# leejaeyong7/tiny-cuda-nn

Hardware: AMD Instinct MI355X
Metric: training_step throughput (samples/s) HashGrid+64-wide FFMLP, batch=256k; % fp16-MFMA peak (higher is better)
Workload: dtype f16

## Files before the change

include/tcnn_amd.h:

```cpp
#ifndef TCNN_AMD_H
#define TCNN_AMD_H

#include <stddef.h>
#include <stdint.h>

#ifdef __cplusplus
extern "C" {
#endif

#define TCNN_OK 0
#define TCNN_ERROR 1

#define TCNN_PRECISION_FP32 0
#define TCNN_PRECISION_FP16 1

#define TCNN_GRADIENT_IGNORE 0
#define TCNN_GRADIENT_OVERWRITE 1
#define TCNN_GRADIENT_ACCUMULATE 2

#define TCNN_LAYOUT_SOA 0
#define TCNN_LAYOUT_AOS 1

#define TCNN_LOG_INFO 0
#define TCNN_LOG_DEBUG 1
#define TCNN_LOG_WARNING 2
#define TCNN_LOG_ERROR 3
#define TCNN_LOG_SUCCESS 4

#define TCNN_MEMCPY_HOST_TO_DEVICE 1
#define TCNN_MEMCPY_DEVICE_TO_HOST 2
#define TCNN_MEMCPY_DEVICE_TO_DEVICE 3

typedef struct tcnn_module_s* tcnn_module_t;
typedef struct tcnn_context_s* tcnn_context_t;
typedef struct tcnn_trainer_s* tcnn_trainer_t;
typedef struct tcnn_train_ctx_s* tcnn_train_ctx_t;
typedef struct tcnn_optimizer_s* tcnn_optimizer_t;
typedef void* tcnn_stream_t;

const char* tcnn_last_error(void);
const char* tcnn_version(void);

uint32_t tcnn_batch_size_granularity(void);
int      tcnn_device(int* device_out);
int      tcnn_set_device(int device);
void     tcnn_free_temporary_memory(void);
int      tcnn_has_networks(void);
float    tcnn_default_loss_scale(int precision);
int      tcnn_preferred_precision(void);
void     tcnn_set_log_callback(void (*callback)(int severity, const char* message, void* user), void* user);

int tcnn_gpu_malloc(size_t bytes, void** out);
int tcnn_gpu_free(void* ptr);
int tcnn_gpu_memcpy(void* dst, const void* src, size_t bytes, int kind);
int tcnn_gpu_memset(void* ptr, int value, size_t bytes);
int tcnn_stream_synchronize(tcnn_stream_t stream);
int tcnn_generate_random_uniform(tcnn_stream_t stream, uint64_t rng_state_inc[2], size_t n, float* out, float lower, float upper);

int  tcnn_create_network_with_input_encoding(uint32_t n_input_dims, uint32_t n_output_dims, const char* encoding_json, const char* network_json, tcnn_module_t* out);
int  tcnn_create_network(uint32_t n_input_dims, uint32_t n_output_dims, const char* network_json, tcnn_module_t* out);
int  tcnn_create_encoding(uint32_t n_input_dims, const char* encoding_json, int precision, tcnn_module_t* out);
int  tcnn_create_network_with_input_encoding_precision(uint32_t n_input_dims, uint32_t n_output_dims, const char* encoding_json, const char* network_json, int precision, tcnn_module_t* out);
int  tcnn_create_network_precision(uint32_t n_input_dims, uint32_t n_output_dims, const char* network_json, int precision, tcnn_module_t* out);
void tcnn_module_destroy(tcnn_module_t module);

int  tcnn_module_inference(tcnn_module_t m, tcnn_stream_t stream, uint32_t n_elements, const float* input, void* output, void* params);
int  tcnn_module_forward(tcnn_module_t m, tcnn_stream_t stream, uint32_t n_elements, const float* input, void* output, void* params,
                         int prepare_input_gradients, tcnn_context_t* ctx_out);
int  tcnn_module_backward(tcnn_module_t m, tcnn_stream_t stream, tcnn_context_t ctx, uint32_t n_elements, float* dL_dinput,
                          const void* dL_doutput, void* dL_dparams, const float* input, const void* output, const void* params);
int  tcnn_module_backward_backward_input(tcnn_module_t m, tcnn_stream_t stream, tcnn_context_t ctx, uint32_t n_elements, const float* dL_ddLdinput,
                                         const float* input, const void* dL_doutput, void* dL_dparams, void* dL_ddLdoutput, float* dL_dinput, const void* params);
int  tcnn_module_backward_backward_input_mode(tcnn_module_t m, tcnn_stream_t stream, tcnn_context_t ctx, uint32_t n_elements, const float* dL_ddLdinput,
                                              const float* input, const void* dL_doutput, void* dL_dparams, void* dL_ddLdoutput, float* dL_dinput, const void* params,
                                              int gradient_mode);
int  tcnn_module_input_gradient(tcnn_module_t m, tcnn_stream_t stream, uint32_t n_elements, uint32_t dim, const float* input, float* d_dinput, void* output,
                                const void* params, float backprop_scale);
const char* tcnn_module_last_input_gradient_route(tcnn_module_t m);
int  tcnn_module_input_jacobian(tcnn_module_t m, tcnn_stream_t stream, uint32_t n_elements, const uint32_t* dims, uint32_t n_dims, const float* input, float* jacobian,
                                void* output, const void* params, float backprop_scale);
const char* tcnn_module_last_input_jacobian_route(tcnn_module_t m);
int  tcnn_module_input_jvp(tcnn_module_t m, tcnn_stream_t stream, uint32_t n_elements, uint32_t n_tangents, const float* input, const float* tangents, void* jvp, void* output,
                           const void* params);
const char* tcnn_module_last_input_jvp_route(tcnn_module_t m);
int  tcnn_module_input_jvp_forward(tcnn_module_t m, tcnn_stream_t stream, uint32_t n_elements, uint32_t n_tangents, const float* input, const float* tangents, void* jvp,
                                   void* output, const void* params, tcnn_context_t* ctx_out);
int  tcnn_module_input_jvp_backward(tcnn_module_t m, tcnn_stream_t stream, tcnn_context_t ctx, uint32_t n_elements, uint32_t n_tangents, const float* input,
                                    const float* tangents, const void* dL_djvp, const void* dL_doutput, const void* params, void* dL_dparams, float* dL_dinput,
                                    float* dL_dtangents, int gradient_mode);
const char* tcnn_module_last_input_jvp_backward_route(tcnn_module_t m);
void tcnn_context_destroy(tcnn_context_t ctx);

uint32_t    tcnn_module_n_input_dims(tcnn_module_t m);
uint32_t    tcnn_module_n_output_dims(tcnn_module_t m);
size_t      tcnn_module_n_params(tcnn_module_t m);
int         tcnn_module_param_precision(tcnn_module_t m);
int         tcnn_module_output_precision(tcnn_module_t m);
int         tcnn_module_initialize_params(tcnn_module_t m, uint64_t seed, float* params_full_precision, float scale);
const char* tcnn_module_hyperparams(tcnn_module_t m);
const char* tcnn_module_name(tcnn_module_t m);

int  tcnn_create_from_config(uint32_t n_input_dims, uint32_t n_output_dims, const char* config_json, tcnn_trainer_t* out);
int  tcnn_create_from_config_seeded(uint32_t n_input_dims, uint32_t n_output_dims, const char* config_json, uint32_t seed, tcnn_trainer_t* out);
int  tcnn_create_from_config_precision(uint32_t n_input_dims, uint32_t n_output_dims, const char* config_json, uint32_t seed, int precision, tcnn_trainer_t* out);
int  tcnn_trainer_precision(tcnn_trainer_t t);
void tcnn_trainer_destroy(tcnn_trainer_t t);

int  tcnn_trainer_training_step(tcnn_trainer_t t, tcnn_stream_t stream, uint32_t n_elements, const float* input, int input_layout,
                                const float* target, const float* data_pdf, int run_optimizer, float* dL_dinput, int use_inference_params,
                                int gradient_mode, const void* external_dL_dy, tcnn_train_ctx_t* ctx_out);
int  tcnn_trainer_loss(tcnn_trainer_t t, tcnn_stream_t stream, tcnn_train_ctx_t ctx, float* loss_out);
int  tcnn_trainer_forward(tcnn_trainer_t t, tcnn_stream_t stream, float loss_scale, uint32_t n_elements, const float* input, int input_layout, const float* target,
                          const float* data_pdf, int use_inference_params, int prepare_input_gradients, const void* external_dL_dy, tcnn_train_ctx_t* ctx_out);
int  tcnn_trainer_backward(tcnn_trainer_t t, tcnn_stream_t stream, tcnn_train_ctx_t ctx, uint32_t n_elements, const float* input, int input_layout,
                           float* dL_dinput, int use_inference_params, int gradient_mode);
int  tcnn_trainer_optimizer_step(tcnn_trainer_t t, tcnn_stream_t stream, float loss_scale);
void tcnn_train_ctx_destroy(tcnn_train_ctx_t ctx);
const void*  tcnn_train_ctx_output(tcnn_train_ctx_t ctx);
const void*  tcnn_train_ctx_dL_doutput(tcnn_train_ctx_t ctx);
const float* tcnn_train_ctx_L(tcnn_train_ctx_t ctx);

int  tcnn_trainer_inference(tcnn_trainer_t t, tcnn_stream_t stream, uint32_t n_elements, const float* input, int input_layout,
                            float* output, int output_layout, int use_inference_params);
int  tcnn_trainer_input_gradient(tcnn_trainer_t t, tcnn_stream_t stream, uint32_t n_elements, uint32_t dim, const float* input, float* d_dinput, float backprop_scale);
int  tcnn_trainer_input_jacobian(tcnn_trainer_t t, tcnn_stream_t stream, uint32_t n_elements, const uint32_t* dims, uint32_t n_dims, const float* input, float* jacobian,
                                 float backprop_scale);
int  tcnn_trainer_input_jvp(tcnn_trainer_t t, tcnn_stream_t stream, uint32_t n_elements, uint32_t n_tangents, const float* input, const float* tangents, void* jvp);
int  tcnn_trainer_input_jvp_forward(tcnn_trainer_t t, tcnn_stream_t stream, uint32_t n_elements, uint32_t n_tangents, const float* input, const float* tangents, void* jvp,
                                    void* output, tcnn_context_t* ctx_out);
int  tcnn_trainer_input_jvp_backward(tcnn_trainer_t t, tcnn_stream_t stream, tcnn_context_t ctx, uint32_t n_elements, uint32_t n_tangents, const float* input,
                                     const float* tangents, const void* dL_djvp, const void* dL_doutput, float* dL_dinput, float* dL_dtangents, int gradient_mode);

int  tcnn_trainer_inference_mixed_precision(tcnn_trainer_t t, tcnn_stream_t stream, uint32_t n_elements, const float* input, int input_layout,
                                            void* output_half, int use_inference_params);

size_t   tcnn_trainer_n_params(tcnn_trainer_t t);
uint32_t tcnn_trainer_padded_output_width(tcnn_trainer_t t);
float*   tcnn_trainer_params_full_precision(tcnn_trainer_t t);
void*    tcnn_trainer_params(tcnn_trainer_t t);
void*    tcnn_trainer_params_inference(tcnn_trainer_t t);
void*    tcnn_trainer_param_gradients(tcnn_trainer_t t);
int      tcnn_trainer_set_params_full_precision(tcnn_trainer_t t, const float* params, size_t n_params, int device_ptr);
int      tcnn_trainer_set_params(tcnn_trainer_t t, const void* params_half, size_t n_params, int device_ptr);
int      tcnn_trainer_initialize_params(tcnn_trainer_t t);
int      tcnn_trainer_update_hyperparams(tcnn_trainer_t t, const char* json);
const char* tcnn_trainer_hyperparams(tcnn_trainer_t t);
int      tcnn_trainer_serialize(tcnn_trainer_t t, int serialize_optimizer, const void** out_bytes, size_t* out_size);
int      tcnn_trainer_deserialize(tcnn_trainer_t t, const void* bytes, size_t size);
const char* tcnn_trainer_network_hyperparams(tcnn_trainer_t t);
uint32_t tcnn_trainer_optimizer_step_count(tcnn_trainer_t t);
int  tcnn_trainer_profile_next_step(tcnn_trainer_t t);
int  tcnn_trainer_profile_collect(tcnn_trainer_t t, tcnn_stream_t stream, float* ms_per_piece , uint32_t* n_steps);
size_t tcnn_trainer_params_updated_in_flush(tcnn_trainer_t t);
size_t tcnn_trainer_image_preps(tcnn_trainer_t t);
size_t tcnn_trainer_scatter_wide_fallbacks(tcnn_trainer_t t);
size_t tcnn_trainer_optimizer_prologue_steps(tcnn_trainer_t t);
size_t tcnn_trainer_list_scatters(tcnn_trainer_t t);
size_t tcnn_module_list_scatters(tcnn_module_t m);
size_t tcnn_trainer_list_gradient_tails(tcnn_trainer_t t);
const char* tcnn_trainer_last_step_kernel(tcnn_trainer_t t);

int   tcnn_module_set_max_level(tcnn_module_t m, float max_level);
float tcnn_module_max_level(tcnn_module_t m);
int   tcnn_module_set_max_level_gpu(tcnn_module_t m, const float* per_sample);
int   tcnn_trainer_set_max_level(tcnn_trainer_t t, float max_level);
int   tcnn_trainer_set_max_level_gpu(tcnn_trainer_t t, const float* per_sample);
float tcnn_trainer_max_level(tcnn_trainer_t t);
int tcnn_train_ctx_keeps_weight_gradient_slabs(tcnn_trainer_t t, tcnn_train_ctx_t ctx);


int         tcnn_module_layer_sizes(tcnn_module_t m, uint32_t* rows_cols, size_t capacity, size_t* n_layers_out);
int         tcnn_optimizer_create(const char* optimizer_json, size_t n_params, const uint32_t* layer_sizes, size_t n_layers, tcnn_optimizer_t* out);
int         tcnn_optimizer_create_precision(const char* optimizer_json, size_t n_params, const uint32_t* layer_sizes, size_t n_layers, int weight_precision, tcnn_optimizer_t* out);
int         tcnn_optimizer_weight_precision(tcnn_optimizer_t o);
void        tcnn_optimizer_destroy(tcnn_optimizer_t o);
int         tcnn_optimizer_step(tcnn_optimizer_t o, tcnn_stream_t stream, float loss_scale, float* params_full_precision, void* params_half,
                                const void* gradients, int gradient_precision);
uint32_t    tcnn_optimizer_step_count(tcnn_optimizer_t o);
size_t      tcnn_optimizer_n_params(tcnn_optimizer_t o);
float       tcnn_optimizer_learning_rate(tcnn_optimizer_t o);
int         tcnn_optimizer_set_learning_rate(tcnn_optimizer_t o, float learning_rate);
int         tcnn_optimizer_update_hyperparams(tcnn_optimizer_t o, const char* json);
const char* tcnn_optimizer_hyperparams(tcnn_optimizer_t o);
void*       tcnn_optimizer_custom_weights(tcnn_optimizer_t o);
int         tcnn_optimizer_weights_restored(tcnn_optimizer_t o, tcnn_stream_t stream, const void* params_half);
int         tcnn_optimizer_serialize(tcnn_optimizer_t o, const void** out_bytes, size_t* out_size);
int         tcnn_optimizer_deserialize(tcnn_optimizer_t o, const void* bytes, size_t size);


int         tcnn_loss_type(const char* loss_json, int* type_out);
const char* tcnn_loss_name(int type);
int         tcnn_loss_evaluate(int type, tcnn_stream_t stream, float loss_scale, const float* scale_dev ,
                               uint32_t n, uint32_t dims, const void* prediction, uint32_t prediction_stride, int precision,
                               const float* target, const float* data_pdf ,
                               float* values, uint32_t values_stride,
                               void* gradients, uint32_t gradients_stride,
                               float* loss_sum );

#ifdef __cplusplus
}
#endif
#endif
```

tiny-cuda-nn_amd/csrc/adam_device.h:

```cpp
#pragma once
#include "tcnn_common.h"

namespace tcnn_amd {

template <typename DebiasOf, typename G, typename W>
__device__ inline void adam_one(const AdamArgs& a, DebiasOf&& debias_of, const float common_debias, const bool is_matrix, const G g_in, float& w_fp, W& w_h,
                                float& m1, float& m2, uint32_t& step, bool& updated) {
	const float g = (float)g_in;
	float gradient = a.inv_loss_scale_exact ? g * a.inv_loss_scale : g / a.loss_scale;
	updated = is_matrix ? a.optimize_matrix_params != 0 : (a.optimize_non_matrix_params != 0 && gradient != 0);
	const float weight_fp = w_fp;
	if (is_matrix) gradient += a.l2_reg * weight_fp;
	const float gradient_sq = gradient * gradient;
	const float first_moment = a.beta1 * m1 + (1 - a.beta1) * gradient;
	const float second_moment = a.beta2 * m2 + (1 - a.beta2) * gradient_sq;
	float learning_rate = a.learning_rate;
	if (!is_matrix) learning_rate *= a.non_matrix_learning_rate_factor;
	const uint32_t current_step = step + 1;
	float debias = common_debias;
	if (updated && current_step != a.common_step) debias = debias_of(min(current_step, a.common_step));
	learning_rate *= debias;
	const float effective_learning_rate = fminf(fmaxf(learning_rate / (sqrtf(second_moment) + a.epsilon), a.lower_lr_bound), a.upper_lr_bound);
	const float decayed_weight = (1 - a.relative_weight_decay * learning_rate) * weight_fp - copysignf(a.absolute_weight_decay * learning_rate, weight_fp);
	float new_weight = decayed_weight - effective_learning_rate * first_moment;
	if (a.weight_clipping_magnitude != 0.0f) new_weight = fminf(fmaxf(new_weight, -a.weight_clipping_magnitude), a.weight_clipping_magnitude);
	w_fp = updated ? new_weight : weight_fp;
	w_h = (W)new_weight;
	m1 = updated ? first_moment : m1;
	m2 = updated ? second_moment : m2;
	step = updated ? current_step : step;
}

}
```

tiny-cuda-nn_amd/csrc/capi.cpp:

```cpp
#include "../../include/tcnn_amd.h"

#include "model.h"

#include <mutex>
#include <string>

using namespace tcnn_amd;

namespace {
thread_local std::string g_last_error;
tcnn_amd::Switches g_switches;
std::mutex g_switches_mutex;

bool env_is(const char* name, char c) {
	const char* e = getenv(name);
	return e && e[0] == c;
}
int env_01(const char* name) {
	const char* e = getenv(name);
	return (e && (e[0] == '0' || e[0] == '1')) ? e[0] - '0' : -1;
}

template <typename F>
int guarded(F&& f) {
	try {
		f();
		return TCNN_OK;
	} catch (const std::exception& e) {
		g_last_error = e.what();
		log_message(TCNN_LOG_ERROR, g_last_error);
		return TCNN_ERROR;
	} catch (...) {
		g_last_error = "unknown error";
		return TCNN_ERROR;
	}
}

Json parse_or_empty(const char* text) {
	if (!text || !*text) return Json::object();
	return Json::parse(text);
}
}

struct tcnn_module_s {
	std::unique_ptr<Model> model;
	std::string hyperparams_text;
	std::string name_text;
};

struct tcnn_context_s {
	std::unique_ptr<ModelContext> ctx;
};

struct tcnn_trainer_s {
	std::unique_ptr<Trainer> trainer;
	std::string hyperparams_text;
	std::string network_hyperparams_text;
	std::vector<uint8_t> snapshot;
};

struct tcnn_train_ctx_s {
	std::unique_ptr<TrainContext> ctx;
};

struct tcnn_optimizer_s {
	std::unique_ptr<Optimizer> optimizer;
	size_t n_params = 0;
	std::string hyperparams_text;
	std::vector<uint8_t> snapshot;
};

namespace tcnn_amd {
Switches switches() {
	std::lock_guard<std::mutex> lock{g_switches_mutex};
	return g_switches;
}
void switches_reload() {
	Switches w;
	w.grid_planes = !env_is("TCNN_AMD_GRID_PLANES", '0');
	w.grid_rows_planes = !env_is("TCNN_AMD_GRID_ROWS_PLANES", '0');
	{ const char* e = getenv("TCNN_AMD_GRID_SCATTER"); w.grid_scatter_lds = !(e && std::string{e} == "atomic"); }
	w.scatter_records = !env_is("TCNN_AMD_SCATTER_RECORDS", '0');
	w.scatter_tune = !env_is("TCNN_AMD_SCATTER_TUNE", '0');
	w.scatter_lists = env_01("TCNN_AMD_SCATTER_LISTS");
	w.scatter_wide = env_is("TCNN_AMD_SCATTER_WIDE", '1');
	w.fused_step = !env_is("TCNN_AMD_FUSED_STEP", '0');
	w.side_jobs = !env_is("TCNN_AMD_SIDE_JOBS", '0');
	w.live_image = !env_is("TCNN_AMD_LIVE_IMAGE", '0');
	w.adam_steps32 = env_is("TCNN_AMD_ADAM_STEPS32", '1');
	w.adam_in_reduce = !env_is("TCNN_AMD_ADAM_IN_REDUCE", '0');
	w.adam_prologue = !env_is("TCNN_AMD_ADAM_PROLOGUE", '0');
	w.adam_prologue_refused = env_is("TCNN_AMD_ADAM_PROLOGUE", 'r');
	w.mlp_r32 = !env_is("TCNN_AMD_MLP_R32", '0');
	w.mlp_r32a = env_01("TCNN_AMD_MLP_R32A");
	w.mlp_regs = !env_is("TCNN_AMD_MLP_REGS", '0');
	w.mlp_fast = !env_is("TCNN_AMD_MLP_FAST", '0');
	if (const char* e = getenv("TCNN_AMD_MLP_PRIO")) w.mlp_prio = (uint32_t)atoi(e);
	w.listgrad_in_mlp = !env_is("TCNN_AMD_LISTGRAD_IN_MLP", '0');
	w.mlp_layerwise = env_is("TCNN_AMD_MLP_LAYERWISE", '1');
	w.mlp_regw = !env_is("TCNN_AMD_MLP_REGW", '0');
	if (const char* e = getenv("TCNN_AMD_MLP_VARIANT")) {
		int v[3] = {0, 0, 0};
		if (sscanf(e, "%d,%d,%d", &v[0], &v[1], &v[2]) == 3) {
			w.mlp_variant_forced = true;
			for (int i = 0; i < 3; ++i) w.mlp_variant[i] = v[i];
		}
	}
	w.wgrad_rows = !env_is("TCNN_AMD_WGRAD_ROWS", '0');
	w.mlp_fwd_lds = !env_is("TCNN_AMD_MLP_FWD_LDS", '0');
	w.fuse_oneblob = !env_is("TCNN_AMD_FUSE_ONEBLOB", '0');
	std::lock_guard<std::mutex> lock{g_switches_mutex};
	g_switches = w;
}
}

extern "C" {

const char* tcnn_last_error(void) { return g_last_error.c_str(); }
const char* tcnn_version(void) { return "tcnn_amd 0.1 (gfx950)"; }

uint32_t tcnn_batch_size_granularity(void) { return BATCH_SIZE_GRANULARITY; }

int tcnn_device(int* device_out) {
	return guarded([&] { HIP_CHECK_THROW(hipGetDevice(device_out)); });
}

int tcnn_set_device(int device) {
	return guarded([&] { HIP_CHECK_THROW(hipSetDevice(device)); });
}

void tcnn_free_temporary_memory(void) { Arena::instance().release_all(); }

int tcnn_gpu_malloc(size_t bytes, void** out) {
	return guarded([&] {
		CHECK_THROW(out != nullptr);
		*out = nullptr;
		if (bytes) HIP_CHECK_THROW(hipMalloc(out, bytes));
	});
}
int tcnn_gpu_free(void* ptr) {
	return guarded([&] { if (ptr) HIP_CHECK_THROW(hipFree(ptr)); });
}
int tcnn_gpu_memcpy(void* dst, const void* src, size_t bytes, int kind) {
	return guarded([&] {
		const hipMemcpyKind k = kind == TCNN_MEMCPY_HOST_TO_DEVICE ? hipMemcpyHostToDevice : kind == TCNN_MEMCPY_DEVICE_TO_HOST ? hipMemcpyDeviceToHost : hipMemcpyDeviceToDevice;
		if (bytes) HIP_CHECK_THROW(hipMemcpy(dst, src, bytes, k));
	});
}
int tcnn_gpu_memset(void* ptr, int value, size_t bytes) {
	return guarded([&] { if (bytes) HIP_CHECK_THROW(hipMemset(ptr, value, bytes)); });
}
int tcnn_stream_synchronize(tcnn_stream_t stream) {
	return guarded([&] { HIP_CHECK_THROW(hipStreamSynchronize((hipStream_t)stream)); });
}
int tcnn_generate_random_uniform(tcnn_stream_t stream, uint64_t rng_state_inc[2], size_t n, float* out, float lower, float upper) {
	return guarded([&] {
		CHECK_THROW(rng_state_inc != nullptr && (out != nullptr || n == 0));
		generate_random_uniform((hipStream_t)stream, rng_state_inc, n, out, lower, upper);
		HIP_CHECK_THROW(hipGetLastError());
	});
}
int tcnn_has_networks(void) { return 1; }
float tcnn_default_loss_scale(int precision) { return precision == TCNN_PRECISION_FP32 ? 1.0f : LOSS_SCALE_FP16; }
int tcnn_preferred_precision(void) { return TCNN_PRECISION_FP16; }

void tcnn_set_log_callback(void (*callback)(int, const char*, void*), void* user) {
	log_sink().callback = callback;
	log_sink().user = user;
}

int tcnn_create_network_with_input_encoding_precision(uint32_t n_input_dims, uint32_t n_output_dims, const char* encoding_json, const char* network_json, int precision, tcnn_module_t* out) {
	switches_reload();
	return guarded([&] {
		CHECK_THROW(out != nullptr);
		if (precision != TCNN_PRECISION_FP32 && precision != TCNN_PRECISION_FP16) throw std::runtime_error{"Unknown precision " + std::to_string(precision)};
		auto m = std::make_unique<tcnn_module_s>();
		m->model.reset(new NetworkWithInputEncoding{n_input_dims, n_output_dims, parse_or_empty(encoding_json), parse_or_empty(network_json),
		                                            precision == TCNN_PRECISION_FP32 ? Precision::Fp32 : Precision::Fp16});
		*out = m.release();
	});
}

int tcnn_create_network_with_input_encoding(uint32_t n_input_dims, uint32_t n_output_dims, const char* encoding_json, const char* network_json, tcnn_module_t* out) {
	return tcnn_create_network_with_input_encoding_precision(n_input_dims, n_output_dims, encoding_json, network_json, TCNN_PRECISION_FP16, out);
}

int tcnn_create_network_precision(uint32_t n_input_dims, uint32_t n_output_dims, const char* network_json, int precision, tcnn_module_t* out) {
	return tcnn_create_network_with_input_encoding_precision(n_input_dims, n_output_dims, "{\"otype\": \"Identity\"}", network_json, precision, out);
}

int tcnn_create_network(uint32_t n_input_dims, uint32_t n_output_dims, const char* network_json, tcnn_module_t* out) {
	return tcnn_create_network_precision(n_input_dims, n_output_dims, network_json, TCNN_PRECISION_FP16, out);
}

int tcnn_create_encoding(uint32_t n_input_dims, const char* encoding_json, int precision, tcnn_module_t* out) {
	switches_reload();
	return guarded([&] {
		CHECK_THROW(out != nullptr);
		auto m = std::make_unique<tcnn_module_s>();
		m->model.reset(new EncodingModel{n_input_dims, parse_or_empty(encoding_json), precision == TCNN_PRECISION_FP32 ? Precision::Fp32 : Precision::Fp16});
		*out = m.release();
	});
}

void tcnn_module_destroy(tcnn_module_t module) { delete module; }

int tcnn_module_inference(tcnn_module_t m, tcnn_stream_t stream, uint32_t n, const float* input, void* output, void* params) {
	return guarded([&] {
		CHECK_THROW(m && m->model);
		m->model->inference((hipStream_t)stream, n, MatView{input, m->model->input_width(), 1u}, output, params);
	});
}

int tcnn_module_forward(tcnn_module_t m, tcnn_stream_t stream, uint32_t n, const float* input, void* output, void* params, int prepare_input_gradients, tcnn_context_t* ctx_out) {
	return guarded([&] {
		CHECK_THROW(m && m->model && ctx_out);
		auto c = std::make_unique<tcnn_context_s>();
		c->ctx = m->model->forward((hipStream_t)stream, n, MatView{input, m->model->input_width(), 1u}, output, params, prepare_input_gradients != 0);
		*ctx_out = c.release();
	});
}

int tcnn_module_backward(tcnn_module_t m, tcnn_stream_t stream, tcnn_context_t ctx, uint32_t n, float* dL_dinput, const void* dL_doutput, void* dL_dparams,
                         const float* input, const void* output, const void* params) {
	return guarded([&] {
		CHECK_THROW(m && m->model);
		if (!ctx || !ctx->ctx || dynamic_cast<const Model::InputJvpContext*>(ctx->ctx.get())) {
			throw std::runtime_error{"Module::bwd: called with invalid context. fwd likely (mistakenly) ran in inference mode."};
		}
		MatViewMut dx{dL_dinput, m->model->input_width(), 1u};
		m->model->backward((hipStream_t)stream, *ctx->ctx, n, MatView{input, m->model->input_width(), 1u}, output, dL_doutput, dL_dinput ? &dx : nullptr, params,
		                   dL_dparams, dL_dparams ? GradientMode::Overwrite : GradientMode::Ignore);
	});
}

int tcnn_module_backward_backward_input(tcnn_module_t m, tcnn_stream_t stream, tcnn_context_t ctx, uint32_t n, const float* dL_ddLdinput, const float* input, const void* dL_doutput,
                                        void* dL_dparams, void* dL_ddLdoutput, float* dL_dinput, const void* params) {
	return tcnn_module_backward_backward_input_mode(m, stream, ctx, n, dL_ddLdinput, input, dL_doutput, dL_dparams, dL_ddLdoutput, dL_dinput, params,
	                                                dL_dparams ? TCNN_GRADIENT_OVERWRITE : TCNN_GRADIENT_IGNORE);
}

int tcnn_module_backward_backward_input_mode(tcnn_module_t m, tcnn_stream_t stream, tcnn_context_t ctx, uint32_t n, const float* dL_ddLdinput, const float* input, const void* dL_doutput,
                                             void* dL_dparams, void* dL_ddLdoutput, float* dL_dinput, const void* params, int gradient_mode) {
	return guarded([&] {
		CHECK_THROW(gradient_mode == TCNN_GRADIENT_IGNORE || ((gradient_mode == TCNN_GRADIENT_OVERWRITE || gradient_mode == TCNN_GRADIENT_ACCUMULATE) && dL_dparams != nullptr));
		CHECK_THROW(m && m->model);
		if (!ctx || !ctx->ctx || dynamic_cast<const Model::InputJvpContext*>(ctx->ctx.get())) {
			throw std::runtime_error{"Module::bwd_bwd_input: called with invalid context. fwd likely (mistakenly) ran in inference mode."};
		}
		CHECK_THROW(dL_ddLdinput != nullptr && input != nullptr);
		const uint32_t w = m->model->input_width();
		MatViewMut dx{dL_dinput, w, 1u};
		m->model->backward_backward_input((hipStream_t)stream, *ctx->ctx, n, MatView{input, w, 1u}, MatView{dL_ddLdinput, w, 1u}, dL_doutput, dL_ddLdoutput, dL_dinput ? &dx : nullptr, params,
		                                  gradient_mode == TCNN_GRADIENT_IGNORE ? nullptr : dL_dparams, (GradientMode)gradient_mode);
	});
}

int tcnn_module_input_gradient(tcnn_module_t m, tcnn_stream_t stream, uint32_t n, uint32_t dim, const float* input, float* d_dinput, void* output, const void* params,
                               float backprop_scale) {
	return guarded([&] {
		CHECK_THROW(m && m->model);
		const uint32_t w = m->model->input_width();
		m->model->input_gradient((hipStream_t)stream, n, dim, MatView{input, w, 1u}, MatViewMut{d_dinput, w, 1u}, output, params, backprop_scale);
	});
}

const char* tcnn_module_last_input_gradient_route(tcnn_module_t m) {
	if (!m || !m->model) {
		g_last_error = "tcnn_module_last_input_gradient_route: null module";
		return nullptr;
	}
	return m->model->last_input_gradient_route();
}

int tcnn_module_input_jacobian(tcnn_module_t m, tcnn_stream_t stream, uint32_t n, const uint32_t* dims, uint32_t n_dims, const float* input, float* jacobian, void* output,
                               const void* params, float backprop_scale) {
	return guarded([&] {
		CHECK_THROW(m && m->model);
		m->model->input_jacobian((hipStream_t)stream, n, dims, n_dims, MatView{input, m->model->input_width(), 1u}, jacobian, output, params, backprop_scale);
	});
}

const char* tcnn_module_last_input_jacobian_route(tcnn_module_t m) {
	if (!m || !m->model) {
		g_last_error = "tcnn_module_last_input_jacobian_route: null module";
		return nullptr;
	}
	return m->model->last_input_jacobian_route();
}

int tcnn_module_input_jvp(tcnn_module_t m, tcnn_stream_t stream, uint32_t n, uint32_t n_tangents, const float* input, const float* tangents, void* jvp, void* output, const void* params) {
	return guarded([&] {
		CHECK_THROW(m && m->model);
		m->model->input_jvp((hipStream_t)stream, n, n_tangents, MatView{input, m->model->input_width(), 1u}, tangents, jvp, output, params);
	});
}

const char* tcnn_module_last_input_jvp_route(tcnn_module_t m) {
	if (!m || !m->model) {
		g_last_error = "tcnn_module_last_input_jvp_route: null module";
		return nullptr;
	}
	return m->model->last_input_jvp_route();
}

int tcnn_module_input_jvp_forward(tcnn_module_t m, tcnn_stream_t stream, uint32_t n, uint32_t n_tangents, const float* input, const float* tangents, void* jvp, void* output,
                                  const void* params, tcnn_context_t* ctx_out) {
	return guarded([&] {
		CHECK_THROW(m && m->model && ctx_out);
		auto c = std::make_unique<tcnn_context_s>();
		c->ctx = m->model->input_jvp_forward((hipStream_t)stream, n, n_tangents, MatView{input, m->model->input_width(), 1u}, tangents, jvp, output, params);
		*ctx_out = c.release();
	});
}

int tcnn_module_input_jvp_backward(tcnn_module_t m, tcnn_stream_t stream, tcnn_context_t ctx, uint32_t n, uint32_t n_tangents, const float* input, const float* tangents,
                                   const void* dL_djvp, const void* dL_doutput, const void* params, void* dL_dparams, float* dL_dinput, float* dL_dtangents, int gradient_mode) {
	return guarded([&] {
		CHECK_THROW(gradient_mode == TCNN_GRADIENT_IGNORE || ((gradient_mode == TCNN_GRADIENT_OVERWRITE || gradient_mode == TCNN_GRADIENT_ACCUMULATE) && dL_dparams != nullptr));
		CHECK_THROW(m && m->model);
		if (!ctx || !ctx->ctx) throw std::runtime_error{"Module::bwd: called with invalid context. fwd likely (mistakenly) ran in inference mode."};
		MatViewMut dx{dL_dinput, m->model->input_width(), 1u};
		m->model->input_jvp_backward((hipStream_t)stream, *ctx->ctx, n, n_tangents, MatView{input, m->model->input_width(), 1u}, tangents, dL_djvp, dL_doutput, params,
		                             gradient_mode == TCNN_GRADIENT_IGNORE ? nullptr : dL_dparams, dL_dinput ? &dx : nullptr, dL_dtangents, (GradientMode)gradient_mode);
	});
}

const char* tcnn_module_last_input_jvp_backward_route(tcnn_module_t m) {
	if (!m || !m->model) {
		g_last_error = "tcnn_module_last_input_jvp_backward_route: null module";
		return nullptr;
	}
	return m->model->last_input_jvp_backward_route();
}

void tcnn_context_destroy(tcnn_context_t ctx) { delete ctx; }

uint32_t tcnn_module_n_input_dims(tcnn_module_t m) { return m->model->input_width(); }
uint32_t tcnn_module_n_output_dims(tcnn_module_t m) { return m->model->padded_output_width(); }
size_t tcnn_module_n_params(tcnn_module_t m) { return m->model->n_params(); }
size_t tcnn_module_list_scatters(tcnn_module_t m) { return (size_t)m->model->list_scatters(); }

namespace {
[[noreturn]] void no_grid(Model& model) {
	throw std::runtime_error{"max_level: " + model.name() + " has no grid encoding (GridEncoding::set_max_level, grid_interface.h:101-123)"};
}
}

int tcnn_module_set_max_level(tcnn_module_t m, float max_level) {
	return guarded([&] {
		CHECK_THROW(m && m->model);
		if (!m->model->set_max_level(max_level)) no_grid(*m->model);
	});
}
int tcnn_module_set_max_level_gpu(tcnn_module_t m, const float* per_sample) {
	return guarded([&] {
		CHECK_THROW(m && m->model);
		if (!m->model->set_max_level_gpu(per_sample)) no_grid(*m->model);
	});
}
float tcnn_module_max_level(tcnn_module_t m) {
	float v = std::numeric_limits<float>::quiet_NaN();
	const float* per_sample = nullptr;
	guarded([&] {
		CHECK_THROW(m && m->model);
		if (!m->model->get_max_level(v, per_sample)) no_grid(*m->model);
		g_last_error.clear();
	});
	return v;
}
int tcnn_module_param_precision(tcnn_module_t m) { return (int)m->model->precision(); }
int tcnn_module_output_precision(tcnn_module_t m) { return (int)m->model->precision(); }

int tcnn_module_initialize_params(tcnn_module_t m, uint64_t seed, float* params_full_precision, float scale) {
	return guarded([&] {
		CHECK_THROW(m && m->model);
		Pcg32 rng{seed};
		m->model->initialize_params(rng, params_full_precision, scale);
		HIP_CHECK_THROW(hipDeviceSynchronize());
	});
}

const char* tcnn_module_hyperparams(tcnn_module_t m) {
	m->hyperparams_text = m->model->hyperparams().dump();
	return m->hyperparams_text.c_str();
}

const char* tcnn_module_name(tcnn_module_t m) {
	m->name_text = m->model->name();
	return m->name_text.c_str();
}

int tcnn_create_from_config_precision(uint32_t n_input_dims, uint32_t n_output_dims, const char* config_json, uint32_t seed, int precision, tcnn_trainer_t* out) {
	switches_reload();
	return guarded([&] {
		CHECK_THROW(out != nullptr);
		if (precision != TCNN_PRECISION_FP32 && precision != TCNN_PRECISION_FP16) throw std::runtime_error{"Unknown precision " + std::to_string(precision)};
		auto t = std::make_unique<tcnn_trainer_s>();
		t->trainer.reset(new Trainer{n_input_dims, n_output_dims, parse_or_empty(config_json), seed, precision == TCNN_PRECISION_FP32 ? Precision::Fp32 : Precision::Fp16});
		*out = t.release();
	});
}

int tcnn_create_from_config_seeded(uint32_t n_input_dims, uint32_t n_output_dims, const char* config_json, uint32_t seed, tcnn_trainer_t* out) {
	return tcnn_create_from_config_precision(n_input_dims, n_output_dims, config_json, seed, TCNN_PRECISION_FP16, out);
}

int tcnn_trainer_precision(tcnn_trainer_t t) {
	int v = -1;
	guarded([&] { CHECK_THROW(t && t->trainer); v = (int)t->trainer->precision(); });
	return v;
}

int tcnn_create_from_config(uint32_t n_input_dims, uint32_t n_output_dims, const char* config_json, tcnn_trainer_t* out) {
	return tcnn_create_from_config_seeded(n_input_dims, n_output_dims, config_json, 1337, out);
}

void tcnn_trainer_destroy(tcnn_trainer_t t) { delete t; }

int tcnn_trainer_training_step(tcnn_trainer_t t, tcnn_stream_t stream, uint32_t n, const float* input, int input_layout, const float* target, const float* data_pdf,
                               int run_optimizer, float* dL_dinput, int use_inference_params, int gradient_mode, const void* external_dL_dy, tcnn_train_ctx_t* ctx_out) {
	return guarded([&] {
		CHECK_THROW(t && t->trainer && ctx_out);
		Trainer& tr = *t->trainer;
		const uint32_t w = tr.model().input_width();
		MatViewMut dx = make_view_mut(dL_dinput, w, n, input_layout);
		auto c = std::make_unique<tcnn_train_ctx_s>();
		c->ctx = tr.training_step((hipStream_t)stream, n, make_view(input, w, n, input_layout), target, data_pdf, run_optimizer != 0, dL_dinput ? &dx : nullptr,
		                          use_inference_params != 0, (GradientMode)gradient_mode, external_dL_dy);
		*ctx_out = c.release();
	});
}

int tcnn_trainer_loss(tcnn_trainer_t t, tcnn_stream_t stream, tcnn_train_ctx_t ctx, float* loss_out) {
	return guarded([&] {
		CHECK_THROW(t && t->trainer && ctx && ctx->ctx && loss_out);
		*loss_out = t->trainer->loss((hipStream_t)stream, *ctx->ctx);
	});
}

int tcnn_trainer_forward(tcnn_trainer_t t, tcnn_stream_t stream, float loss_scale, uint32_t n, const float* input, int input_layout, const float* target, const float* data_pdf,
                         int use_inference_params, int prepare_input_gradients, const void* external_dL_dy, tcnn_train_ctx_t* ctx_out) {
	return guarded([&] {
		CHECK_THROW(t && t->trainer && ctx_out);
		Trainer& tr = *t->trainer;
		auto c = std::make_unique<tcnn_train_ctx_s>();
		c->ctx = tr.forward((hipStream_t)stream, loss_scale, n, make_view(input, tr.model().input_width(), n, input_layout), target, data_pdf, use_inference_params != 0,
		                    prepare_input_gradients != 0, external_dL_dy);
		*ctx_out = c.release();
	});
}

int tcnn_trainer_backward(tcnn_trainer_t t, tcnn_stream_t stream, tcnn_train_ctx_t ctx, uint32_t n, const float* input, int input_layout, float* dL_dinput,
                          int use_inference_params, int gradient_mode) {
	return guarded([&] {
		CHECK_THROW(t && t->trainer && ctx && ctx->ctx);
		Trainer& tr = *t->trainer;
		const uint32_t w = tr.model().input_width();
		MatViewMut dx = make_view_mut(dL_dinput, w, n, input_layout);
		tr.backward((hipStream_t)stream, *ctx->ctx, n, make_view(input, w, n, input_layout), dL_dinput ? &dx : nullptr, use_inference_params != 0, (GradientMode)gradient_mode);
	});
}

int tcnn_trainer_optimizer_step(tcnn_trainer_t t, tcnn_stream_t stream, float loss_scale) {
// ... 337 lines not shown
```

tiny-cuda-nn_amd/csrc/k_misc.hip:

```cpp
#include "tcnn_common.h"
#include "adam_device.h"
#include "grid_fixed.h"
#include "loss_device.h"
#include "mlp_side_jobs.h"
#include "oneblob_device.h"
#include "reduce_device.h"

#include <hip/hip_fp16.h>

#include <cmath>
#include <limits>

namespace tcnn_amd {
namespace {

typedef _Float16 half_t;
typedef _Float16 h8 __attribute__((ext_vector_type(8)));
typedef _Float16 h4 __attribute__((ext_vector_type(4)));

template <typename T>
__global__ void __launch_bounds__(256) k_oneblob_fwd(const uint32_t n, const uint32_t n_dims, const uint32_t log2_bins, const MatView x, T* __restrict__ out, const uint32_t out_stride) {
	const uint32_t gid = blockIdx.x * blockDim.x + threadIdx.x;
	const uint32_t i = gid / out_stride;
	if (i >= n) return;
	const uint32_t j = gid - i * out_stride;
	const uint32_t n_bins = 1u << log2_bins;
	if (j >= n_dims * n_bins) {
		out[gid] = (T)1.0f;
		return;
	}
	const uint32_t dim = j >> log2_bins, bin = j & (n_bins - 1);
	const float xv = x.data[(size_t)i * x.stride_sample + (size_t)dim * x.stride_dim];
	const float nb = (float)n_bins;
	const float lb = scalbnf((float)bin, -(int)log2_bins);
	const float l = quartic_cdf(lb - xv, nb) + quartic_cdf(lb - xv - 1.0f, nb) + quartic_cdf(lb - xv + 1.0f, nb);
	const float rb = scalbnf((float)((bin + 1) & (n_bins - 1)), -(int)log2_bins);
	float r = quartic_cdf(rb - xv, nb) + quartic_cdf(rb - xv - 1.0f, nb) + quartic_cdf(rb - xv + 1.0f, nb);
	if (bin == n_bins - 1) r += 1;
	out[gid] = (T)(r - l);
}

template <typename T>
__global__ void __launch_bounds__(256) k_oneblob_fwd8(const uint32_t n, const uint32_t n_dims, const uint32_t log2_bins, const MatView x, T* __restrict__ out, const uint32_t out_stride) {
	const uint32_t gid = blockIdx.x * blockDim.x + threadIdx.x;
	const uint32_t chunks = out_stride / 8;
	const uint32_t i = gid / chunks;
	if (i >= n) return;
	const uint32_t j0 = (gid - i * chunks) * 8;
	const uint32_t n_bins = 1u << log2_bins;
	typedef T vec8 __attribute__((ext_vector_type(8)));
	vec8 v;
	if (j0 >= n_dims * n_bins) {
#pragma unroll
		for (int k = 0; k < 8; ++k) v[k] = (T)1.0f;
	} else {
		const uint32_t dim = j0 >> log2_bins, b0 = j0 & (n_bins - 1);
		const float xv = x.data[(size_t)i * x.stride_sample + (size_t)dim * x.stride_dim];
		const float nb = (float)n_bins;
		float edge[9];
#pragma unroll
		for (int k = 0; k < 9; ++k) {
			const float lb = scalbnf((float)((b0 + k) & (n_bins - 1)), -(int)log2_bins);
			edge[k] = quartic_cdf(lb - xv, nb) + quartic_cdf(lb - xv - 1.0f, nb) + quartic_cdf(lb - xv + 1.0f, nb);
		}
		if (b0 + 8 == n_bins) edge[8] += 1;
#pragma unroll
		for (int k = 0; k < 8; ++k) v[k] = (T)(edge[k + 1] - edge[k]);
	}
	*(vec8*)(out + (size_t)i * out_stride + j0) = v;
}

template <typename T, int CPR>
__global__ void __launch_bounds__(256) k_oneblob_fwd_sparse(const uint32_t n, const uint32_t n_dims, const uint32_t log2_bins, const MatView x, T* __restrict__ out, const uint32_t out_stride) {
	const uint32_t gid = blockIdx.x * blockDim.x + threadIdx.x;
	typedef T vec8 __attribute__((ext_vector_type(8)));
	const uint32_t n_bins = 1u << log2_bins;
	constexpr uint32_t cpr = CPR;
	const uint32_t row_threads = n * n_dims * cpr;
	if (gid >= row_threads) {
		const uint32_t pad_chunks = (out_stride - n_dims * n_bins) >> 3;
		const uint32_t p = gid - row_threads;
		if (pad_chunks == 0 || p >= n * pad_chunks) return;
		const uint32_t i = p / pad_chunks, pc = p - i * pad_chunks;
		vec8 ones;
#pragma unroll
		for (int k = 0; k < 8; ++k) ones[k] = (T)1.0f;
		*(vec8*)(out + (size_t)i * out_stride + n_dims * n_bins + 8 * pc) = ones;
		return;
	}
	const uint32_t r = gid / cpr, j = gid - r * cpr;
	const uint32_t i = r / n_dims, dim = r - i * n_dims;
	const uint32_t b0 = 8 * j;
	const float xv = x.data[(size_t)i * x.stride_sample + (size_t)dim * x.stride_dim];
	const float nb = (float)n_bins;
	auto edge = [&](const uint32_t bin) {
		const float lb = scalbnf((float)(bin & (n_bins - 1)), -(int)log2_bins);
		return quartic_cdf(lb - xv, nb) + quartic_cdf(lb - xv - 1.0f, nb) + quartic_cdf(lb - xv + 1.0f, nb);
	};
	vec8 v;
	if (!(xv >= 0.0f && xv <= 1.0f)) {
		float e[9];
#pragma unroll
		for (int k = 0; k < 9; ++k) e[k] = edge(b0 + k);
		if (b0 + 8 == n_bins) e[8] += 1;
#pragma unroll
		for (int k = 0; k < 8; ++k) v[k] = (T)(e[k + 1] - e[k]);
	} else {
		const uint32_t centre = (uint32_t)(int)floorf(xv * nb) + n_bins - 2u;
		constexpr int PER = (5 + CPR - 1) / CPR;
		float mine[PER];
#pragma unroll
		for (int t = 0; t < PER; ++t) {
			const uint32_t o = min(j + (uint32_t)t * cpr, 4u);
			const uint32_t bin = (centre + o) & (n_bins - 1);
			const float l = edge(bin);
			float rr = edge(bin + 1);
			if (bin == n_bins - 1) rr += 1;
			mine[t] = rr - l;
		}
#pragma unroll
		for (int k = 0; k < 8; ++k) v[k] = (T)0.0f;
#pragma unroll
		for (int o = 0; o < 5; ++o) {
			const float val = CPR == 1 ? mine[o / CPR] : __shfl(mine[o / CPR], o % CPR, CPR);
			const uint32_t d = ((centre + o) & (n_bins - 1)) - b0;
#pragma unroll
			for (int k = 0; k < 8; ++k) v[k] = d == (uint32_t)k ? (T)val : v[k];
		}
	}
	*(vec8*)(out + (size_t)i * out_stride + (size_t)dim * n_bins + b0) = v;
}

template <typename T>
__global__ void __launch_bounds__(128) k_oneblob_bwd_input(const uint32_t n, const uint32_t n_dims, const uint32_t log2_bins, const MatView x, const T* __restrict__ dL_dy, const uint32_t dy_stride, const MatViewMut dL_dx) {
	const uint32_t gid = blockIdx.x * blockDim.x + threadIdx.x;
	const uint32_t i = gid / n_dims;
	if (i >= n) return;
	const uint32_t j = gid - i * n_dims;
	const uint32_t n_bins = 1u << log2_bins;
	const float nb = (float)n_bins;
	const float xv = x.data[(size_t)i * x.stride_sample + (size_t)j * x.stride_dim];
	float result = 0;
	float left = quartic_cdf_deriv(-xv, nb) + quartic_cdf_deriv(-xv - 1.0f, nb) + quartic_cdf_deriv(-xv + 1.0f, nb);
	for (uint32_t k = 0; k < n_bins; ++k) {
		const float rb = scalbnf((float)(k + 1), -(int)log2_bins);
		const float right = quartic_cdf_deriv(rb - xv, nb) + quartic_cdf_deriv(rb - xv - 1.0f, nb) + quartic_cdf_deriv(rb - xv + 1.0f, nb);
		const float deriv = left - right;
		left = right;
		result += (float)dL_dy[(size_t)i * dy_stride + j * n_bins + k] * deriv;
	}
	dL_dx.data[(size_t)i * dL_dx.stride_sample + (size_t)j * dL_dx.stride_dim] = result;
}

template <typename T>
__global__ void __launch_bounds__(256) k_identity_fwd(const uint32_t n, const uint32_t n_dims, const float scale, const float offset, const MatView x, T* __restrict__ out, const uint32_t out_stride) {
	const uint32_t gid = blockIdx.x * blockDim.x + threadIdx.x;
	const uint32_t i = gid / out_stride;
	if (i >= n) return;
	const uint32_t j = gid - i * out_stride;
	out[gid] = j >= n_dims ? (T)1.0f : (T)(x.data[(size_t)i * x.stride_sample + (size_t)j * x.stride_dim] * scale + offset);
}

template <typename T>
__global__ void __launch_bounds__(256) k_identity_bwd_input(const uint32_t n, const uint32_t n_dims, const float scale, const T* __restrict__ dL_dy, const uint32_t dy_stride, const MatViewMut dL_dx) {
	const uint32_t gid = blockIdx.x * blockDim.x + threadIdx.x;
	const uint32_t i = gid / n_dims;
	if (i >= n) return;
	const uint32_t j = gid - i * n_dims;
	dL_dx.data[(size_t)i * dL_dx.stride_sample + (size_t)j * dL_dx.stride_dim] = (float)(T)((float)dL_dy[(size_t)i * dy_stride + j] * scale);
}

template <typename T>
__global__ void __launch_bounds__(256) k_identity_bwd_bwd_input(const uint32_t n, const uint32_t n_dims, const float scale, const MatView dL_ddLdx, T* __restrict__ dL_ddLdy, const uint32_t dy_stride) {
	const uint32_t gid = blockIdx.x * blockDim.x + threadIdx.x;
	const uint32_t i = gid / dy_stride;
	if (i >= n) return;
	const uint32_t j = gid - i * dy_stride;
	dL_ddLdy[gid] = j >= n_dims ? (T)0.0f : (T)(dL_ddLdx.data[(size_t)i * dL_ddLdx.stride_sample + (size_t)j * dL_ddLdx.stride_dim] * scale);
}


template <typename P>
__global__ void __launch_bounds__(256) k_loss(
	const uint32_t type, const uint32_t n_elements, const uint32_t stride, const uint32_t dims, const float loss_scale,
	const P* __restrict__ predictions, const float* __restrict__ targets, float* __restrict__ values, P* __restrict__ gradients, const float* __restrict__ data_pdf
) {
	const uint32_t i = blockIdx.x * blockDim.x + threadIdx.x;
	if (i >= n_elements) return;
	const uint32_t intra = i % stride;
	const uint32_t inter = i / stride;
	if (intra >= dims) {
		values[i] = 0;
		gradients[i] = (P)0.0f;
		return;
	}
	const uint32_t target_idx = inter * dims + intra;
	const uint32_t n_total = n_elements / stride * dims;
	const float prediction = (float)predictions[i];
	const float pdf = data_pdf ? data_pdf[target_idx] : 1;
	float value;
	P grad;
	loss_element(type, prediction, targets[target_idx], pdf, n_total, loss_scale, predictions + (i - intra), dims, value, grad);
	values[i] = value;
	gradients[i] = grad;
}

__global__ void __launch_bounds__(256) k_loss8(
	const uint32_t type, const uint32_t n_elements, const uint32_t stride, const uint32_t dims, const uint32_t n_total, const float loss_scale,
	const half_t* __restrict__ predictions, const float* __restrict__ targets, float* __restrict__ values, half_t* __restrict__ gradients, const float* __restrict__ data_pdf
) {
	const uint32_t i0 = (blockIdx.x * blockDim.x + threadIdx.x) * 8;
	if (i0 >= n_elements) return;
	const uint32_t inter = i0 / stride, intra0 = i0 - inter * stride;
	const h8 pv = *(const h8*)(predictions + i0);
	float v[8];
	h8 g;
#pragma unroll
	for (int k = 0; k < 8; ++k) {
		const uint32_t intra = intra0 + k;
		v[k] = 0;
		g[k] = (half_t)0.0f;
		if (intra < dims) {
			const uint32_t target_idx = inter * dims + intra;
			const float pdf = data_pdf ? data_pdf[target_idx] : 1;
			half_t gk;
			loss_element(type, (float)pv[k], targets[target_idx], pdf, n_total, loss_scale, predictions + (i0 - intra0), dims, v[k], gk);
			g[k] = gk;
		}
	}
	*(float4*)(values + i0) = float4{v[0], v[1], v[2], v[3]};
	*(float4*)(values + i0 + 4) = float4{v[4], v[5], v[6], v[7]};
	*(h8*)(gradients + i0) = g;
}

__global__ void __launch_bounds__(256) k_loss4_f32(
	const uint32_t type, const uint32_t n_elements, const uint32_t stride, const uint32_t dims, const uint32_t n_total, const float loss_scale,
	const float* __restrict__ predictions, const float* __restrict__ targets, float* __restrict__ values, float* __restrict__ gradients, const float* __restrict__ data_pdf
) {
	const uint32_t i0 = (blockIdx.x * blockDim.x + threadIdx.x) * 4;
	if (i0 >= n_elements) return;
	const uint32_t inter = i0 / stride, intra0 = i0 - inter * stride;
	const float4 pv4 = *(const float4*)(predictions + i0);
	const float pv[4] = {pv4.x, pv4.y, pv4.z, pv4.w};
	float v[4], g[4];
#pragma unroll
	for (int k = 0; k < 4; ++k) {
		const uint32_t intra = intra0 + k;
		v[k] = 0;
		g[k] = 0;
		if (intra < dims) {
			const uint32_t target_idx = inter * dims + intra;
			const float pdf = data_pdf ? data_pdf[target_idx] : 1;
			loss_element(type, pv[k], targets[target_idx], pdf, n_total, loss_scale, predictions + (i0 - intra0), dims, v[k], g[k]);
		}
	}
	*(float4*)(values + i0) = float4{v[0], v[1], v[2], v[3]};
	*(float4*)(gradients + i0) = float4{g[0], g[1], g[2], g[3]};
}

__global__ void __launch_bounds__(256) k_reduce_stage1(const size_t n, const float* __restrict__ values, float* __restrict__ partials) {
	__shared__ float sm[4];
	float acc = 0.0f;
	const size_t n4 = n / 4;
	const float4* v4 = (const float4*)values;
	for (size_t i = (size_t)blockIdx.x * blockDim.x + threadIdx.x; i < n4; i += (size_t)gridDim.x * blockDim.x) {
		const float4 v = v4[i];
		acc += (v.x + v.y) + (v.z + v.w);
	}
	if (blockIdx.x == 0 && threadIdx.x < (n & 3)) acc += values[n4 * 4 + threadIdx.x];
	const float s = block_sum_256(acc, sm);
	if (threadIdx.x == 0) partials[blockIdx.x] = s;
}

__global__ void __launch_bounds__(256) k_reduce_stage2(const uint32_t n_partials, const float* __restrict__ partials, float* __restrict__ result) {
	__shared__ float sm[4];
	float acc = 0.0f;
	for (uint32_t i = threadIdx.x; i < n_partials; i += 256) acc += partials[i];
	const float s = block_sum_256(acc, sm);
	if (threadIdx.x == 0) *result = s;
}


__device__ inline float adam_debias(const float beta1, const float beta2, uint32_t step) { return sqrtf(1 - powf(beta2, (float)step)) / (1 - powf(beta1, (float)step)); }

__global__ void __launch_bounds__(256) k_adam_debias_table(const float beta1, const float beta2, const uint32_t from, const uint32_t to, float* __restrict__ table) {
	const uint32_t t = from + blockIdx.x * blockDim.x + threadIdx.x;
	if (t < to) table[t] = adam_debias(beta1, beta2, t);
}

constexpr int ADAM_Q = 1;

typedef uint16_t adam_u16x4 __attribute__((ext_vector_type(4)));
template <typename STEP_T> __device__ inline uint4 adam_load_steps(const STEP_T* p) {
	if constexpr (sizeof(STEP_T) == 2) {
		const adam_u16x4 v = *(const adam_u16x4*)p;
		return uint4{v[0], v[1], v[2], v[3]};
	} else {
		return *(const uint4*)p;
	}
}
template <typename STEP_T> __device__ inline void adam_store_steps(STEP_T* p, const uint4 v) {
	if constexpr (sizeof(STEP_T) == 2) *(adam_u16x4*)p = adam_u16x4{(uint16_t)v.x, (uint16_t)v.y, (uint16_t)v.z, (uint16_t)v.w};
	else *(uint4*)p = v;
}
typedef float f4 __attribute__((ext_vector_type(4)));
template <typename G> struct GradQuad;
template <> struct GradQuad<half_t> { typedef h4 type; };
template <> struct GradQuad<float> { typedef f4 type; };
template <bool QUAD_UNIFORM, typename STEP_T, typename G, typename W>
__global__ void __launch_bounds__(256) k_adam(
	const AdamArgs a, const size_t n, const size_t n_matrix,
	float* __restrict__ w_fp, W* __restrict__ w, const G* __restrict__ g, float* __restrict__ m1, float* __restrict__ m2, STEP_T* __restrict__ steps,
	const float* __restrict__ debias_table
) {
	const size_t base = (size_t)blockIdx.x * (256 * 4 * ADAM_Q) + threadIdx.x * 4;
	const float debias = debias_table[a.common_step];
	const auto from_table = [&](const uint32_t t) { return debias_table[t]; };
	typedef typename GradQuad<G>::type g4;
	g4 gv[ADAM_Q];
	bool live[ADAM_Q];
#pragma unroll
	for (int q = 0; q < ADAM_Q; ++q) {
		const size_t i4 = base + (size_t)q * 1024;
		live[q] = i4 + 4 <= n;
		gv[q] = live[q] ? *(const g4*)(g + i4) : g4{0, 0, 0, 0};
	}
#pragma unroll
	for (int q = 0; q < ADAM_Q; ++q) {
		const size_t i4 = base + (size_t)q * 1024;
		const bool zero = gv[q][0] == (G)0.0f && gv[q][1] == (G)0.0f && gv[q][2] == (G)0.0f && gv[q][3] == (G)0.0f;
		if (live[q] && i4 >= n_matrix && zero) live[q] = false;
	}
	float4 wf[ADAM_Q], a1[ADAM_Q], a2[ADAM_Q];
	uint4 st[ADAM_Q];
#pragma unroll
	for (int q = 0; q < ADAM_Q; ++q) {
		const size_t i4 = base + (size_t)q * 1024;
		if (live[q]) {
			wf[q] = *(const float4*)(w_fp + i4);
			a1[q] = *(const float4*)(m1 + i4);
			a2[q] = *(const float4*)(m2 + i4);
			st[q] = adam_load_steps(steps + i4);
		}
	}
#pragma unroll
	for (int q = 0; q < ADAM_Q; ++q) {
		const size_t i4 = base + (size_t)q * 1024;
		if (live[q]) {
			W wh[4];
			bool up[4];
			const bool quad_matrix = i4 < n_matrix;
			adam_one(a, from_table, debias, QUAD_UNIFORM ? quad_matrix : i4 + 0 < n_matrix, gv[q][0], wf[q].x, wh[0], a1[q].x, a2[q].x, st[q].x, up[0]);
			adam_one(a, from_table, debias, QUAD_UNIFORM ? quad_matrix : i4 + 1 < n_matrix, gv[q][1], wf[q].y, wh[1], a1[q].y, a2[q].y, st[q].y, up[1]);
			adam_one(a, from_table, debias, QUAD_UNIFORM ? quad_matrix : i4 + 2 < n_matrix, gv[q][2], wf[q].z, wh[2], a1[q].z, a2[q].z, st[q].z, up[2]);
			adam_one(a, from_table, debias, QUAD_UNIFORM ? quad_matrix : i4 + 3 < n_matrix, gv[q][3], wf[q].w, wh[3], a1[q].w, a2[q].w, st[q].w, up[3]);
			*(float4*)(w_fp + i4) = wf[q];
			*(float4*)(m1 + i4) = a1[q];
			*(float4*)(m2 + i4) = a2[q];
			adam_store_steps(steps + i4, st[q]);
			if constexpr (sizeof(W) == 2) {
				if (up[0] && up[1] && up[2] && up[3]) {
					*(h4*)(w + i4) = h4{wh[0], wh[1], wh[2], wh[3]};
				} else {
#pragma unroll
					for (int e = 0; e < 4; ++e) if (up[e]) w[i4 + e] = wh[e];
				}
			}
		} else if (i4 < n && i4 + 4 > n) {
			for (size_t i = i4; i < n; ++i) {
				bool up;
				W wh;
				uint32_t st1 = steps[i];
				adam_one(a, from_table, debias, i < n_matrix, g[i], w_fp[i], wh, m1[i], m2[i], st1, up);
				steps[i] = (STEP_T)st1;
				if constexpr (sizeof(W) == 2) { if (up) w[i] = wh; }
			}
		}
	}
}

template <typename STEP_T, typename G, typename W>
__global__ void __launch_bounds__(256) k_adam_scalar(
	const AdamArgs a, const size_t n, const size_t n_matrix,
	float* __restrict__ w_fp, W* __restrict__ w, const G* __restrict__ g, float* __restrict__ m1, float* __restrict__ m2, STEP_T* __restrict__ steps,
	const float* __restrict__ debias_table
) {
	const size_t i = (size_t)blockIdx.x * blockDim.x + threadIdx.x;
	if (i >= n) return;
	const float debias = debias_table[a.common_step];
	const auto from_table = [&](const uint32_t t) { return debias_table[t]; };
	bool up;
	W wh;
	uint32_t st1 = steps[i];
	adam_one(a, from_table, debias,  i < n_matrix, g[i], w_fp[i], wh, m1[i], m2[i], st1, up);
	steps[i] = (STEP_T)st1;
	if constexpr (sizeof(W) == 2) { if (up) w[i] = wh; }
}

__global__ void __launch_bounds__(128) k_random_uniform(const size_t n, const uint64_t state, const uint64_t inc, float* __restrict__ out, const float lower, const float upper) {
	const uint64_t MULT = 0x5851f42d4c957f2dULL;
	const size_t i = (size_t)blockIdx.x * blockDim.x + threadIdx.x;
	const size_t n_threads = (size_t)blockDim.x * gridDim.x;
	uint64_t cur_mult = MULT, cur_plus = inc, acc_mult = 1u, acc_plus = 0u;
	uint64_t delta = (uint64_t)i * 4;
	while (delta > 0) {
		if (delta & 1) {
			acc_mult *= cur_mult;
			acc_plus = acc_plus * cur_mult + cur_plus;
		}
		cur_plus = (cur_mult + 1) * cur_plus;
		cur_mult *= cur_mult;
		delta /= 2;
	}
	uint64_t st = acc_mult * state + acc_plus;
	for (size_t j = 0; j < 4; ++j) {
		const size_t idx = i + n_threads * j;
		if (idx >= n) return;
		const uint64_t old = st;
		st = old * MULT + inc;
		const uint32_t xorshifted = (uint32_t)(((old >> 18u) ^ old) >> 27u);
		const uint32_t rot = (uint32_t)(old >> 59u);
		const uint32_t u = ((xorshifted >> rot) | (xorshifted << ((~rot + 1u) & 31)));
		const float f = __uint_as_float((u >> 9) | 0x3f800000u) - 1.0f;
		out[idx] = f * (upper - lower) + lower;
	}
}

__global__ void __launch_bounds__(256) k_cast_f2h(const size_t n, const float* __restrict__ in, half_t* __restrict__ out) {
	const size_t i = ((size_t)blockIdx.x * blockDim.x + threadIdx.x) * 4;
	if (i + 4 <= n) {
		const float4 v = *(const float4*)(in + i);
		*(h4*)(out + i) = h4{(half_t)v.x, (half_t)v.y, (half_t)v.z, (half_t)v.w};
	} else {
		for (size_t k = i; k < n; ++k) out[k] = (half_t)in[k];
	}
}

__global__ void __launch_bounds__(256) k_cast_h2f(const size_t n, const half_t* __restrict__ in, float* __restrict__ out) {
	const size_t i = ((size_t)blockIdx.x * blockDim.x + threadIdx.x) * 4;
	if (i + 4 <= n) {
		const h4 v = *(const h4*)(in + i);
		*(float4*)(out + i) = float4{(float)v[0], (float)v[1], (float)v[2], (float)v[3]};
	} else {
		for (size_t k = i; k < n; ++k) out[k] = (float)in[k];
	}
}

template <typename T>
__global__ void __launch_bounds__(256) k_trim_and_cast(const uint32_t n, const uint32_t in_stride, const uint32_t dims, const T* __restrict__ in, const MatViewMut out) {
	const uint32_t gid = blockIdx.x * blockDim.x + threadIdx.x;
	const uint32_t i = gid / dims;
	if (i >= n) return;
	const uint32_t d = gid - i * dims;
	out.data[(size_t)i * out.stride_sample + (size_t)d * out.stride_dim] = (float)in[(size_t)i * in_stride + d];
}

__global__ void __launch_bounds__(256) k_fill_half(const size_t n, half_t* __restrict__ out, const half_t v) {
	const size_t i = (size_t)blockIdx.x * blockDim.x + threadIdx.x;
	if (i < n) out[i] = v;
}

inline uint32_t log2_exact(uint32_t v) {
	uint32_t l = 0;
	while ((1u << l) < v) ++l;
	return l;
}

inline uint32_t blocks_for(uint64_t total, uint32_t threads) {
	const uint64_t b = (total + threads - 1) / threads;
	CHECK_THROW(b < (1ull << 31));
	return (uint32_t)b;
}

}

void oneblob_forward(hipStream_t stream, bool fp32, uint32_t n, uint32_t n_dims, uint32_t n_bins, MatView x, void* out, uint32_t out_stride) {
	const uint64_t total = (uint64_t)n * out_stride;
	if (total == 0) return;
	CHECK_THROW(total < (1ull << 32));
	const uint32_t lb = log2_exact(n_bins);
	if (n_bins % 8 == 0 && n_bins <= 512 && out_stride % 8 == 0) {
		const uint64_t threads = total / 8;
		const dim3 grid(blocks_for(threads, 256));
#define TCNN_ONEBLOB_SPARSE(CPR_) \
		case CPR_: \
			if (fp32) hipLaunchKernelGGL((k_oneblob_fwd_sparse<float, CPR_>), grid, dim3(256), 0, stream, n, n_dims, lb, x, (float*)out, out_stride); \
			else hipLaunchKernelGGL((k_oneblob_fwd_sparse<half_t, CPR_>), grid, dim3(256), 0, stream, n, n_dims, lb, x, (half_t*)out, out_stride); \
			break;
		switch (n_bins / 8) {
			TCNN_ONEBLOB_SPARSE(1) TCNN_ONEBLOB_SPARSE(2) TCNN_ONEBLOB_SPARSE(4) TCNN_ONEBLOB_SPARSE(8)
			TCNN_ONEBLOB_SPARSE(16) TCNN_ONEBLOB_SPARSE(32) TCNN_ONEBLOB_SPARSE(64)
			default: CHECK_THROW(false);
		}
#undef TCNN_ONEBLOB_SPARSE
		return;
	}
	if (n_bins % 8 == 0 && out_stride % 8 == 0) {
		const uint64_t threads = total / 8;
		if (fp32) hipLaunchKernelGGL(k_oneblob_fwd8<float>, dim3(blocks_for(threads, 256)), dim3(256), 0, stream, n, n_dims, lb, x, (float*)out, out_stride);
		else hipLaunchKernelGGL(k_oneblob_fwd8<half_t>, dim3(blocks_for(threads, 256)), dim3(256), 0, stream, n, n_dims, lb, x, (half_t*)out, out_stride);
		return;
	}
	if (fp32) hipLaunchKernelGGL(k_oneblob_fwd<float>, dim3(blocks_for(total, 256)), dim3(256), 0, stream, n, n_dims, lb, x, (float*)out, out_stride);
	else hipLaunchKernelGGL(k_oneblob_fwd<half_t>, dim3(blocks_for(total, 256)), dim3(256), 0, stream, n, n_dims, lb, x, (half_t*)out, out_stride);
}

void oneblob_backward_input(hipStream_t stream, bool fp32, uint32_t n, uint32_t n_dims, uint32_t n_bins, MatView x, const void* dL_dy, uint32_t dy_stride, MatViewMut dL_dx) {
	const uint64_t total = (uint64_t)n * n_dims;
	if (total == 0) return;
	const uint32_t lb = log2_exact(n_bins);
	if (fp32) hipLaunchKernelGGL(k_oneblob_bwd_input<float>, dim3(blocks_for(total, 128)), dim3(128), 0, stream, n, n_dims, lb, x, (const float*)dL_dy, dy_stride, dL_dx);
	else hipLaunchKernelGGL(k_oneblob_bwd_input<half_t>, dim3(blocks_for(total, 128)), dim3(128), 0, stream, n, n_dims, lb, x, (const half_t*)dL_dy, dy_stride, dL_dx);
}

void identity_forward(hipStream_t stream, bool fp32, uint32_t n, uint32_t n_dims, float scale, float offset, MatView x, void* out, uint32_t out_stride) {
	const uint64_t total = (uint64_t)n * out_stride;
	if (total == 0) return;
	CHECK_THROW(total < (1ull << 32));
	if (fp32) hipLaunchKernelGGL(k_identity_fwd<float>, dim3(blocks_for(total, 256)), dim3(256), 0, stream, n, n_dims, scale, offset, x, (float*)out, out_stride);
	else hipLaunchKernelGGL(k_identity_fwd<half_t>, dim3(blocks_for(total, 256)), dim3(256), 0, stream, n, n_dims, scale, offset, x, (half_t*)out, out_stride);
}

void identity_backward_input(hipStream_t stream, bool fp32, uint32_t n, uint32_t n_dims, float scale, const void* dL_dy, uint32_t dy_stride, MatViewMut dL_dx) {
	const uint64_t total = (uint64_t)n * n_dims;
	if (total == 0) return;
	if (fp32) hipLaunchKernelGGL(k_identity_bwd_input<float>, dim3(blocks_for(total, 256)), dim3(256), 0, stream, n, n_dims, scale, (const float*)dL_dy, dy_stride, dL_dx);
	else hipLaunchKernelGGL(k_identity_bwd_input<half_t>, dim3(blocks_for(total, 256)), dim3(256), 0, stream, n, n_dims, scale, (const half_t*)dL_dy, dy_stride, dL_dx);
}

void identity_backward_backward_input(hipStream_t stream, bool fp32, uint32_t n, uint32_t n_dims, float scale, MatView dL_ddLdx, void* dL_ddLdy, uint32_t dy_stride) {
	const uint64_t total = (uint64_t)n * dy_stride;
	if (total == 0) return;
	CHECK_THROW(total < (1ull << 32));
	if (fp32) hipLaunchKernelGGL(k_identity_bwd_bwd_input<float>, dim3(blocks_for(total, 256)), dim3(256), 0, stream, n, n_dims, scale, dL_ddLdx, (float*)dL_ddLdy, dy_stride);
	else hipLaunchKernelGGL(k_identity_bwd_bwd_input<half_t>, dim3(blocks_for(total, 256)), dim3(256), 0, stream, n, n_dims, scale, dL_ddLdx, (half_t*)dL_ddLdy, dy_stride);
}

void loss_evaluate(hipStream_t stream, LossType type, uint32_t n, uint32_t stride, uint32_t dims, float loss_scale,
                   const void* pred_half, const float* target, float* values, void* grads_half, const float* data_pdf, Precision precision) {
	const uint64_t total = (uint64_t)n * stride;
	if (total == 0) return;
	CHECK_THROW(total < (1ull << 32));
	if (precision == Precision::Fp32) {
		if (stride % 4 == 0 && ((uintptr_t)pred_half | (uintptr_t)values | (uintptr_t)grads_half) % 16 == 0) {
			hipLaunchKernelGGL(k_loss4_f32, dim3(blocks_for(total / 4, 256)), dim3(256), 0, stream, (uint32_t)type, (uint32_t)total, stride, dims, (uint32_t)(total / stride * dims), loss_scale,
			                   (const float*)pred_half, target, values, (float*)grads_half, data_pdf);
			return;
		}
		hipLaunchKernelGGL(k_loss<float>, dim3(blocks_for(total, 256)), dim3(256), 0, stream, (uint32_t)type, (uint32_t)total, stride, dims, loss_scale,
		                   (const float*)pred_half, target, values, (float*)grads_half, data_pdf);
		return;
	}
	if (stride % 8 == 0 && ((uintptr_t)pred_half | (uintptr_t)values | (uintptr_t)grads_half) % 16 == 0) {
		hipLaunchKernelGGL(k_loss8, dim3(blocks_for(total / 8, 256)), dim3(256), 0, stream, (uint32_t)type, (uint32_t)total, stride, dims, (uint32_t)(total / stride * dims), loss_scale,
		                   (const half_t*)pred_half, target, values, (half_t*)grads_half, data_pdf);
		return;
	}
	hipLaunchKernelGGL(k_loss<half_t>, dim3(blocks_for(total, 256)), dim3(256), 0, stream, (uint32_t)type, (uint32_t)total, stride, dims, loss_scale,
	                   (const half_t*)pred_half, target, values, (half_t*)grads_half, data_pdf);
}

void reduce_sum(hipStream_t stream, size_t n, const float* values, float* partials, float* result_dev) {
	uint32_t blocks = blocks_for((n + 3) / 4, 256);
	if (blocks > 1024) blocks = 1024;
	if (blocks == 0) blocks = 1;
	hipLaunchKernelGGL(k_reduce_stage1, dim3(blocks), dim3(256), 0, stream, n, values, partials);
	hipLaunchKernelGGL(k_reduce_stage2, dim3(1), dim3(256), 0, stream, blocks, partials, result_dev);
}

void reduce_partials(hipStream_t stream, uint32_t n_partials, const float* partials, float* result_dev) {
	hipLaunchKernelGGL(k_reduce_stage2, dim3(1), dim3(256), 0, stream, n_partials, partials, result_dev);
}

AdamArgs make_adam_args(const AdamHyper& h, float loss_scale, uint32_t current_step) {
	AdamArgs a;
	a.relative_weight_decay = h.relative_decay;
	a.absolute_weight_decay = h.absolute_decay;
	a.weight_clipping_magnitude = h.clipping_magnitude;
	a.loss_scale = loss_scale;
	a.learning_rate = h.learning_rate;
	a.non_matrix_learning_rate_factor = h.non_matrix_learning_rate_factor;
	a.beta1 = h.beta1;
	a.beta2 = h.beta2;
	a.epsilon = h.epsilon;
	a.lower_lr_bound = 0;
	a.upper_lr_bound = std::numeric_limits<float>::max();
	if (h.adabound) {
		a.lower_lr_bound = 0.1f - 0.1f / ((1 - h.beta2) * (float)current_step + 1);
		a.upper_lr_bound = 0.1f + 0.1f / ((1 - h.beta2) * (float)current_step);
	}
	a.l2_reg = h.l2_reg;
	a.optimize_matrix_params = h.optimize_matrix_params;
	a.optimize_non_matrix_params = h.optimize_non_matrix_params;
	a.common_step = current_step;
	int exponent = 0;
	a.inv_loss_scale_exact = (std::frexp(loss_scale, &exponent) == 0.5f && loss_scale >= 1.0f / 65536 && loss_scale <= 65536.0f) ? 1 : 0;
	a.inv_loss_scale = 1.0f / loss_scale;
	return a;
}

namespace {
__global__ void __launch_bounds__(256) k_adam_widen_steps(const size_t n, const uint16_t* __restrict__ in, uint32_t* __restrict__ out) {
	const size_t i = (size_t)blockIdx.x * blockDim.x + threadIdx.x;
	if (i < n) out[i] = in[i];
}
template <typename STEP_T, typename G, typename W>
void adam_launch(hipStream_t stream, const AdamArgs& a, size_t n, size_t n_matrix, float* w_fp, W* w, const G* g, float* m1, float* m2, STEP_T* steps, const float* debias_table) {
	const auto aligned = [](const void* p, size_t bytes) { return ((uintptr_t)p & (bytes - 1)) == 0; };
	if (!(aligned(w_fp, 16) && aligned(m1, 16) && aligned(m2, 16) && aligned(steps, 4 * sizeof(STEP_T)) && (sizeof(W) == 4 || aligned(w, 8)) && aligned(g, 4 * sizeof(G)))) {
		hipLaunchKernelGGL((k_adam_scalar<STEP_T, G, W>), dim3(blocks_for(n, 256)), dim3(256), 0, stream, a, n, n_matrix, w_fp, w, g, m1, m2, steps, debias_table);
		return;
	}
	const dim3 grid(blocks_for((n + 3) / 4, 256 * ADAM_Q));
	if (n_matrix % 4 == 0) hipLaunchKernelGGL((k_adam<true, STEP_T, G, W>), grid, dim3(256), 0, stream, a, n, n_matrix, w_fp, w, g, m1, m2, steps, debias_table);
	else hipLaunchKernelGGL((k_adam<false, STEP_T, G, W>), grid, dim3(256), 0, stream, a, n, n_matrix, w_fp, w, g, m1, m2, steps, debias_table);
}
template <typename G, typename W>
void adam_launch_steps(hipStream_t stream, const AdamArgs& a, size_t n, size_t n_matrix, float* w_fp, W* w, const G* g, float* m1, float* m2, void* steps, bool steps16, const float* debias_table) {
	if (steps16) adam_launch<uint16_t, G, W>(stream, a, n, n_matrix, w_fp, w, g, m1, m2, (uint16_t*)steps, debias_table);
	else adam_launch<uint32_t, G, W>(stream, a, n, n_matrix, w_fp, w, g, m1, m2, (uint32_t*)steps, debias_table);
}
}

void adam_widen_steps(hipStream_t stream, size_t n, const void* steps16, void* steps32) {
	if (n == 0) return;
	hipLaunchKernelGGL(k_adam_widen_steps, dim3(blocks_for(n, 256)), dim3(256), 0, stream, n, (const uint16_t*)steps16, (uint32_t*)steps32);
}

void adam_step(hipStream_t stream, const AdamHyper& h, size_t n, size_t n_matrix, float loss_scale, uint32_t current_step,
               float* w_fp, void* w_half, const void* gradients, float* m1, float* m2, void* steps, bool steps16, const float* debias_table, GradientPrecision precision, Precision weight_precision) {
	if (n == 0) return;
	const AdamArgs a = make_adam_args(h, loss_scale, current_step);
	if (weight_precision == Precision::Fp32) {
		CHECK_THROW(precision == GradientPrecision::Fp32);
		adam_launch_steps(stream, a, n, n_matrix, w_fp, (float*)nullptr, (const float*)gradients, m1, m2, steps, steps16, debias_table);
	} else if (precision == GradientPrecision::Fp32) adam_launch_steps(stream, a, n, n_matrix, w_fp, (half_t*)w_half, (const float*)gradients, m1, m2, steps, steps16, debias_table);
	else adam_launch_steps(stream, a, n, n_matrix, w_fp, (half_t*)w_half, (const half_t*)gradients, m1, m2, steps, steps16, debias_table);
}

namespace {
constexpr uint32_t PRO_THREADS = SLAB_REDUCE_ELEMS * SLAB_REDUCE_GROUPS;
constexpr uint32_t PRO_MAX_BLOCKS_PER_RANGE = 64;
__host__ __device__ inline uint32_t pro_range_blocks(const uint32_t n_elems) { return min(PRO_MAX_BLOCKS_PER_RANGE, max(1u, (n_elems / 4 + PRO_THREADS - 1) / PRO_THREADS)); }

template <typename STEP_T, typename DebiasOf>
__device__ inline void adam_quad(const AdamArgs& a, DebiasOf&& from_table, const float debias, const bool quad_matrix, const size_t i4, const h4 gv,
                                 float* __restrict__ w_fp, half_t* __restrict__ w, float* __restrict__ m1, float* __restrict__ m2, STEP_T* __restrict__ steps) {
	if (!quad_matrix && gv[0] == (half_t)0.0f && gv[1] == (half_t)0.0f && gv[2] == (half_t)0.0f && gv[3] == (half_t)0.0f) return;
	float4 wf = *(const float4*)(w_fp + i4), a1 = *(const float4*)(m1 + i4), a2 = *(const float4*)(m2 + i4);
	uint4 st = adam_load_steps(steps + i4);
	half_t wh[4];
	bool up[4];
	adam_one(a, from_table, debias, quad_matrix, gv[0], wf.x, wh[0], a1.x, a2.x, st.x, up[0]);
	adam_one(a, from_table, debias, quad_matrix, gv[1], wf.y, wh[1], a1.y, a2.y, st.y, up[1]);
	adam_one(a, from_table, debias, quad_matrix, gv[2], wf.z, wh[2], a1.z, a2.z, st.z, up[2]);
	adam_one(a, from_table, debias, quad_matrix, gv[3], wf.w, wh[3], a1.w, a2.w, st.w, up[3]);
	*(float4*)(w_fp + i4) = wf;
	*(float4*)(m1 + i4) = a1;
	*(float4*)(m2 + i4) = a2;
	adam_store_steps(steps + i4, st);
	if (up[0] && up[1] && up[2] && up[3]) {
		*(h4*)(w + i4) = h4{wh[0], wh[1], wh[2], wh[3]};
	} else {
#pragma unroll
		for (int e = 0; e < 4; ++e) if (up[e]) w[i4 + e] = wh[e];
	}
}

struct PrologueArgs {
	uint32_t n_reduce_blocks, reduce_elems, reduce_slabs;
	int reduce_accumulate;
	const float* slabs;
	const GridScatterRange* ranges;
	uint32_t n_ranges, n_range_blocks;
	int accumulate;
	unsigned long long* scratch;
	size_t range_base;
	size_t bulk_begin;
};

#ifndef TCNN_PRO_BOUNDS
#define TCNN_PRO_BOUNDS __launch_bounds__(PRO_THREADS)
#endif
#ifndef TCNN_PRO_Q
#define TCNN_PRO_Q 1
#endif
constexpr int PRO_Q = TCNN_PRO_Q;
template <typename STEP_T>
__global__ void TCNN_PRO_BOUNDS k_adam_prologue(const AdamArgs a, const size_t n, const size_t n_matrix, float* __restrict__ w_fp, half_t* __restrict__ w, half_t* __restrict__ g,
                                                               float* __restrict__ m1, float* __restrict__ m2, STEP_T* __restrict__ steps, const float* __restrict__ debias_table, const PrologueArgs p) {
	__shared__ float part[SLAB_REDUCE_GROUPS * SLAB_REDUCE_ELEMS];
	const float debias = debias_table[a.common_step];
	const auto from_table = [&](const uint32_t t) { return debias_table[t]; };
	const uint32_t tid = threadIdx.x;
	if (blockIdx.x < p.n_reduce_blocks) {
		const uint32_t e = tid & (SLAB_REDUCE_ELEMS - 1), grp = tid / SLAB_REDUCE_ELEMS;
		const uint32_t i = blockIdx.x * SLAB_REDUCE_ELEMS + e;
		float q[4] = {0, 0, 0, 0};
		if (i < p.reduce_elems) {
			uint32_t k = grp;
			for (; k + 3 * SLAB_REDUCE_GROUPS < p.reduce_slabs; k += 4 * SLAB_REDUCE_GROUPS) {
#pragma unroll
				for (int u = 0; u < 4; ++u) q[u] += p.slabs[(size_t)(k + u * SLAB_REDUCE_GROUPS) * p.reduce_elems + i];
			}
			for (; k < p.reduce_slabs; k += SLAB_REDUCE_GROUPS) q[0] += p.slabs[(size_t)k * p.reduce_elems + i];
		}
		part[grp * SLAB_REDUCE_ELEMS + e] = (q[0] + q[1]) + (q[2] + q[3]);
		__syncthreads();
		if (grp == 0 && i < p.reduce_elems) {
			float s = 0;
#pragma unroll
			for (int gi = 0; gi < SLAB_REDUCE_GROUPS; ++gi) s += part[gi * SLAB_REDUCE_ELEMS + e];
			if (p.reduce_accumulate) s += (float)g[i];
			const half_t gh = (half_t)s;
			g[i] = gh;
			bool up;
			half_t wh;
			uint32_t st1 = steps[i];
			adam_one(a, from_table, debias, i < n_matrix, gh, w_fp[i], wh, m1[i], m2[i], st1, up);
			steps[i] = (STEP_T)st1;
			if (up) w[i] = wh;
		}
		return;
	}
	const uint32_t b = blockIdx.x - p.n_reduce_blocks;
	if (b < p.n_range_blocks) {
		uint32_t ri = 0, first = 0;
		for (uint32_t nb = pro_range_blocks(p.ranges[0].n_elems); b >= first + nb; nb = pro_range_blocks(p.ranges[ri].n_elems)) { first += nb; ++ri; }
		const GridScatterRange r = p.ranges[ri];
		const uint32_t my = b - first, of = pro_range_blocks(r.n_elems);
		typedef unsigned long long u64x2 __attribute__((ext_vector_type(2)));
		u64x2* sc = (u64x2*)(p.scratch + r.scratch_begin);
		const size_t g0 = p.range_base + r.grad_begin;
		for (uint32_t quad = my * PRO_THREADS + tid; quad < r.n_elems / 4; quad += of * PRO_THREADS) {
			const u64x2 lo = sc[2 * quad], hi = sc[2 * quad + 1];
			sc[2 * quad] = u64x2{0, 0};
			sc[2 * quad + 1] = u64x2{0, 0};
			long long s[4] = {(long long)lo.x, (long long)lo.y, (long long)hi.x, (long long)hi.y};
			const size_t i4 = g0 + 4 * (size_t)quad;
			if (p.accumulate) {
				const h4 old = *(const h4*)(g + i4);
#pragma unroll
				for (int e = 0; e < 4; ++e) s[e] += half_to_fixed(old[e]);
			}
			const h4 gv = h4{fixed_to_half(s[0]), fixed_to_half(s[1]), fixed_to_half(s[2]), fixed_to_half(s[3])};
			*(h4*)(g + i4) = gv;
			adam_quad(a, from_table, debias, i4 < n_matrix, i4, gv, w_fp, w, m1, m2, steps);
		}
		return;
	}
	h4 gv[PRO_Q];
	bool live[PRO_Q];
#pragma unroll
	for (int k = 0; k < PRO_Q; ++k) {
		const size_t i4 = p.bulk_begin + (((size_t)(b - p.n_range_blocks) * PRO_Q + k) * PRO_THREADS + tid) * 4;
		live[k] = i4 < n;
		for (uint32_t r = 0; r < p.n_ranges; ++r) {
			const size_t rb = p.range_base + p.ranges[r].grad_begin;
			if (i4 >= rb && i4 < rb + p.ranges[r].n_elems) live[k] = false;
		}
		if (live[k]) gv[k] = *(const h4*)(g + i4);
	}
#pragma unroll
	for (int k = 0; k < PRO_Q; ++k) {
		const size_t i4 = p.bulk_begin + (((size_t)(b - p.n_range_blocks) * PRO_Q + k) * PRO_THREADS + tid) * 4;
		if (live[k]) adam_quad(a, from_table, debias, i4 < n_matrix, i4, gv[k], w_fp, w, m1, m2, steps);
	}
}
}

bool adam_step_with_prologue(hipStream_t stream, const AdamHyper& h, size_t n, size_t n_matrix, float loss_scale, uint32_t current_step,
                             float* w_fp, void* w_half, void* g_half, float* m1, float* m2, void* steps, bool steps16, const float* debias_table, const AdamPrologue& pro) {
	const auto aligned = [](const void* ptr, size_t bytes) { return ((uintptr_t)ptr & (bytes - 1)) == 0; };
	if (n == 0 || !(aligned(w_fp, 16) && aligned(m1, 16) && aligned(m2, 16) && aligned(steps, steps16 ? 8 : 16) && aligned(w_half, 8) && aligned(g_half, 8))) return false;
	PrologueArgs p{};
	p.bulk_begin = 0;
	if (pro.has_reduce) {
		if (pro.reduce_elems % 4 != 0 || pro.reduce_elems > n || n_matrix % 4 != 0) return false;
		p.n_reduce_blocks = div_round_up(pro.reduce_elems, (uint32_t)SLAB_REDUCE_ELEMS);
		p.reduce_elems = pro.reduce_elems;
		p.reduce_slabs = pro.reduce_slabs;
		p.reduce_accumulate = pro.reduce_accumulate;
		p.slabs = pro.slabs;
		p.bulk_begin = pro.reduce_elems;
	} else if (n_matrix % 4 != 0) return false;
	if ((n - p.bulk_begin) % 4 != 0) return false;
	if (!pro.ranges.empty()) {
		if ((const char*)pro.grad_base < (const char*)g_half || !aligned(pro.scratch, 16)) return false;
		p.range_base = (size_t)((const half_t*)pro.grad_base - (const half_t*)g_half);
		if (p.range_base % 4 != 0) return false;
		for (const GridScatterRange& r : pro.ranges) {
			if (r.grad_begin % 4 != 0 || r.n_elems % 4 != 0 || r.scratch_begin % 2 != 0 || p.range_base + r.grad_begin + r.n_elems > n || p.range_base + r.grad_begin < p.bulk_begin) return false;
		}
		for (bool moved = true; moved;) {
			moved = false;
			for (const GridScatterRange& r : pro.ranges) {
				if (r.n_elems && p.range_base + r.grad_begin == p.bulk_begin) { p.bulk_begin += r.n_elems; moved = true; }
			}
		}
		p.ranges = pro.dev_ranges;
		p.n_ranges = (uint32_t)pro.ranges.size();
		for (const GridScatterRange& r : pro.ranges) p.n_range_blocks += pro_range_blocks(r.n_elems);
		p.scratch = (unsigned long long*)pro.scratch;
		p.accumulate = pro.accumulate ? 1 : 0;
	}
	const AdamArgs a = make_adam_args(h, loss_scale, current_step);
	const uint32_t bulk_blocks = div_round_up((uint32_t)((n - p.bulk_begin) / 4), PRO_THREADS * (uint32_t)PRO_Q);
	const dim3 grid(p.n_reduce_blocks + p.n_range_blocks + bulk_blocks);
	if (steps16) hipLaunchKernelGGL(k_adam_prologue<uint16_t>, grid, dim3(PRO_THREADS), 0, stream, a, n, n_matrix, w_fp, (half_t*)w_half, (half_t*)g_half, m1, m2, (uint16_t*)steps, debias_table, p);
	else hipLaunchKernelGGL(k_adam_prologue<uint32_t>, grid, dim3(PRO_THREADS), 0, stream, a, n, n_matrix, w_fp, (half_t*)w_half, (half_t*)g_half, m1, m2, (uint32_t*)steps, debias_table, p);
	HIP_CHECK_THROW(hipGetLastError());
	return true;
}

void adam_fill_debias_table(hipStream_t stream, float beta1, float beta2, uint32_t from, uint32_t to, float* table) {
	if (to <= from) return;
	hipLaunchKernelGGL(k_adam_debias_table, dim3(blocks_for(to - from, 256)), dim3(256), 0, stream, beta1, beta2, from, to, table);
}

namespace {
template <typename G, typename W>
__global__ void __launch_bounds__(256) k_sgd(const size_t n, const float loss_scale, const float learning_rate, const float l2_reg, float* __restrict__ w_fp, W* __restrict__ w,
                                             const G* __restrict__ g) {
	const size_t i = (size_t)blockIdx.x * blockDim.x + threadIdx.x;
	if (i >= n) return;
	const float weight_fp = w_fp[i];
	float gradient = (float)g[i] / loss_scale;
	gradient += l2_reg * weight_fp;
	const float new_weight = weight_fp - learning_rate * gradient;
	w_fp[i] = new_weight;
	if constexpr (sizeof(W) == 2) w[i] = (W)new_weight;
}

template <typename W>
__global__ void __launch_bounds__(256) k_ema(const size_t n, const float decay, const float debias_old, const float debias_new, const W* __restrict__ weights, W* __restrict__ weights_ema,
                                             float* __restrict__ tmp) {
	const size_t i = (size_t)blockIdx.x * blockDim.x + threadIdx.x;
	if (i >= n) return;
	const float previous = tmp ? tmp[i] : (float)weights_ema[i];
	const float filtered = (previous * decay * debias_old + (float)weights[i] * (1 - decay)) * debias_new;
	if (tmp) tmp[i] = filtered;
	weights_ema[i] = (W)filtered;
}
template <typename W>
__global__ void __launch_bounds__(256) k_average_step(const size_t n, const uint32_t n_samples, const W* __restrict__ weights, W* __restrict__ current, W* __restrict__ average) {
	const size_t i = (size_t)blockIdx.x * blockDim.x + threadIdx.x;
	if (i >= n) return;
	const W weight = weights[i];
	average[i] = (W)((float)average[i] + ((float)weight - (float)current[i]) / (float)n_samples);
	current[i] = weight;
}
template <typename G>
__global__ void __launch_bounds__(256) k_batched_accumulate(const size_t n, const int first, const uint32_t multiplier, const G* __restrict__ gradients, float* __restrict__ pool) {
	const size_t i = (size_t)blockIdx.x * blockDim.x + threadIdx.x;
	if (i >= n) return;
	float v = first ? 0.0f : pool[i];
	v += (float)gradients[i] / (float)multiplier;
	pool[i] = v;
}
template <typename G>
__global__ void __launch_bounds__(1024) k_novo_second_moment(const size_t n, const float loss_scale, const float beta2, const G* __restrict__ gradients, float* __restrict__ moment) {
	__shared__ float part[1024];
	float acc = 0.0f;
	for (size_t i = threadIdx.x; i < n; i += 1024) {
		const float g = (float)gradients[i];
		acc += g * g;
	}
	part[threadIdx.x] = acc;
	__syncthreads();
	for (uint32_t stride = 512; stride > 0; stride >>= 1) {
		if (threadIdx.x < stride) part[threadIdx.x] += part[threadIdx.x + stride];
		__syncthreads();
	}
	if (threadIdx.x == 0) *moment = beta2 * *moment + (1 - beta2) * part[0] / loss_scale / loss_scale;
}
template <typename G, typename W>
__global__ void __launch_bounds__(256) k_novo_step(const size_t n, const float relative_weight_decay, const float absolute_weight_decay, const float loss_scale, const float learning_rate,
                                                   const float beta1, const float epsilon, float* __restrict__ weights_fp, W* __restrict__ weights, const G* __restrict__ gradients,
                                                   float* __restrict__ first_moments, const float* __restrict__ layer_second_moment) {
	const size_t i = (size_t)blockIdx.x * blockDim.x + threadIdx.x;
	if (i >= n) return;
	const float weight_fp = weights_fp[i];
	const float gradient = (float)gradients[i] / loss_scale;
	const float first_moment = beta1 * first_moments[i] + (1 - beta1) * gradient / (sqrtf(*layer_second_moment) + epsilon);
	first_moments[i] = first_moment;
	const float decayed_weight = (1 - relative_weight_decay * learning_rate) * weight_fp - copysignf(absolute_weight_decay * learning_rate, weight_fp);
	const float new_weight = decayed_weight - learning_rate * first_moment;
	weights_fp[i] = new_weight;
	if constexpr (sizeof(W) == 2) weights[i] = (W)new_weight;
}
template <typename W>
__global__ void __launch_bounds__(256) k_lookahead_step(const size_t n, const float alpha, float* __restrict__ weights_fp, W* __restrict__ weights, W* __restrict__ lookahead) {
	const size_t i = (size_t)blockIdx.x * blockDim.x + threadIdx.x;
	if (i >= n) return;
	const float new_weight = (float)lookahead[i] * (1.0f - alpha) + weights_fp[i] * alpha;
	weights_fp[i] = new_weight;
	const W h = (W)new_weight;
	lookahead[i] = h;
	if constexpr (sizeof(W) == 2) weights[i] = h;
}
}

namespace {
template <typename T>
__global__ void __launch_bounds__(256) k_copy_columns(const uint32_t n_elements, const uint32_t width, const T* __restrict__ src, const uint32_t src_stride, const uint32_t src_col,
                                                      T* __restrict__ dst, const uint32_t dst_stride, const uint32_t dst_col) {
	const uint32_t e = blockIdx.x * blockDim.x + threadIdx.x;
	if (e >= n_elements) return;
	const uint32_t i = e / width, j = e - i * width;
	dst[(size_t)i * dst_stride + dst_col + j] = src[(size_t)i * src_stride + src_col + j];
}
}

void copy_columns(hipStream_t stream, size_t elem_bytes, uint32_t n, const void* src, uint32_t src_stride, uint32_t src_col, void* dst, uint32_t dst_stride, uint32_t dst_col, uint32_t width) {
	const uint64_t total = (uint64_t)n * width;
	if (total == 0) return;
	CHECK_THROW(total < (1ull << 32) && (elem_bytes == 2 || elem_bytes == 4));
	const dim3 blocks((uint32_t)((total + 255) / 256));
	if (elem_bytes == 2) hipLaunchKernelGGL((k_copy_columns<uint16_t>), blocks, dim3(256), 0, stream, (uint32_t)total, width, (const uint16_t*)src, src_stride, src_col, (uint16_t*)dst, dst_stride, dst_col);
	else hipLaunchKernelGGL((k_copy_columns<uint32_t>), blocks, dim3(256), 0, stream, (uint32_t)total, width, (const uint32_t*)src, src_stride, src_col, (uint32_t*)dst, dst_stride, dst_col);
}

void sgd_step(hipStream_t stream, size_t n, float loss_scale, float learning_rate, float l2_reg, float* weights_full_precision, void* weights, const void* gradients, GradientPrecision precision, Precision weight_precision) {
	if (n == 0) return;
	if (weight_precision == Precision::Fp32) {
		CHECK_THROW(precision == GradientPrecision::Fp32);
		hipLaunchKernelGGL((k_sgd<float, float>), dim3(blocks_for(n, 256)), dim3(256), 0, stream, n, loss_scale, learning_rate, l2_reg, weights_full_precision, (float*)nullptr, (const float*)gradients);
	} else if (precision == GradientPrecision::Fp32) hipLaunchKernelGGL((k_sgd<float, half_t>), dim3(blocks_for(n, 256)), dim3(256), 0, stream, n, loss_scale, learning_rate, l2_reg, weights_full_precision, (half_t*)weights, (const float*)gradients);
	else hipLaunchKernelGGL((k_sgd<half_t, half_t>), dim3(blocks_for(n, 256)), dim3(256), 0, stream, n, loss_scale, learning_rate, l2_reg, weights_full_precision, (half_t*)weights, (const half_t*)gradients);
}

void average_step(hipStream_t stream, size_t n, uint32_t n_samples, const void* weights, void* current_sample, void* average, Precision weight_precision) {
	if (n == 0) return;
	if (weight_precision == Precision::Fp32) hipLaunchKernelGGL(k_average_step<float>, dim3(blocks_for(n, 256)), dim3(256), 0, stream, n, n_samples, (const float*)weights, (float*)current_sample, (float*)average);
	else hipLaunchKernelGGL(k_average_step<half_t>, dim3(blocks_for(n, 256)), dim3(256), 0, stream, n, n_samples, (const half_t*)weights, (half_t*)current_sample, (half_t*)average);
}
void batched_accumulate(hipStream_t stream, size_t n, bool first, uint32_t multiplier, const void* gradients, float* pool, GradientPrecision precision) {
	if (n == 0) return;
	if (precision == GradientPrecision::Fp32) hipLaunchKernelGGL(k_batched_accumulate<float>, dim3(blocks_for(n, 256)), dim3(256), 0, stream, n, first ? 1 : 0, multiplier, (const float*)gradients, pool);
	else hipLaunchKernelGGL(k_batched_accumulate<half_t>, dim3(blocks_for(n, 256)), dim3(256), 0, stream, n, first ? 1 : 0, multiplier, (const half_t*)gradients, pool);
}
void novograd_layer_step(hipStream_t stream, size_t n, float relative_decay, float absolute_decay, float loss_scale, float learning_rate, float beta1, float beta2, float epsilon,
                         float* weights_full_precision, void* weights, const void* gradients, float* first_moments, float* layer_second_moment, GradientPrecision precision, Precision weight_precision) {
	if (n == 0) return;
	if (weight_precision == Precision::Fp32) {
		CHECK_THROW(precision == GradientPrecision::Fp32);
		hipLaunchKernelGGL(k_novo_second_moment<float>, dim3(1), dim3(1024), 0, stream, n, loss_scale, beta2, (const float*)gradients, layer_second_moment);
		hipLaunchKernelGGL((k_novo_step<float, float>), dim3(blocks_for(n, 256)), dim3(256), 0, stream, n, relative_decay, absolute_decay, loss_scale, learning_rate, beta1, epsilon, weights_full_precision,
		                   (float*)nullptr, (const float*)gradients, first_moments, layer_second_moment);
		return;
	}
	if (precision == GradientPrecision::Fp32) {
		hipLaunchKernelGGL(k_novo_second_moment<float>, dim3(1), dim3(1024), 0, stream, n, loss_scale, beta2, (const float*)gradients, layer_second_moment);
		hipLaunchKernelGGL((k_novo_step<float, half_t>), dim3(blocks_for(n, 256)), dim3(256), 0, stream, n, relative_decay, absolute_decay, loss_scale, learning_rate, beta1, epsilon, weights_full_precision,
		                   (half_t*)weights, (const float*)gradients, first_moments, layer_second_moment);
		return;
	}
	hipLaunchKernelGGL(k_novo_second_moment<half_t>, dim3(1), dim3(1024), 0, stream, n, loss_scale, beta2, (const half_t*)gradients, layer_second_moment);
	hipLaunchKernelGGL((k_novo_step<half_t, half_t>), dim3(blocks_for(n, 256)), dim3(256), 0, stream, n, relative_decay, absolute_decay, loss_scale, learning_rate, beta1, epsilon, weights_full_precision,
	                   (half_t*)weights, (const half_t*)gradients, first_moments, layer_second_moment);
}
void lookahead_step(hipStream_t stream, size_t n, float alpha, float* weights_full_precision, void* weights, void* weights_lookahead, Precision weight_precision) {
	if (n == 0) return;
	if (weight_precision == Precision::Fp32) hipLaunchKernelGGL(k_lookahead_step<float>, dim3(blocks_for(n, 256)), dim3(256), 0, stream, n, alpha, weights_full_precision, (float*)nullptr, (float*)weights_lookahead);
	else hipLaunchKernelGGL(k_lookahead_step<half_t>, dim3(blocks_for(n, 256)), dim3(256), 0, stream, n, alpha, weights_full_precision, (half_t*)weights, (half_t*)weights_lookahead);
}

void ema_step(hipStream_t stream, size_t n, float decay, float debias_old, float debias_new, const void* weights, void* weights_ema, float* tmp, Precision weight_precision) {
	if (n == 0) return;
	if (weight_precision == Precision::Fp32) hipLaunchKernelGGL(k_ema<float>, dim3(blocks_for(n, 256)), dim3(256), 0, stream, n, decay, debias_old, debias_new, (const float*)weights, (float*)weights_ema, tmp);
	else hipLaunchKernelGGL(k_ema<half_t>, dim3(blocks_for(n, 256)), dim3(256), 0, stream, n, decay, debias_old, debias_new, (const half_t*)weights, (half_t*)weights_ema, tmp);
}

namespace {
void pcg32_advance_host(uint64_t* st, uint64_t delta) {
	const uint64_t MULT = 0x5851f42d4c957f2dULL;
	uint64_t cur_mult = MULT, cur_plus = st[1], acc_mult = 1u, acc_plus = 0u;
	while (delta > 0) {
		if (delta & 1) {
			acc_mult *= cur_mult;
			acc_plus = acc_plus * cur_mult + cur_plus;
		}
		cur_plus = (cur_mult + 1) * cur_plus;
		cur_mult *= cur_mult;
		delta /= 2;
	}
	st[0] = acc_mult * st[0] + acc_plus;
}
}

void generate_random_uniform(hipStream_t stream, uint64_t* state_inc_host, size_t n, float* out, float lower, float upper) {
	if (n > 0) {
		const size_t n_threads = (n + 3) / 4;
		const uint32_t blocks = blocks_for(n_threads, 128);
		hipLaunchKernelGGL(k_random_uniform, dim3(blocks), dim3(128), 0, stream, n, state_inc_host[0], state_inc_host[1], out, lower, upper);
	}
	pcg32_advance_host(state_inc_host, (uint64_t)n);
}

void cast_float_to_half(hipStream_t stream, size_t n, const float* in, void* out) {
	if (n == 0) return;
	hipLaunchKernelGGL(k_cast_f2h, dim3(blocks_for((n + 3) / 4, 256)), dim3(256), 0, stream, n, in, (half_t*)out);
}

void cast_half_to_float(hipStream_t stream, size_t n, const void* in, float* out) {
	if (n == 0) return;
	hipLaunchKernelGGL(k_cast_h2f, dim3(blocks_for((n + 3) / 4, 256)), dim3(256), 0, stream, n, (const half_t*)in, out);
}

void trim_and_cast(hipStream_t stream, bool fp32, uint32_t n, uint32_t in_stride, uint32_t dims, const void* in, MatViewMut out) {
	const uint64_t total = (uint64_t)n * dims;
	if (total == 0) return;
	CHECK_THROW(total < (1ull << 32));
	if (fp32) hipLaunchKernelGGL(k_trim_and_cast<float>, dim3(blocks_for(total, 256)), dim3(256), 0, stream, n, in_stride, dims, (const float*)in, out);
	else hipLaunchKernelGGL(k_trim_and_cast<half_t>, dim3(blocks_for(total, 256)), dim3(256), 0, stream, n, in_stride, dims, (const half_t*)in, out);
}

void fill_half(hipStream_t stream, size_t n, void* out, float value) {
	if (n == 0) return;
	hipLaunchKernelGGL(k_fill_half, dim3(blocks_for(n, 256)), dim3(256), 0, stream, n, (half_t*)out, (half_t)value);
}

}
```

tiny-cuda-nn_amd/csrc/k_mlp.hip:

```cpp
#include "mlp_device.h"
#include "mlp_side_jobs.h"
#include "adam_device.h"
#include "oneblob_device.h"

namespace tcnn_amd {
namespace {

__global__ void __launch_bounds__(256) k_mlp_prep(const MlpDesc d, const half_t* __restrict__ params, half_t* __restrict__ image, const uint32_t n_frags_total) {
	const uint32_t gid = blockIdx.x * blockDim.x + threadIdx.x;
	if (gid >= n_frags_total * 512) return;
	mlp_prep_element(d, params, image, gid);
}


#ifndef TCNN_MLP_FWD_PF
#define TCNN_MLP_FWD_PF 3
#endif
__device__ __host__ inline size_t hidden_tile_off(const uint32_t n, const uint32_t W, const uint32_t l, const uint32_t sample16, const uint32_t t) {
	return ((size_t)l * n + sample16) * W + (size_t)t * 256;
}

template <int W, int NB, int ACT, bool IMG_LDS = false, int THREADS = 256, bool OB = false>
__global__ void __launch_bounds__(THREADS) __attribute__((amdgpu_waves_per_eu((W >= 128 && !IMG_LDS) ? 3 : 1, 8))) k_mlp_fwd(const MlpDesc d, const FwdArgs a) {
	constexpr int T = W / 16;
// ... 283 lines not shown
						for (int b = 0; b < NB; ++b) acc[t][b] = mfma(af[i & 1], hf[s][b], acc[t][b]);
					}
				} else {
#pragma unroll
					for (int i = 0; i < KS * T; ++i) {
						const int s = i / T, t = i % T;
						const h8 af = frag_of(i);
#pragma unroll
						for (int b = 0; b < NB; ++b) acc[t][b] = mfma(af, hf[s][b], acc[t][b]);
					}
				}
			}
		}

		if (a.dL_dx) {
			const h8* img = a.image + (size_t)d.layers[0].bwd_off * 64 + lane;
			for (uint32_t ti = 0; ti < in_w / 16; ++ti) {
				f4 o[NB];
#pragma unroll
				for (int b = 0; b < NB; ++b) o[b] = f4{0, 0, 0, 0};
#pragma unroll
				for (int s = 0; s < KS; ++s) {
					const h8 af = img[(size_t)(ti * KS + s) * 64];
#pragma unroll
					for (int b = 0; b < NB; ++b) o[b] = mfma(af, hf[s][b], o[b]);
				}
#pragma unroll
				for (int b = 0; b < NB; ++b) {
					const h4 v = h4{(half_t)o[b][0], (half_t)o[b][1], (half_t)o[b][2], (half_t)o[b][3]};
					store_dx(a.dL_dx, a.dx_plane_f, a.n, in_w, s0 + 16 * b + c, 16 * ti + 4 * q, v);
				}
			}
		}
	}
}

struct WgPiece { size_t src; uint32_t row, col; };
__device__ inline WgPiece wg_piece(const uint32_t p, const uint32_t per_row, const size_t base_sample, const uint32_t ld, const bool tiled) {
	WgPiece r;
	if (!tiled) {
		r.row = p / per_row;
		r.col = (p - r.row * per_row) * 8;
		r.src = (base_sample + r.row) * ld + r.col;
	} else {
		const uint32_t half = p & 1u, c = (p >> 1) & 15u, rest = p >> 5, tiles = per_row / 2, st = rest / tiles, t = rest - st * tiles;
		r.row = st * 16 + c;
		r.col = t * 16 + half * 8;
		r.src = (base_sample + st * 16) * ld + (size_t)t * 256 + c * 16 + half * 8;
	}
	return r;
}

constexpr int WG_CHUNK = 64;
constexpr int WG_MAX_TILES = 16;
constexpr int WG_PAD = 16;

__global__ void __launch_bounds__(256) k_wgrad(
	const uint32_t n, const half_t* __restrict__ dO, const uint32_t ldo, const uint32_t R,
	const half_t* __restrict__ In, const uint32_t ldi, const uint32_t C, float* __restrict__ slabs, const uint32_t tiled
) {
	extern __shared__ __attribute__((aligned(16))) char smem[];
	const uint32_t rp = R + WG_PAD, cp = C + WG_PAD;
	half_t* P = (half_t*)smem;
	half_t* Q = P + (size_t)WG_CHUNK * rp;

	const uint32_t tid = threadIdx.x;
	const uint32_t lane = tid & 63, w = tid >> 6;
	const uint32_t grp = lane >> 4, li = lane & 15;
	const uint32_t TR = R / 16, TC = C / 16;
	const uint32_t n_tiles = TR * TC;
	const uint32_t per = (n_tiles + 3) / 4;
	const uint32_t tile0 = w * per;

	f4 acc[WG_MAX_TILES];
#pragma unroll
	for (int i = 0; i < WG_MAX_TILES; ++i) acc[i] = f4{0, 0, 0, 0};

	const uint32_t n_chunks = n / WG_CHUNK;
	for (uint32_t ch = blockIdx.x; ch < n_chunks; ch += gridDim.x) {
		const size_t base = (size_t)ch * WG_CHUNK;
		const uint32_t ppr = R / 8, pqr = C / 8;
		for (uint32_t p = tid; p < WG_CHUNK * ppr; p += 256) {
			const WgPiece w = wg_piece(p, ppr, base, ldo, (tiled & 1u) != 0);
			*(h8*)(P + (size_t)w.row * rp + w.col) = *(const h8*)(dO + w.src);
		}
		for (uint32_t p = tid; p < WG_CHUNK * pqr; p += 256) {
			const WgPiece w = wg_piece(p, pqr, base, ldi, (tiled & 2u) != 0);
			*(h8*)(Q + (size_t)w.row * cp + w.col) = *(const h8*)(In + w.src);
		}
		__syncthreads();

#pragma unroll
		for (int i = 0; i < WG_MAX_TILES; ++i) {
			const uint32_t tile = tile0 + i;
			if (i < (int)per && tile < n_tiles) {
				const uint32_t tr = tile / TC, tc = tile - tr * TC;
#pragma unroll
				for (int ks = 0; ks < WG_CHUNK / 32; ++ks) {
					const uint32_t row_lo = 32 * ks + 8 * grp + (li >> 2);
					const uint32_t colo = 4 * (li & 3);
					const h4 a_lo = lds_read_tr(P + (size_t)row_lo * rp + 16 * tr + colo);
					const h4 a_hi = lds_read_tr(P + (size_t)(row_lo + 4) * rp + 16 * tr + colo);
					const h4 b_lo = lds_read_tr(Q + (size_t)row_lo * cp + 16 * tc + colo);
					const h4 b_hi = lds_read_tr(Q + (size_t)(row_lo + 4) * cp + 16 * tc + colo);
					const h8 af = h8{a_lo[0], a_lo[1], a_lo[2], a_lo[3], a_hi[0], a_hi[1], a_hi[2], a_hi[3]};
					const h8 bf = h8{b_lo[0], b_lo[1], b_lo[2], b_lo[3], b_hi[0], b_hi[1], b_hi[2], b_hi[3]};
					acc[i] = mfma(af, bf, acc[i]);
				}
			}
		}
		__syncthreads();
	}

	float* slab = slabs + (size_t)blockIdx.x * R * C;
#pragma unroll
	for (int i = 0; i < WG_MAX_TILES; ++i) {
		const uint32_t tile = tile0 + i;
		if (i < (int)per && tile < n_tiles) {
			const uint32_t tr = tile / TC, tc = tile - tr * TC;
#pragma unroll
			for (int r = 0; r < 4; ++r) slab[(size_t)(16 * tr + 4 * grp + r) * C + 16 * tc + li] = acc[i][r];
		}
	}
}

constexpr uint32_t WG_MAX_JOBS = 8;
struct WgradJobs {
	const half_t* dO[WG_MAX_JOBS];
	const half_t* In[WG_MAX_JOBS];
	float* slabs[WG_MAX_JOBS];
	half_t* grad[WG_MAX_JOBS];
	uint32_t ldo[WG_MAX_JOBS], ldi[WG_MAX_JOBS], ldg[WG_MAX_JOBS];
	uint32_t tiled[WG_MAX_JOBS];
};

template <int TRW, int TC>
__global__ void __launch_bounds__(256) k_wgrad_rows(const uint32_t n, const WgradJobs jobs) {
	const half_t* __restrict__ dO = jobs.dO[blockIdx.y];
	const half_t* __restrict__ In = jobs.In[blockIdx.y];
	float* __restrict__ slabs = jobs.slabs[blockIdx.y];
	const uint32_t ldo = jobs.ldo[blockIdx.y], ldi = jobs.ldi[blockIdx.y];
	const bool p_tiled = (jobs.tiled[blockIdx.y] & 1u) != 0, q_tiled = (jobs.tiled[blockIdx.y] & 2u) != 0;
	constexpr uint32_t R = 4 * TRW * 16, C = TC * 16;
	constexpr uint32_t rp = R + WG_PAD, cp = C + WG_PAD;
	constexpr uint32_t ppr = R / 8, pqr = C / 8;
	constexpr uint32_t NP = WG_CHUNK * ppr / 256, NQ = WG_CHUNK * pqr / 256;
	static_assert(WG_CHUNK * ppr % 256 == 0 && WG_CHUNK * pqr % 256 == 0, "whole pieces per thread");
	extern __shared__ __attribute__((aligned(16))) char smem[];
	half_t* P = (half_t*)smem;
	half_t* Q = P + (size_t)WG_CHUNK * rp;

	const uint32_t tid = threadIdx.x;
	const uint32_t lane = tid & 63, w = tid >> 6;
	const uint32_t grp = lane >> 4, li = lane & 15;
	f4 acc[TRW][TC];
#pragma unroll
	for (int i = 0; i < TRW; ++i)
#pragma unroll
		for (int j = 0; j < TC; ++j) acc[i][j] = f4{0, 0, 0, 0};

	const uint32_t n_chunks = n / WG_CHUNK;
	h8 pv[NP], qv[NQ];
	auto fetch = [&](const uint32_t ch) {
		const size_t base = (size_t)min(ch, n_chunks - 1) * WG_CHUNK;
#pragma unroll
		for (uint32_t k = 0; k < NP; ++k) pv[k] = *(const h8*)(dO + wg_piece(tid + k * 256, ppr, base, ldo, p_tiled).src);
#pragma unroll
		for (uint32_t k = 0; k < NQ; ++k) qv[k] = *(const h8*)(In + wg_piece(tid + k * 256, pqr, base, ldi, q_tiled).src);
	};
	if (blockIdx.x < n_chunks) fetch(blockIdx.x);
	for (uint32_t ch = blockIdx.x; ch < n_chunks; ch += gridDim.x) {
#pragma unroll
		for (uint32_t k = 0; k < NP; ++k) {
			const WgPiece w = wg_piece(tid + k * 256, ppr, 0, ldo, p_tiled);
			*(h8*)(P + (size_t)w.row * rp + w.col) = pv[k];
		}
#pragma unroll
		for (uint32_t k = 0; k < NQ; ++k) {
			const WgPiece w = wg_piece(tid + k * 256, pqr, 0, ldi, q_tiled);
			*(h8*)(Q + (size_t)w.row * cp + w.col) = qv[k];
		}
		__syncthreads();
		fetch(ch + gridDim.x);
#pragma unroll
		for (int ks = 0; ks < WG_CHUNK / 32; ++ks) {
			const uint32_t row_lo = 32 * ks + 8 * grp + (li >> 2), colo = 4 * (li & 3);
			h8 af[TRW];
#pragma unroll
			for (int i = 0; i < TRW; ++i) {
				const uint32_t tr = w * TRW + i;
				const h4 lo = lds_read_tr(P + (size_t)row_lo * rp + 16 * tr + colo), hi = lds_read_tr(P + (size_t)(row_lo + 4) * rp + 16 * tr + colo);
				af[i] = h8{lo[0], lo[1], lo[2], lo[3], hi[0], hi[1], hi[2], hi[3]};
			}
#pragma unroll
			for (int tc = 0; tc < TC; ++tc) {
				const h4 lo = lds_read_tr(Q + (size_t)row_lo * cp + 16 * tc + colo), hi = lds_read_tr(Q + (size_t)(row_lo + 4) * cp + 16 * tc + colo);
				const h8 bf = h8{lo[0], lo[1], lo[2], lo[3], hi[0], hi[1], hi[2], hi[3]};
#pragma unroll
				for (int i = 0; i < TRW; ++i) acc[i][tc] = mfma(af[i], bf, acc[i][tc]);
			}
		}
		__syncthreads();
	}

	float* slab = slabs + (size_t)blockIdx.x * R * C;
#pragma unroll
	for (int i = 0; i < TRW; ++i)
#pragma unroll
		for (int tc = 0; tc < TC; ++tc)
#pragma unroll
			for (int r = 0; r < 4; ++r) slab[(size_t)(16 * (w * TRW + i) + 4 * grp + r) * C + 16 * tc + li] = acc[i][tc][r];
}

template <int TCW>
__global__ void __launch_bounds__(256) k_wgrad_cols(const uint32_t n, const WgradJobs jobs) {
	const half_t* __restrict__ dO = jobs.dO[blockIdx.y];
	const half_t* __restrict__ In = jobs.In[blockIdx.y];
	float* __restrict__ slabs = jobs.slabs[blockIdx.y];
	const uint32_t ldo = jobs.ldo[blockIdx.y], ldi = jobs.ldi[blockIdx.y];
	const bool p_tiled = (jobs.tiled[blockIdx.y] & 1u) != 0, q_tiled = (jobs.tiled[blockIdx.y] & 2u) != 0;
	constexpr uint32_t R = 16, C = 4 * TCW * 16;
	constexpr uint32_t rp = R + WG_PAD, cp = C + WG_PAD;
	constexpr uint32_t ppr = R / 8, pqr = C / 8;
	constexpr uint32_t NQ = WG_CHUNK * pqr / 256;
	static_assert(WG_CHUNK * ppr <= 256 && WG_CHUNK * pqr % 256 == 0, "one piece of dO per thread at most, whole pieces of In per thread");
	extern __shared__ __attribute__((aligned(16))) char smem[];
	half_t* P = (half_t*)smem;
	half_t* Q = P + (size_t)WG_CHUNK * rp;

	const uint32_t tid = threadIdx.x;
	const uint32_t lane = tid & 63, w = tid >> 6;
	const uint32_t grp = lane >> 4, li = lane & 15;
	f4 acc[TCW];
#pragma unroll
	for (int j = 0; j < TCW; ++j) acc[j] = f4{0, 0, 0, 0};

	const uint32_t n_chunks = n / WG_CHUNK;
	const bool has_p = tid < WG_CHUNK * ppr;
	const WgPiece pw = wg_piece(has_p ? tid : 0u, ppr, 0, ldo, p_tiled);
	h8 pv = h8{0, 0, 0, 0, 0, 0, 0, 0}, qv[NQ];
	auto fetch = [&](const uint32_t ch) {
		const size_t base = (size_t)min(ch, n_chunks - 1) * WG_CHUNK;
		if (has_p) pv = *(const h8*)(dO + base * ldo + pw.src);
#pragma unroll
		for (uint32_t k = 0; k < NQ; ++k) qv[k] = *(const h8*)(In + wg_piece(tid + k * 256, pqr, base, ldi, q_tiled).src);
	};
	if (blockIdx.x < n_chunks) fetch(blockIdx.x);
	for (uint32_t ch = blockIdx.x; ch < n_chunks; ch += gridDim.x) {
		if (has_p) *(h8*)(P + (size_t)pw.row * rp + pw.col) = pv;
#pragma unroll
		for (uint32_t k = 0; k < NQ; ++k) {
			const WgPiece w = wg_piece(tid + k * 256, pqr, 0, ldi, q_tiled);
			*(h8*)(Q + (size_t)w.row * cp + w.col) = qv[k];
		}
		__syncthreads();
		fetch(ch + gridDim.x);
#pragma unroll
		for (int ks = 0; ks < WG_CHUNK / 32; ++ks) {
			const uint32_t row_lo = 32 * ks + 8 * grp + (li >> 2), colo = 4 * (li & 3);
			const h4 alo = lds_read_tr(P + (size_t)row_lo * rp + colo), ahi = lds_read_tr(P + (size_t)(row_lo + 4) * rp + colo);
			const h8 af = h8{alo[0], alo[1], alo[2], alo[3], ahi[0], ahi[1], ahi[2], ahi[3]};
#pragma unroll
			for (int j = 0; j < TCW; ++j) {
				const uint32_t tc = w * TCW + j;
				const h4 lo = lds_read_tr(Q + (size_t)row_lo * cp + 16 * tc + colo), hi = lds_read_tr(Q + (size_t)(row_lo + 4) * cp + 16 * tc + colo);
				acc[j] = mfma(af, h8{lo[0], lo[1], lo[2], lo[3], hi[0], hi[1], hi[2], hi[3]}, acc[j]);
			}
		}
		__syncthreads();
	}
	float* slab = slabs + (size_t)blockIdx.x * R * C;
#pragma unroll
	for (int j = 0; j < TCW; ++j)
#pragma unroll
		for (int r = 0; r < 4; ++r) slab[(size_t)(4 * grp + r) * C + 16 * (w * TCW + j) + li] = acc[j][r];
}

constexpr int WR_ELEMS = SLAB_REDUCE_ELEMS, WR_GROUPS = SLAB_REDUCE_GROUPS;
__global__ void __launch_bounds__(WR_ELEMS * WR_GROUPS) k_wgrad_reduce(const uint32_t n_elems, const uint32_t cols, const uint32_t ldg, const uint32_t n_slabs, const float* __restrict__ slabs, half_t* __restrict__ grad, const int accumulate) {
	__shared__ float part[WR_GROUPS * WR_ELEMS];
	mlp_reduce_block(part, blockIdx.x, threadIdx.x, n_elems, cols, ldg, n_slabs, slabs, grad, accumulate);
}

__global__ void __launch_bounds__(WR_ELEMS * WR_GROUPS) k_wgrad_reduce_jobs(const uint32_t n_elems, const uint32_t cols, const uint32_t n_slabs, const WgradJobs jobs, const int accumulate) {
	__shared__ float part[WR_GROUPS * WR_ELEMS];
	mlp_reduce_block(part, blockIdx.x, threadIdx.x, n_elems, cols, jobs.ldg[blockIdx.y], n_slabs, jobs.slabs[blockIdx.y], jobs.grad[blockIdx.y], accumulate);
}

template <typename STEP_T>
__global__ void __launch_bounds__(WR_ELEMS * WR_GROUPS) k_wgrad_reduce_adam(const uint32_t n_elems, const uint32_t n_slabs, const float* __restrict__ slabs, half_t* __restrict__ grad,
                                                                            const AdamInReduce adam) {
	__shared__ float part[WR_GROUPS * WR_ELEMS];
	mlp_reduce_block(part, blockIdx.x, threadIdx.x, n_elems, n_elems, n_elems, n_slabs, slabs, grad, 0);
	const uint32_t e = threadIdx.x & (WR_ELEMS - 1), grp = threadIdx.x / WR_ELEMS;
	const uint32_t i = blockIdx.x * WR_ELEMS + e;
	if (grp != 0 || i >= n_elems) return;
	const half_t g = grad[i];
	float w_fp = adam.w_fp[i], m1 = adam.m1[i], m2 = adam.m2[i];
	STEP_T* steps = (STEP_T*)adam.steps;
	uint32_t step = steps[i];
	half_t w_h;
	bool updated;
	const float* __restrict__ table = adam.debias_table;
	adam_one(adam.args, [&](const uint32_t t) { return table[t]; }, table[adam.args.common_step], true, g, w_fp, w_h, m1, m2, step, updated);
	if (updated) {
		adam.w_fp[i] = w_fp;
		((half_t*)adam.w_half)[i] = w_h;
		adam.m1[i] = m1;
		adam.m2[i] = m2;
		steps[i] = (STEP_T)step;
		if (adam.image) {
			const uint4 where = *(const uint4*)(adam.image_inv + (size_t)IMAGE_INV_WIDTH * i);
			half_t* image = (half_t*)adam.image;
			if (where.x != 0xffffffffu) image[where.x] = w_h;
			if (where.y != 0xffffffffu) image[where.y] = w_h;
			if (where.z != 0xffffffffu) image[where.z] = w_h;
			if (where.w != 0xffffffffu) image[where.w] = w_h;
		}
	}
}

inline uint32_t wgrad_grid(uint32_t n) {
	const uint32_t n_chunks = n / WG_CHUNK;
	return n_chunks < 256 ? (n_chunks ? n_chunks : 1) : 256;
}

template <int W, int NB>
void launch_fwd_oneblob(hipStream_t stream, const MlpDesc& d, const FwdArgs& a, uint32_t grid) {
	if (d.activation == (uint32_t)Activation::ReLU) hipLaunchKernelGGL((k_mlp_fwd<W, NB, (int)Activation::ReLU, false, 256, true>), dim3(grid), dim3(256), 0, stream, d, a);
	else hipLaunchKernelGGL((k_mlp_fwd<W, NB, -1, false, 256, true>), dim3(grid), dim3(256), 0, stream, d, a);
}

template <int W, int NB>
void launch_fwd_act(hipStream_t stream, const MlpDesc& d, const FwdArgs& a, uint32_t grid) {
	if (d.activation == (uint32_t)Activation::ReLU) hipLaunchKernelGGL((k_mlp_fwd<W, NB, (int)Activation::ReLU>), dim3(grid), dim3(256), 0, stream, d, a);
	else if (d.activation == (uint32_t)Activation::None) hipLaunchKernelGGL((k_mlp_fwd<W, NB, (int)Activation::None>), dim3(grid), dim3(256), 0, stream, d, a);
	else hipLaunchKernelGGL((k_mlp_fwd<W, NB, -1>), dim3(grid), dim3(256), 0, stream, d, a);
}

template <int W, int NB>
void launch_bwd_act(hipStream_t stream, const MlpDesc& d, const BwdArgs& a, uint32_t grid) {
	if (d.activation == (uint32_t)Activation::ReLU) hipLaunchKernelGGL((k_mlp_bwd<W, NB, (int)Activation::ReLU>), dim3(grid), dim3(256), 0, stream, d, a);
	else if (d.activation == (uint32_t)Activation::None) hipLaunchKernelGGL((k_mlp_bwd<W, NB, (int)Activation::None>), dim3(grid), dim3(256), 0, stream, d, a);
	else hipLaunchKernelGGL((k_mlp_bwd<W, NB, -1>), dim3(grid), dim3(256), 0, stream, d, a);
}

constexpr int nb_for_width(int W) { return W >= 256 ? 1 : (W >= 128 ? 2 : 4); }

inline uint32_t mlp_grid(uint32_t n, int nb) {
	const uint32_t n_iters = n / (16 * nb);
	const uint32_t wgs = div_round_up(n_iters, 4);
	const uint32_t cap = 256 * 8;
	return wgs < cap ? (wgs ? wgs : 1) : cap;
}

}

size_t mlp_image_bytes(const MlpDesc& d) { return (size_t)(d.n_frags_fwd + d.n_frags_bwd + d.n_frags_r32) * 1024; }

void mlp_prepare_weights(hipStream_t stream, const MlpDesc& d, const void* params, void* image, bool want_bwd) {
	const uint32_t n_frags = d.n_frags_fwd + (want_bwd ? d.n_frags_bwd + d.n_frags_r32 : 0);
	const uint32_t total = n_frags * 512;
	hipLaunchKernelGGL(k_mlp_prep, dim3(div_round_up(total, 256)), dim3(256), 0, stream, d, (const half_t*)params, (half_t*)image, n_frags);
}

void mlp_forward(hipStream_t stream, const MlpDesc& d, const void* image, uint32_t n, const void* x, void* out, void* hidden) {
	MlpIo io{};
	io.x_half = x;
	io.out_half = out;
	mlp_forward_io(stream, d, image, n, io, hidden);
}

void mlp_forward_io(hipStream_t stream, const MlpDesc& d, const void* image, uint32_t n, const MlpIo& io, void* hidden) {
	CHECK_THROW(n % BATCH_SIZE_GRANULARITY == 0);
	CHECK_THROW(d.n_hidden >= 1);
	CHECK_THROW(io.x_half != nullptr || io.x_f32.data != nullptr);
	CHECK_THROW(io.out_half != nullptr || io.out_f32.data != nullptr);
	if (n == 0) return;
	FwdArgs a{(const half_t*)io.x_half, (half_t*)io.out_half, (half_t*)hidden, (const h8*)image, n, io.x_plane_features,
	          io.x_f32, io.x_f32_dims, io.x_scale, io.x_offset, 0u, io.out_f32, io.out_f32_dims};
	if (io.x_oneblob_bins) {
		CHECK_THROW(io.x_f32.data != nullptr && io.x_oneblob_bins >= 32 && (io.x_oneblob_bins & (io.x_oneblob_bins - 1)) == 0);
		while ((1u << a.oneblob_log2) < io.x_oneblob_bins) ++a.oneblob_log2;
	}
	const bool small = n / 64 < 4 * 256;
	if (a.oneblob_log2) {
		if (d.width == 64 && small) return launch_fwd_oneblob<64, 1>(stream, d, a, mlp_grid(n, 1));
		if (d.width == 64) return launch_fwd_oneblob<64, nb_for_width(64)>(stream, d, a, mlp_grid(n, nb_for_width(64)));
		if (d.width == 128) return launch_fwd_oneblob<128, nb_for_width(128)>(stream, d, a, mlp_grid(n, nb_for_width(128)));
		throw std::runtime_error{"mlp_forward_io: the fused OneBlob input needs a 64- or 128-wide network"};
	}
	if (d.width == 64 && small && hidden == nullptr) return launch_fwd_act<64, 1>(stream, d, a, mlp_grid(n, 1));
	const uint32_t image_bytes = d.n_frags_fwd * 1024;
	if (d.width == 128 && hidden == nullptr && image_bytes <= 150 * 1024 && n >= 256 * 8 * 64 && switches().mlp_fwd_lds) {
		constexpr int NB = 4, THREADS = 512;
		const uint32_t grid = std::min<uint32_t>(256, div_round_up(n / (16 * NB), THREADS / 64));
		auto go = [&](auto kernel) {
			HIP_CHECK_THROW(hipFuncSetAttribute((const void*)kernel, hipFuncAttributeMaxDynamicSharedMemorySize, (int)image_bytes));
			hipLaunchKernelGGL(kernel, dim3(grid), dim3(THREADS), image_bytes, stream, d, a);
			HIP_CHECK_THROW(hipGetLastError());
		};
		if (d.activation == (uint32_t)Activation::ReLU) go(k_mlp_fwd<128, NB, (int)Activation::ReLU, true, THREADS>);
		else go(k_mlp_fwd<128, NB, -1, true, THREADS>);
		return;
	}
	switch (d.width) {
		case 16: return launch_fwd_act<16, nb_for_width(16)>(stream, d, a, mlp_grid(n, nb_for_width(16)));
		case 32: return launch_fwd_act<32, nb_for_width(32)>(stream, d, a, mlp_grid(n, nb_for_width(32)));
		case 64: return launch_fwd_act<64, nb_for_width(64)>(stream, d, a, mlp_grid(n, nb_for_width(64)));
		case 128: return launch_fwd_act<128, nb_for_width(128)>(stream, d, a, mlp_grid(n, nb_for_width(128)));
		case 256: return launch_fwd_act<256, nb_for_width(256)>(stream, d, a, mlp_grid(n, nb_for_width(256)));
		default: throw std::runtime_error{"FullyFusedMLP only supports 16, 32, 64, and 128 neurons."};
	}
}

void mlp_backward(hipStream_t stream, const MlpDesc& d, const void* image, uint32_t n, const void* dL_dout, const void* out, const void* hidden, void* dhidden, void* dL_dx,
                  uint32_t dx_plane_features) {
	CHECK_THROW(n % BATCH_SIZE_GRANULARITY == 0);
	CHECK_THROW(d.n_hidden >= 1);
	if (n == 0) return;
	BwdArgs a{(const half_t*)dL_dout, (const half_t*)out, (const half_t*)hidden, (half_t*)dhidden, (half_t*)dL_dx,
	          (const h8*)((const char*)image + (size_t)d.n_frags_fwd * 1024), n, dx_plane_features};
	switch (d.width) {
		case 16: return launch_bwd_act<16, nb_for_width(16)>(stream, d, a, mlp_grid(n, nb_for_width(16)));
		case 32: return launch_bwd_act<32, nb_for_width(32)>(stream, d, a, mlp_grid(n, nb_for_width(32)));
		case 64: return launch_bwd_act<64, nb_for_width(64)>(stream, d, a, mlp_grid(n, nb_for_width(64)));
		case 128: return launch_bwd_act<128, nb_for_width(128)>(stream, d, a, mlp_grid(n, nb_for_width(128)));
		case 256: return launch_bwd_act<256, nb_for_width(256)>(stream, d, a, mlp_grid(n, nb_for_width(256)));
		default: throw std::runtime_error{"FullyFusedMLP only supports 16, 32, 64, and 128 neurons."};
	}
}

void mlp_reduce_slabs(hipStream_t stream, uint32_t n_params, uint32_t n_slabs, const float* slabs, void* grad_half, bool accumulate, const AdamInReduce* adam) {
	if (n_params == 0) return;
	const dim3 grid(div_round_up(n_params, (uint32_t)WR_ELEMS)), block(WR_ELEMS * WR_GROUPS);
	if (adam && !accumulate) {
		if (adam->steps16) hipLaunchKernelGGL(k_wgrad_reduce_adam<uint16_t>, grid, block, 0, stream, n_params, n_slabs, slabs, (half_t*)grad_half, *adam);
		else hipLaunchKernelGGL(k_wgrad_reduce_adam<uint32_t>, grid, block, 0, stream, n_params, n_slabs, slabs, (half_t*)grad_half, *adam);
	} else {
		hipLaunchKernelGGL(k_wgrad_reduce, grid, block, 0, stream, n_params, n_params, n_params, n_slabs, slabs, (half_t*)grad_half, accumulate ? 1 : 0);
	}
	HIP_CHECK_THROW(hipGetLastError());
}

size_t wgrad_workspace_floats(uint32_t rows, uint32_t cols, uint32_t n) { return (size_t)wgrad_grid(n) * rows * cols; }

static bool wgrad_fast_shape(const Switches& sw, uint32_t rows, uint32_t cols) {
	return sw.wgrad_rows && ((rows == 128 || rows == 64) && (cols == 128 || cols == 64 || cols == 32) || (rows == 16 && (cols == 128 || cols == 64)));
}

static void launch_wgrad_jobs(hipStream_t stream, uint32_t n, uint32_t rows, uint32_t cols, const WgradJobs& jobs, uint32_t n_jobs, bool accumulate) {
	const uint32_t grid = wgrad_grid(n);
	const size_t shmem = (size_t)WG_CHUNK * ((rows + WG_PAD) + (cols + WG_PAD)) * sizeof(half_t);
	const dim3 g(grid, n_jobs), b(256);
#define TCNN_WGRAD_ROWS(TRW, TC) hipLaunchKernelGGL((k_wgrad_rows<TRW, TC>), g, b, shmem, stream, n, jobs)
	if (rows == 128 && cols == 128) TCNN_WGRAD_ROWS(2, 8);
	else if (rows == 128 && cols == 64) TCNN_WGRAD_ROWS(2, 4);
	else if (rows == 128 && cols == 32) TCNN_WGRAD_ROWS(2, 2);
	else if (rows == 64 && cols == 128) TCNN_WGRAD_ROWS(1, 8);
	else if (rows == 64 && cols == 64) TCNN_WGRAD_ROWS(1, 4);
	else if (rows == 64 && cols == 32) TCNN_WGRAD_ROWS(1, 2);
	else if (rows == 16 && cols == 128) hipLaunchKernelGGL((k_wgrad_cols<2>), g, b, shmem, stream, n, jobs);
	else if (rows == 16 && cols == 64) hipLaunchKernelGGL((k_wgrad_cols<1>), g, b, shmem, stream, n, jobs);
	else throw std::runtime_error{"launch_wgrad_jobs: no kernel for this shape"};
#undef TCNN_WGRAD_ROWS
	const uint32_t n_elems = rows * cols;
	hipLaunchKernelGGL(k_wgrad_reduce_jobs, dim3(div_round_up(n_elems, (uint32_t)WR_ELEMS), n_jobs), dim3(WR_ELEMS * WR_GROUPS), 0, stream, n_elems, cols, grid, jobs, accumulate ? 1 : 0);
	HIP_CHECK_THROW(hipGetLastError());
}

void mlp_wgrad(hipStream_t stream, uint32_t n, const void* dO, uint32_t ldo, uint32_t rows, const void* In, uint32_t ldi, uint32_t cols,
               void* grad_half, uint32_t ldg, bool accumulate, float* workspace) {
	const WgradPanel p{dO, ldo, rows, In, ldi, cols, grad_half, ldg, false, false};
	mlp_wgrad_panels(stream, Precision::Fp16, n, &p, 1, accumulate, workspace);
}

size_t wgrad_panels_workspace_floats(Precision precision, const WgradPanel* panels, uint32_t count, uint32_t n) {
	if (precision == Precision::Fp32) return wgrad_panels_workspace_floats_f32(panels, count, n);
	size_t total = 0;
	for (uint32_t i = 0; i < count; ++i) total += wgrad_workspace_floats(panels[i].rows, panels[i].cols, n);
	return total;
}

void mlp_wgrad_panels(hipStream_t stream, Precision precision, uint32_t n, const WgradPanel* panels, uint32_t count, bool accumulate, float* workspace) {
	if (precision == Precision::Fp32) return mlp_wgrad_panels_f32(stream, n, panels, count, accumulate, workspace);
	CHECK_THROW(n % WG_CHUNK == 0);
	const Switches sw = switches();
	std::vector<bool> done(count, false);
	std::vector<float*> slabs(count);
	size_t at = 0;
	for (uint32_t i = 0; i < count; ++i) {
		slabs[i] = workspace + at;
		at += wgrad_workspace_floats(panels[i].rows, panels[i].cols, n);
	}
	for (uint32_t i = 0; i < count; ++i) {
		if (done[i]) continue;
		const WgradPanel& p = panels[i];
		CHECK_THROW(p.rows % 16 == 0 && p.cols % 16 == 0);
		CHECK_THROW((p.rows / 16) * (p.cols / 16) <= 4 * WG_MAX_TILES);
		if (wgrad_fast_shape(sw, p.rows, p.cols)) {
			WgradJobs jobs{};
			uint32_t n_jobs = 0;
			for (uint32_t j = i; j < count && n_jobs < WG_MAX_JOBS; ++j) {
				if (done[j] || panels[j].rows != p.rows || panels[j].cols != p.cols) continue;
				jobs.dO[n_jobs] = (const half_t*)panels[j].dO;
				jobs.In[n_jobs] = (const half_t*)panels[j].In;
				jobs.slabs[n_jobs] = slabs[j];
				jobs.grad[n_jobs] = (half_t*)panels[j].grad;
				jobs.ldo[n_jobs] = panels[j].ldo;
				jobs.ldi[n_jobs] = panels[j].ldi;
				jobs.ldg[n_jobs] = panels[j].ldg;
				jobs.tiled[n_jobs] = (panels[j].dO_tiled ? 1u : 0u) | (panels[j].In_tiled ? 2u : 0u);
				done[j] = true;
				++n_jobs;
			}
			launch_wgrad_jobs(stream, n, p.rows, p.cols, jobs, n_jobs, accumulate);
			continue;
		}
		const uint32_t grid = wgrad_grid(n);
		const size_t shmem = (size_t)WG_CHUNK * ((p.rows + WG_PAD) + (p.cols + WG_PAD)) * sizeof(half_t);
		hipLaunchKernelGGL(k_wgrad, dim3(grid), dim3(256), shmem, stream, n, (const half_t*)p.dO, p.ldo, p.rows, (const half_t*)p.In, p.ldi, p.cols, slabs[i], (p.dO_tiled ? 1u : 0u) | (p.In_tiled ? 2u : 0u));
		const uint32_t n_elems = p.rows * p.cols;
		hipLaunchKernelGGL(k_wgrad_reduce, dim3(div_round_up(n_elems, (uint32_t)WR_ELEMS)), dim3(WR_ELEMS * WR_GROUPS), 0, stream, n_elems, p.cols, p.ldg, grid, slabs[i], (half_t*)p.grad, accumulate ? 1 : 0);
		done[i] = true;
	}
}

}
```

tiny-cuda-nn_amd/csrc/tcnn_common.h:

```cpp
#pragma once

#include <hip/hip_runtime.h>

#include <cstddef>
#include <cstdint>
#include <cstdlib>
#include <stdexcept>
#include <string>
#include <vector>

namespace tcnn_amd {

enum class Activation : uint32_t { None = 0, ReLU = 1, LeakyReLU = 2, Exponential = 3, Sine = 4, Sigmoid = 5, Squareplus = 6, Softplus = 7, Tanh = 8 };
enum class GridType : uint32_t { Hash = 0, Dense = 1, Tiled = 2 };
enum class HashType : uint32_t { Prime = 0, CoherentPrime = 1, ReversedPrime = 2, Rng = 3 };
enum class InterpolationType : uint32_t { Nearest = 0, Linear = 1, Smoothstep = 2 };
enum class LossType : uint32_t { L2 = 0, RelativeL2 = 1, L1 = 2, RelativeL1 = 3, Mape = 4, Smape = 5, CrossEntropy = 6, Variance = 7, RelativeL2Luminance = 8 };
enum class Precision : uint32_t { Fp32 = 0, Fp16 = 1 };
enum class GradientPrecision : uint32_t { Fp32 = 0, Fp16 = 1 };
enum class GradientMode : uint32_t { Ignore = 0, Overwrite = 1, Accumulate = 2 };

constexpr uint32_t BATCH_SIZE_GRANULARITY = 256;
constexpr float LOSS_SCALE_FP16 = 128.0f;
constexpr uint32_t MAX_N_LEVELS = 128;
// ... 245 lines not shown
	uint32_t plane_features = 0, record_planes = 0;
	GridGradientKernel kernel = GridGradientKernel::None;
	bool binned = false, tune = false, prologue = false;
	bool stochastic = false;
	bool tail = false;
	GridListTail list_tail;
	size_t tail_bytes = 0;
};
inline GridBackwardRoute grid_backward_route(const GridFacts& g, const Switches& sw, const GridForwardRoute& fwd, bool lists_current, uint32_t n, GridDyForm offer, bool want_dL_dx,
                                             GradientMode mode, GridMaxLevel max_level, bool x_contiguous) {
	const GridMeta& meta = *g.meta;
	const uint32_t F = meta.n_features_per_level;
	GridBackwardRoute r;
	if (mode == GradientMode::Ignore) return r;
	r.stochastic = grid_stochastic_gradients(g);
	if (!(fwd.planned ? fwd.lds : grid_lds_gradients(g, sw, n))) {
		r.kernel = (!g.fp32 && F == 1) ? GridGradientKernel::AtomicScratch32 : GridGradientKernel::Atomic;
		return r;
	}
	const bool lists = fwd.recorded == GridRecorded::HitLists && lists_current && !r.stochastic;
	r.kernel = lists ? GridGradientKernel::Lists : GridGradientKernel::BitPlanes;
	r.binned = !lists && g.any_binned;
	r.tune = !lists && sw.scatter_tune;
	r.prologue = max_level != GridMaxLevel::Scalar && !g.any_binned;
	if (offer == GridDyForm::Rows || want_dL_dx) return r;
	r.dy = GridDyForm::Planes, r.plane_features = F;
	if (offer == GridDyForm::Records && !r.stochastic && fwd.recorded != GridRecorded::HitLists && g.n_to_pad == 0 && max_level != GridMaxLevel::PerSample && sw.scatter_records && !g.any_binned &&
	    grid_scatter_records_supported(meta) && x_contiguous) {
		r.dy = GridDyForm::Records, r.record_planes = grid_scatter_record_planes(meta);
		return r;
	}
	r.tail = offer == GridDyForm::Records && lists && F == 2 && max_level == GridMaxLevel::None && sw.listgrad_in_mlp && meta.n_levels <= 16 &&
	         (grid_hit_item_samples(meta) << (meta.n_pos_dims - 1)) <= 2048;
	if (r.tail) {
		r.list_tail.n_levels = meta.n_levels;
		for (uint32_t l = 0; l < meta.n_levels; ++l) {
			const GridLevel& lv = meta.levels[l];
			if (lv.scatter_n_chunks > 1 && lv.scatter_n_chunks <= GRID_FILTER_MAX_CHUNKS && !lv.scatter_binned) r.list_tail.level_mask |= 1u << l;
		}
	}
	return r;
}

void ppng1_forward(hipStream_t stream, bool fp32_out, uint32_t n, uint32_t F, uint32_t Q, uint32_t C, uint32_t R, int32_t log2_min_freq, int32_t log2_max_freq, MatView x,
                   const void* features, void* out, uint32_t out_stride);
void ppng1_backward(hipStream_t stream, bool fp32_dy, uint32_t n, uint32_t F, uint32_t Q, uint32_t C, uint32_t R, int32_t log2_min_freq, int32_t log2_max_freq, MatView x,
                    const void* features, const void* dL_dy, uint32_t dy_stride, uint64_t* scratch, void* grad, bool accumulate);

void ppng2_forward(hipStream_t stream, bool fp32_out, uint32_t n, uint32_t F, uint32_t Q, uint32_t C, uint32_t R, int32_t log2_min_freq, int32_t log2_max_freq, MatView x,
                   const void* features, void* out, uint32_t out_stride);
void ppng2_backward(hipStream_t stream, bool fp32_dy, uint32_t n, uint32_t F, uint32_t Q, uint32_t C, uint32_t R, int32_t log2_min_freq, int32_t log2_max_freq, MatView x,
                    const void* features, const void* dL_dy, uint32_t dy_stride, uint64_t* scratch, void* grad, bool accumulate);
void ppng3_forward(hipStream_t stream, bool fp32_out, uint32_t n, uint32_t F, uint32_t Q, uint32_t C, int32_t log2_min_freq, int32_t log2_max_freq, MatView x, const void* features, void* out,
                   uint32_t out_stride);
size_t ppng3_backward_workspace_bytes(uint32_t n, uint32_t F, uint32_t Q, uint32_t C);
void ppng3_backward(hipStream_t stream, bool fp32_dy, uint32_t n, uint32_t F, uint32_t Q, uint32_t C, int32_t log2_min_freq, int32_t log2_max_freq, MatView x, const void* dL_dy,
                    uint32_t dy_stride, void* workspace, uint64_t* scratch, void* grad, bool accumulate);
void ppng3_backward_input(hipStream_t stream, bool fp32_dy, uint32_t n, uint32_t F, uint32_t Q, uint32_t C, int32_t log2_min_freq, int32_t log2_max_freq, MatView x, const void* features,
                          const void* dL_dy, uint32_t dy_stride, MatViewMut dL_dx);
void ppng3_backward_backward_input(hipStream_t stream, bool fp32_dy, uint32_t n, uint32_t F, uint32_t Q, uint32_t C, int32_t log2_min_freq, int32_t log2_max_freq, MatView x, MatView dL_ddLdx,
                                   const void* features, const void* dL_dy, uint32_t dy_stride, uint64_t* scratch, void* grad, bool accumulate, void* dL_ddLdy, MatViewMut* dL_dx);

bool grid_bin_supported(const GridMeta& meta);
uint32_t grid_bin_max_chunks();
uint32_t grid_bin_acc_bytes();
size_t grid_bin_workspace_bytes(const GridMeta& meta, uint32_t n);
void grid_backward_binned(hipStream_t stream, const GridMeta& meta, const GridMeta* dev_meta, uint32_t n, MatView x, const void* dL_dy, uint32_t dy_stride_sample,
                          uint32_t dy_stride_level, void* grad, bool accumulate, void* workspace,
                          uint32_t* fallback_count = nullptr,
                          bool stochastic = false);
void grid_backward_input(hipStream_t stream, const GridMeta& meta, bool fp32, uint32_t n, const void* dL_dy, uint32_t dy_stride, const float* dy_dx, MatViewMut dL_dx);
void grid_backward_backward_input(hipStream_t stream, const GridMeta& meta, const GridMeta* dev_meta, bool fp32, bool fp32_grad, uint32_t n, MatView x, MatView dL_ddLdx, const void* dL_dy,
                                  uint32_t dy_stride, const void* grid, const float* dy_dx, void* grad, void* dL_ddLdy, MatViewMut* dL_dx);

void oneblob_forward(hipStream_t stream, bool fp32, uint32_t n, uint32_t n_dims, uint32_t n_bins, MatView x, void* out, uint32_t out_stride);
void oneblob_backward_input(hipStream_t stream, bool fp32, uint32_t n, uint32_t n_dims, uint32_t n_bins, MatView x, const void* dL_dy, uint32_t dy_stride, MatViewMut dL_dx);
void oneblob_tangent(hipStream_t stream, bool fp32, uint32_t n, uint32_t n_dims, uint32_t n_bins, MatView x, MatView v, void* t, uint32_t t_stride);
void identity_forward(hipStream_t stream, bool fp32, uint32_t n, uint32_t n_dims, float scale, float offset, MatView x, void* out, uint32_t out_stride);
void identity_backward_input(hipStream_t stream, bool fp32, uint32_t n, uint32_t n_dims, float scale, const void* dL_dy, uint32_t dy_stride, MatViewMut dL_dx);
void identity_backward_backward_input(hipStream_t stream, bool fp32, uint32_t n, uint32_t n_dims, float scale, MatView dL_ddLdx, void* dL_ddLdy, uint32_t dy_stride);
void periodic_forward(hipStream_t stream, bool triangle, bool fp32, uint32_t n, uint32_t n_dims, uint32_t n_frequencies, MatView x, void* out, uint32_t out_stride, float* dy_dx);
void periodic_backward_input(hipStream_t stream, bool fp32, uint32_t n, uint32_t n_dims, uint32_t outputs_per_input, const void* dL_dy, uint32_t dy_stride, const float* dy_dx, MatViewMut dL_dx);
void periodic_backward_backward_input(hipStream_t stream, bool triangle, bool fp32, uint32_t n, uint32_t n_dims, uint32_t n_frequencies, MatView x, MatView dL_ddLdx, const void* dL_dy,
                                       void* dL_ddLdy, uint32_t dy_stride, MatViewMut* dL_dx);
void composite_reduce_forward(hipStream_t stream, bool fp32, bool product, size_t n_elems, uint32_t n_nested, const void* in, void* out);
void composite_reduce_backward(hipStream_t stream, bool fp32, bool product, size_t n_elems, uint32_t n_nested, const void* in, const void* dL_dout, void* dL_din);
void composite_reduce_backward_backward(hipStream_t stream, bool fp32, size_t n_elems, uint32_t n_nested, const void* in, const void* tangents, const void* dL_dout, void* dL_ddLdout, void* q);
void sh_forward(hipStream_t stream, bool fp32, uint32_t n, uint32_t degree, MatView x, void* out, uint32_t out_stride);
void sh_backward_input(hipStream_t stream, bool fp32, uint32_t n, uint32_t degree, MatView x, const void* dL_dy, uint32_t dy_stride, MatViewMut dL_dx);
void sh_backward_backward_input(hipStream_t stream, bool fp32, uint32_t n, uint32_t degree, MatView x, MatView dL_ddLdx, const void* dL_dy, void* dL_ddLdy, uint32_t dy_stride, MatViewMut* dL_dx);

struct MlpLayer {
	uint32_t rows, cols;
	uint32_t w_off;
	uint32_t fwd_off;
	uint32_t bwd_off;
	uint32_t ks_fwd;
	uint32_t ks_bwd;
	uint32_t natural_k;
};

struct MlpDesc {
	uint32_t in_width, width, out_width, n_hidden, n_layers;
	uint32_t activation, output_activation;
	uint32_t n_frags_fwd, n_frags_bwd;
	uint32_t n_frags_r32;
	MlpLayer layers[MAX_MLP_LAYERS];
};

size_t mlp_image_bytes(const MlpDesc& d);
void mlp_prepare_weights(hipStream_t stream, const MlpDesc& d, const void* params, void* image, bool want_bwd);
void mlp_forward(hipStream_t stream, const MlpDesc& d, const void* image, uint32_t n, const void* x, void* out, void* hidden);
struct MlpIo {
	const void* x_half;
	uint32_t x_plane_features;
	MatView x_f32;
	uint32_t x_f32_dims;
	float x_scale, x_offset;
	uint32_t x_oneblob_bins;
	void* out_half;
	MatViewMut out_f32;
	uint32_t out_f32_dims;
};
void mlp_forward_io(hipStream_t stream, const MlpDesc& d, const void* image, uint32_t n, const MlpIo& io, void* hidden);
void mlp_backward(hipStream_t stream, const MlpDesc& d, const void* image, uint32_t n, const void* dL_dout, const void* out, const void* hidden, void* dhidden, void* dL_dx,
                  uint32_t dx_plane_features);
constexpr uint32_t MLP_INPUT_GRAD_MAX_HIDDEN = 4;
struct MlpInputGradPlan {
	bool fused = false;
	char name[48] = "two-pass";
	uint32_t nb = 0, grid = 0;
	bool relu = false;
};
MlpInputGradPlan mlp_input_gradient_plan(const MlpDesc& d, bool layerwise, uint32_t n);
void mlp_input_gradient(hipStream_t stream, const MlpDesc& d, const MlpInputGradPlan& plan, const void* image, uint32_t n, const MlpIo& io, uint32_t dim, float backprop_scale,
                        void* dL_dx, uint32_t dx_plane_features);
constexpr uint32_t MLP_INPUT_JACOBIAN_MAX_DIMS = 16;
MlpInputGradPlan mlp_input_jacobian_plan(const MlpDesc& d, bool layerwise, uint32_t n, uint32_t n_dims);
void mlp_input_jacobian(hipStream_t stream, const MlpDesc& d, const MlpInputGradPlan& plan, const void* image, uint32_t n, const MlpIo& io, const uint32_t* dims, uint32_t n_dims,
                        float backprop_scale, void* dL_dx, uint32_t dx_plane_features);
constexpr uint32_t MLP_INPUT_JVP_MAX_TT = 3;
struct MlpInputJvpPlan {
	bool fused = false;
	char name[48] = "two-pass";
	uint32_t nb = 0, grid = 0;
	uint32_t tt = 0;
	bool relu = false;
};
MlpInputJvpPlan mlp_input_jvp_plan(const MlpDesc& d, bool layerwise, uint32_t n, uint32_t n_tangents);
void mlp_input_jvp(hipStream_t stream, const MlpDesc& d, const MlpInputJvpPlan& plan, const void* image, uint32_t n, const MlpIo& io, const void* tangents, MatView tangents_f32,
                   uint32_t n_tangents, void* jvp, uint32_t jvp_stride);
struct MlpInputJvpBackwardPlan {
	bool fused = false;
	char name[48] = "two-pass";
	uint32_t nb = 0, grid = 0;
	uint32_t tt = 0;
	bool relu = false;
};
inline MlpInputJvpBackwardPlan mlp_input_jvp_backward_plan(const MlpDesc& d, bool layerwise, uint32_t n, uint32_t n_tangents) {
	(void)d; (void)layerwise; (void)n; (void)n_tangents;
	return MlpInputJvpBackwardPlan{};
}
void input_gradient_one_hot(hipStream_t stream, Precision precision, uint32_t n, uint32_t width, uint32_t dim, float backprop_scale, void* d_doutput);
void input_gradient_rescale(hipStream_t stream, uint32_t n, uint32_t dims, float mult, MatViewMut d_dinput);
struct MlpTrainRequest {
	uint32_t n = 0;
	uint32_t x_plane_features = 0, oneblob_bins = 0, oneblob_dims = 0;
	uint32_t dims = 0;
	LossType loss = LossType::L2;
	bool external_dL_dy = false;
	bool data_pdf = false;
	bool out = false;
	bool dL_dx = false;
	uint32_t dx_plane_features = 0, dx_record_dims = 0;
	bool gradients = false;
	bool compact_context = false;
};
enum class MlpTrainKernel : uint32_t { None, R32ob, R32w, R32, R32a, Regs, Train };
struct MlpTrainPlan {
	bool ok = false;
	MlpTrainKernel kernel = MlpTrainKernel::None;
	const char* name = "";
	uint32_t grid = 0;
	MlpTrainRequest request;
	struct Config { int nb, nw, maxt; uint32_t lds_bytes, s; bool ok, image_in_lds, regw; } config{};
	int regs_in_tiles = 0, regs_hidden = 0;
	bool regs_fast = false;
	bool r32ob_shared = false;
};
MlpTrainPlan mlp_train_plan(const MlpDesc& d, const MlpTrainRequest& request);
struct MlpTrainArgs {
	const void* image = nullptr;
	const void* x = nullptr;
	MatView oneblob_x{};
	const float *target = nullptr, *data_pdf = nullptr;
	const void* external_dL_dy = nullptr;
	float loss_scale = 1.0f;
	void *out = nullptr, *dL_dout = nullptr, *dL_dx = nullptr;
	float *L = nullptr, *slabs = nullptr;
	const float* dx_record_x = nullptr;
	uint32_t n_params = 0;
	const GridListTail* list_tail = nullptr;
};
bool mlp_train_item_map(const MlpTrainPlan& plan, GridItemMap& map);
void mlp_train_launch(hipStream_t stream, const MlpDesc& d, const MlpTrainPlan& plan, const MlpTrainArgs& args);
bool mlp_train_any_kernel(const MlpDesc& d, uint32_t n);
bool mlp_train_oneblob_in_kernel(const MlpDesc& d, uint32_t n, uint32_t n_bins);
bool mlp_train_compact_context(const MlpDesc& d, uint32_t n);
void mlp_expand_context(hipStream_t stream, uint32_t n, uint32_t dims, const void* compact_dL_dout, const float* compact_L, void* dL_dout, float* L);
struct AdamInReduce;
void mlp_reduce_slabs(hipStream_t stream, uint32_t n_params, uint32_t n_slabs, const float* slabs, void* grad_half, bool accumulate, const AdamInReduce* adam = nullptr);
size_t wgrad_workspace_floats(uint32_t rows, uint32_t cols, uint32_t n);
struct WgradPanel { const void* dO; uint32_t ldo, rows; const void* In; uint32_t ldi, cols; void* grad; uint32_t ldg; bool dO_tiled, In_tiled; };
size_t wgrad_panels_workspace_floats(Precision precision, const WgradPanel* panels, uint32_t count, uint32_t n);
void mlp_wgrad_panels(hipStream_t stream, Precision precision, uint32_t n, const WgradPanel* panels, uint32_t count, bool accumulate, float* workspace);
void mlp_wgrad(hipStream_t stream, uint32_t n, const void* dO, uint32_t ldo, uint32_t rows, const void* In, uint32_t ldi, uint32_t cols,
               void* grad_half, uint32_t ldg, bool accumulate, float* workspace);
void mlp_layer_forward(hipStream_t stream, Precision precision, uint32_t n, const void* x, uint32_t ldx, const void* w, uint32_t rows, uint32_t cols, uint32_t activation, void* y,
                       uint32_t ldy, void* pre);
void mlp_layer_backward(hipStream_t stream, Precision precision, uint32_t n, const void* dL_dout, uint32_t ldo, const void* wt, uint32_t rows, uint32_t cols, uint32_t activation,
                        const void* aux, void* dL_din, uint32_t ldi);
void mlp_layer_transpose(hipStream_t stream, Precision precision, uint32_t rows, uint32_t cols, const void* w, void* wt);
void mlp_layer_tangent(hipStream_t stream, Precision precision, uint32_t n, const void* u_in, uint32_t ldu, const void* w, uint32_t rows, uint32_t cols, uint32_t activation,
                       const void* aux, const void* g, void* u_out, void* r_out, uint32_t ldy);
void mlp_layer_backward_keep(hipStream_t stream, Precision precision, uint32_t n, const void* d_out, uint32_t ldo, const void* wt, uint32_t rows, uint32_t cols, uint32_t activation,
                             const void* aux, void* g_in, void* d_in, uint32_t ldi);
void mlp_layer_curvature_backward(hipStream_t stream, Precision precision, uint32_t n, const void* p_out, uint32_t ldo, const void* wt, uint32_t rows, uint32_t cols,
                                  uint32_t activation, const void* aux, const void* r_in, void* p_in, uint32_t ldi);
void mlp_layer_delta(hipStream_t stream, Precision precision, size_t n_elems, uint32_t activation, const void* g, const void* aux, void* delta);
void mlp_activation_backward_output(hipStream_t stream, Precision precision, size_t n_elems, uint32_t activation, const void* dL_dout, const void* out, void* result);
void add_input_gradient(hipStream_t stream, uint32_t n, uint32_t dims, MatView src, MatViewMut dst);

void loss_evaluate(hipStream_t stream, LossType type, uint32_t n, uint32_t stride, uint32_t dims, float loss_scale,
                   const void* pred_half, const float* target, float* values, void* grads_half, const float* data_pdf, Precision precision = Precision::Fp16);
void reduce_sum(hipStream_t stream, size_t n, const float* values, float* partials, float* result_dev);
void reduce_partials(hipStream_t stream, uint32_t n_partials, const float* partials, float* result_dev);

constexpr uint32_t LOSS_EVAL_MAX_BLOCKS = 1024;
struct LossEvalRequest {
	LossType type = LossType::L2;
	Precision precision = Precision::Fp16;
	uint32_t n = 0, dims = 0;
	float loss_scale = 1.0f;
	const float* scale_dev = nullptr;
	const void* prediction = nullptr;
	uint32_t prediction_stride = 0;
	const float* target = nullptr;
	const float* data_pdf = nullptr;
	float* values = nullptr;
	uint32_t values_stride = 0;
	void* gradients = nullptr;
	uint32_t gradients_stride = 0;
	float* loss_sum = nullptr;
	float* partials = nullptr;
};
void loss_eval_launch(hipStream_t stream, const LossEvalRequest& r);

struct AdamHyper {
	float learning_rate = 1e-3f, beta1 = 0.9f, beta2 = 0.999f, epsilon = 1e-8f, l2_reg = 1e-8f;
	float relative_decay = 0.0f, absolute_decay = 0.0f, clipping_magnitude = 0.0f, non_matrix_learning_rate_factor = 1.0f;
	bool adabound = false, optimize_matrix_params = true, optimize_non_matrix_params = true;
};
struct AdamArgs {
	float relative_weight_decay, absolute_weight_decay, weight_clipping_magnitude, loss_scale, learning_rate, non_matrix_learning_rate_factor;
	float beta1, beta2, epsilon, lower_lr_bound, upper_lr_bound, l2_reg;
	uint32_t optimize_matrix_params, optimize_non_matrix_params;
	float inv_loss_scale;
	uint32_t inv_loss_scale_exact;
	uint32_t common_step;
};
AdamArgs make_adam_args(const AdamHyper& h, float loss_scale, uint32_t current_step);
constexpr uint32_t IMAGE_INV_WIDTH = 4;
struct AdamInReduce {
	AdamArgs args;
	float* w_fp = nullptr;
	void* w_half = nullptr;
	float* m1 = nullptr;
	float* m2 = nullptr;
	void* steps = nullptr;
	uint32_t steps16 = 0;
	const float* debias_table = nullptr;
	void* image = nullptr;
	const uint32_t* image_inv = nullptr;
};
struct AdamPrologue {
	bool pending = false;
	const GridScatterRange* dev_ranges = nullptr;
	std::vector<GridScatterRange> ranges;
	uint64_t* scratch = nullptr;
	void* grad_base = nullptr;
	bool accumulate = false;
	bool has_reduce = false;
	uint32_t reduce_elems = 0, reduce_slabs = 0;
	const float* slabs = nullptr;
	int reduce_accumulate = 0;
};
bool adam_step_with_prologue(hipStream_t stream, const AdamHyper& h, size_t n, size_t n_matrix, float loss_scale, uint32_t current_step,
                             float* w_fp, void* w_half, void* g_half, float* m1, float* m2, void* steps, bool steps16, const float* debias_table, const AdamPrologue& p);
void adam_step(hipStream_t stream, const AdamHyper& h, size_t n, size_t n_matrix, float loss_scale, uint32_t current_step,
               float* w_fp, void* w_half, const void* gradients, float* m1, float* m2, void* steps, bool steps16, const float* debias_table,
               GradientPrecision precision = GradientPrecision::Fp16, Precision weight_precision = Precision::Fp16);
void adam_widen_steps(hipStream_t stream, size_t n, const void* steps16, void* steps32);
void adam_fill_debias_table(hipStream_t stream, float beta1, float beta2, uint32_t from, uint32_t to, float* table);
void copy_columns(hipStream_t stream, size_t elem_bytes, uint32_t n, const void* src, uint32_t src_stride, uint32_t src_col, void* dst, uint32_t dst_stride, uint32_t dst_col, uint32_t width);
void sgd_step(hipStream_t stream, size_t n, float loss_scale, float learning_rate, float l2_reg, float* weights_full_precision, void* weights, const void* gradients,
              GradientPrecision precision = GradientPrecision::Fp16, Precision weight_precision = Precision::Fp16);
void ema_step(hipStream_t stream, size_t n, float decay, float debias_old, float debias_new, const void* weights, void* weights_ema, float* tmp, Precision weight_precision = Precision::Fp16);
void average_step(hipStream_t stream, size_t n, uint32_t n_samples, const void* weights, void* current_sample, void* average, Precision weight_precision = Precision::Fp16);
void batched_accumulate(hipStream_t stream, size_t n, bool first, uint32_t multiplier, const void* gradients, float* pool, GradientPrecision precision = GradientPrecision::Fp16);
void lookahead_step(hipStream_t stream, size_t n, float alpha, float* weights_full_precision, void* weights, void* weights_lookahead, Precision weight_precision = Precision::Fp16);
void novograd_layer_step(hipStream_t stream, size_t n, float relative_decay, float absolute_decay, float loss_scale, float learning_rate, float beta1, float beta2, float epsilon,
                         float* weights_full_precision, void* weights, const void* gradients, float* first_moments, float* layer_second_moment,
                         GradientPrecision precision = GradientPrecision::Fp16, Precision weight_precision = Precision::Fp16);

void generate_random_uniform(hipStream_t stream, uint64_t* state_inc_host, size_t n, float* out, float lower, float upper);
void cast_float_to_half(hipStream_t stream, size_t n, const float* in, void* out);
void cast_half_to_float(hipStream_t stream, size_t n, const void* in, float* out);
void trim_and_cast(hipStream_t stream, bool fp32, uint32_t n, uint32_t in_stride, uint32_t dims, const void* in, MatViewMut out);
void fill_half(hipStream_t stream, size_t n, void* out, float value);
void grid_zero_levels(hipStream_t stream, size_t elem_bytes, uint32_t n, uint32_t n_levels, uint32_t level0, uint32_t width, uint64_t sample_stride, uint64_t level_stride,
                      void* data, const void* src, const float* per_sample, uint32_t n_grid_features, uint32_t F, bool gradient_rule);

}
```

tiny-cuda-nn_amd/tinycudann/_C.py:

```python
import ctypes as C
import json
import os

_PKG = os.path.dirname(os.path.dirname(os.path.abspath(__file__)))
LIB_PATH = os.path.join(_PKG, "libtcnn_amd.so")
if os.environ.get("TCNN_AMD_LIB"):
    LIB_PATH = os.path.abspath(os.environ["TCNN_AMD_LIB"])

if not os.path.exists(LIB_PATH):
    raise ImportError(
        f"{LIB_PATH} not found: the HIP extension has not been built. Run `python tiny-cuda-nn_amd/build.py` "
        "(or __graft_entry__.build()). There is no CPU fallback."
    )

import torch

lib = C.CDLL(LIB_PATH)

_hip = None


def hip_runtime():
    global _hip
    if _hip is None:
        cand = os.path.join(os.path.dirname(torch.__file__), "lib", "libamdhip64.so")
        _hip = C.CDLL(cand if os.path.exists(cand) else "libamdhip64.so")
        _hip.hipMemcpy.restype = C.c_int
        _hip.hipMemcpy.argtypes = [C.c_void_p, C.c_void_p, C.c_size_t, C.c_int]
    return _hip


def memcpy_dtod(dst_ptr, src_ptr, n_bytes):
    err = hip_runtime().hipMemcpy(dst_ptr, src_ptr, n_bytes, 3)
    if err != 0:
        raise RuntimeError(f"hipMemcpy failed with error {err}")

_vp, _u32, _u64, _f32, _sz, _int, _cp = C.c_void_p, C.c_uint32, C.c_uint64, C.c_float, C.c_size_t, C.c_int, C.c_char_p
_pp = C.POINTER(C.c_void_p)

_SIGNATURES = {
    "tcnn_last_error": (_cp, []),
    "tcnn_version": (_cp, []),
    "tcnn_batch_size_granularity": (_u32, []),
    "tcnn_device": (_int, [C.POINTER(C.c_int)]),
    "tcnn_set_device": (_int, [_int]),
    "tcnn_free_temporary_memory": (None, []),
    "tcnn_has_networks": (_int, []),
    "tcnn_default_loss_scale": (_f32, [_int]),
    "tcnn_preferred_precision": (_int, []),
    "tcnn_set_log_callback": (None, [_vp, _vp]),
    "tcnn_gpu_malloc": (_int, [_sz, _pp]),
    "tcnn_gpu_free": (_int, [_vp]),
    "tcnn_gpu_memcpy": (_int, [_vp, _vp, _sz, _int]),
    "tcnn_gpu_memset": (_int, [_vp, _int, _sz]),
    "tcnn_stream_synchronize": (_int, [_vp]),
    "tcnn_generate_random_uniform": (_int, [_vp, _vp, _sz, _vp, C.c_float, C.c_float]),
    "tcnn_create_network_with_input_encoding": (_int, [_u32, _u32, _cp, _cp, _pp]),
    "tcnn_create_network": (_int, [_u32, _u32, _cp, _pp]),
    "tcnn_create_encoding": (_int, [_u32, _cp, _int, _pp]),
    "tcnn_create_network_with_input_encoding_precision": (_int, [_u32, _u32, _cp, _cp, _int, _pp]),
    "tcnn_create_network_precision": (_int, [_u32, _u32, _cp, _int, _pp]),
    "tcnn_module_destroy": (None, [_vp]),
    "tcnn_module_inference": (_int, [_vp, _vp, _u32, _vp, _vp, _vp]),
    "tcnn_module_forward": (_int, [_vp, _vp, _u32, _vp, _vp, _vp, _int, _pp]),
    "tcnn_module_backward": (_int, [_vp, _vp, _vp, _u32, _vp, _vp, _vp, _vp, _vp, _vp]),
    "tcnn_module_backward_backward_input": (_int, [_vp, _vp, _vp, _u32, _vp, _vp, _vp, _vp, _vp, _vp, _vp]),
    "tcnn_module_backward_backward_input_mode": (_int, [_vp, _vp, _vp, _u32, _vp, _vp, _vp, _vp, _vp, _vp, _vp, _int]),
    "tcnn_module_input_gradient": (_int, [_vp, _vp, _u32, _u32, _vp, _vp, _vp, _vp, _f32]),
    "tcnn_module_last_input_gradient_route": (_cp, [_vp]),
    "tcnn_trainer_input_gradient": (_int, [_vp, _vp, _u32, _u32, _vp, _vp, _f32]),
    "tcnn_module_input_jacobian": (_int, [_vp, _vp, _u32, _vp, _u32, _vp, _vp, _vp, _vp, _f32]),
    "tcnn_module_last_input_jacobian_route": (_cp, [_vp]),
    "tcnn_trainer_input_jacobian": (_int, [_vp, _vp, _u32, _vp, _u32, _vp, _vp, _f32]),
    "tcnn_module_input_jvp": (_int, [_vp, _vp, _u32, _u32, _vp, _vp, _vp, _vp, _vp]),
    "tcnn_module_last_input_jvp_route": (_cp, [_vp]),
    "tcnn_trainer_input_jvp": (_int, [_vp, _vp, _u32, _u32, _vp, _vp, _vp]),
    "tcnn_module_input_jvp_forward": (_int, [_vp, _vp, _u32, _u32, _vp, _vp, _vp, _vp, _vp, _vp]),
    "tcnn_module_input_jvp_backward": (_int, [_vp, _vp, _vp, _u32, _u32, _vp, _vp, _vp, _vp, _vp, _vp, _vp, _vp, _int]),
    "tcnn_module_last_input_jvp_backward_route": (_cp, [_vp]),
    "tcnn_trainer_input_jvp_forward": (_int, [_vp, _vp, _u32, _u32, _vp, _vp, _vp, _vp, _vp]),
    "tcnn_trainer_input_jvp_backward": (_int, [_vp, _vp, _vp, _u32, _u32, _vp, _vp, _vp, _vp, _vp, _vp, _int]),
    "tcnn_context_destroy": (None, [_vp]),
    "tcnn_module_n_input_dims": (_u32, [_vp]),
    "tcnn_module_n_output_dims": (_u32, [_vp]),
    "tcnn_module_n_params": (_sz, [_vp]),
    "tcnn_module_list_scatters": (_sz, [_vp]),
    "tcnn_module_set_max_level": (_int, [_vp, _f32]),
    "tcnn_module_max_level": (_f32, [_vp]),
    "tcnn_module_set_max_level_gpu": (_int, [_vp, _vp]),
    "tcnn_module_param_precision": (_int, [_vp]),
    "tcnn_module_output_precision": (_int, [_vp]),
    "tcnn_module_initialize_params": (_int, [_vp, _u64, _vp, _f32]),
    "tcnn_module_hyperparams": (_cp, [_vp]),
    "tcnn_module_name": (_cp, [_vp]),
    "tcnn_create_from_config": (_int, [_u32, _u32, _cp, _pp]),
    "tcnn_create_from_config_seeded": (_int, [_u32, _u32, _cp, _u32, _pp]),
    "tcnn_create_from_config_precision": (_int, [_u32, _u32, _cp, _u32, _int, _pp]),
    "tcnn_trainer_precision": (_int, [_vp]),
    "tcnn_trainer_destroy": (None, [_vp]),
    "tcnn_trainer_training_step": (_int, [_vp, _vp, _u32, _vp, _int, _vp, _vp, _int, _vp, _int, _int, _vp, _pp]),
    "tcnn_trainer_loss": (_int, [_vp, _vp, _vp, C.POINTER(C.c_float)]),
    "tcnn_trainer_forward": (_int, [_vp, _vp, _f32, _u32, _vp, _int, _vp, _vp, _int, _int, _vp, _pp]),
    "tcnn_trainer_backward": (_int, [_vp, _vp, _vp, _u32, _vp, _int, _vp, _int, _int]),
    "tcnn_trainer_optimizer_step": (_int, [_vp, _vp, _f32]),
    "tcnn_train_ctx_destroy": (None, [_vp]),
    "tcnn_train_ctx_output": (_vp, [_vp]),
    "tcnn_train_ctx_dL_doutput": (_vp, [_vp]),
    "tcnn_train_ctx_L": (_vp, [_vp]),
    "tcnn_trainer_inference": (_int, [_vp, _vp, _u32, _vp, _int, _vp, _int, _int]),
    "tcnn_trainer_inference_mixed_precision": (_int, [_vp, _vp, _u32, _vp, _int, _vp, _int]),
    "tcnn_trainer_n_params": (_sz, [_vp]),
    "tcnn_trainer_padded_output_width": (_u32, [_vp]),
    "tcnn_trainer_params_full_precision": (_vp, [_vp]),
    "tcnn_trainer_params": (_vp, [_vp]),
    "tcnn_trainer_params_inference": (_vp, [_vp]),
    "tcnn_trainer_param_gradients": (_vp, [_vp]),
    "tcnn_trainer_set_params_full_precision": (_int, [_vp, _vp, _sz, _int]),
    "tcnn_trainer_set_params": (_int, [_vp, _vp, _sz, _int]),
    "tcnn_trainer_initialize_params": (_int, [_vp]),
    "tcnn_trainer_update_hyperparams": (_int, [_vp, _cp]),
    "tcnn_trainer_hyperparams": (_cp, [_vp]),
    "tcnn_trainer_network_hyperparams": (_cp, [_vp]),
    "tcnn_trainer_optimizer_step_count": (_u32, [_vp]),
    "tcnn_trainer_params_updated_in_flush": (C.c_size_t, [_vp]),
    "tcnn_trainer_image_preps": (C.c_size_t, [_vp]),
    "tcnn_trainer_scatter_wide_fallbacks": (C.c_size_t, [_vp]),
    "tcnn_trainer_optimizer_prologue_steps": (C.c_size_t, [_vp]),
    "tcnn_trainer_list_scatters": (C.c_size_t, [_vp]),
    "tcnn_trainer_list_gradient_tails": (C.c_size_t, [_vp]),
    "tcnn_trainer_last_step_kernel": (_cp, [_vp]),
    "tcnn_trainer_set_max_level": (_int, [_vp, _f32]),
    "tcnn_trainer_set_max_level_gpu": (_int, [_vp, _vp]),
    "tcnn_trainer_max_level": (_f32, [_vp]),
    "tcnn_train_ctx_keeps_weight_gradient_slabs": (C.c_int, [_vp, _vp]),
    "tcnn_trainer_profile_next_step": (_int, [_vp]),
    "tcnn_trainer_profile_collect": (_int, [_vp, _vp, C.POINTER(C.c_float), C.POINTER(_u32)]),
    "tcnn_trainer_serialize": (_int, [_vp, _int, _pp, C.POINTER(_sz)]),
    "tcnn_trainer_deserialize": (_int, [_vp, _vp, _sz]),
    "tcnn_module_layer_sizes": (_int, [_vp, C.POINTER(_u32), _sz, C.POINTER(_sz)]),
    "tcnn_optimizer_create": (_int, [_cp, _sz, C.POINTER(_u32), _sz, _pp]),
    "tcnn_optimizer_create_precision": (_int, [_cp, _sz, C.POINTER(_u32), _sz, _int, _pp]),
    "tcnn_optimizer_weight_precision": (_int, [_vp]),
    "tcnn_optimizer_destroy": (None, [_vp]),
    "tcnn_optimizer_step": (_int, [_vp, _vp, _f32, _vp, _vp, _vp, _int]),
    "tcnn_optimizer_step_count": (_u32, [_vp]),
    "tcnn_optimizer_n_params": (_sz, [_vp]),
    "tcnn_optimizer_learning_rate": (_f32, [_vp]),
    "tcnn_optimizer_set_learning_rate": (_int, [_vp, _f32]),
    "tcnn_optimizer_update_hyperparams": (_int, [_vp, _cp]),
    "tcnn_optimizer_hyperparams": (_cp, [_vp]),
    "tcnn_optimizer_custom_weights": (_vp, [_vp]),
    "tcnn_optimizer_weights_restored": (_int, [_vp, _vp, _vp]),
    "tcnn_optimizer_serialize": (_int, [_vp, _pp, C.POINTER(_sz)]),
    "tcnn_optimizer_deserialize": (_int, [_vp, _vp, _sz]),
    "tcnn_loss_type": (_int, [_cp, C.POINTER(C.c_int)]),
    "tcnn_loss_name": (_cp, [_int]),
    "tcnn_loss_evaluate": (_int, [_int, _vp, _f32, _vp, _u32, _u32, _vp, _u32, _int, _vp, _vp, _vp, _u32, _vp, _u32, _vp]),
}

for _name, (_res, _args) in _SIGNATURES.items():
    _fn = getattr(lib, _name)
    _fn.restype = _res
    _fn.argtypes = _args


class Precision:
    Fp32 = 0
    Fp16 = 1


class LogSeverity:
    Info, Debug, Warning, Error, Success = range(5)


def check(status):
    if status != 0:
        raise RuntimeError(lib.tcnn_last_error().decode("utf-8", "replace"))


def to_json_bytes(obj):
    if obj is None:
        return b"{}"
    if isinstance(obj, (bytes, bytearray)):
        return bytes(obj)
    if isinstance(obj, str):
        return obj.encode()
    return json.dumps(obj).encode()


def batch_size_granularity():
    return int(lib.tcnn_batch_size_granularity())


def default_loss_scale(precision):
    return float(lib.tcnn_default_loss_scale(int(precision)))


def preferred_precision():
    return int(lib.tcnn_preferred_precision())


def has_networks():
    return bool(lib.tcnn_has_networks())


def free_temporary_memory():
    lib.tcnn_free_temporary_memory()
```

Measured before the change: 1.395 billion.

## Use range-guarded fast sqrt/div in Adam and specialize plain-args kernels

Replaces IEEE sqrtf and division in the Adam update with rsq/rcp hardware approximations refined by Newton steps. These are guarded by exponent-range checks, and a four-lane joint test picks the fast path when all operands are in range. Adds a PLAIN template specialization that skips the loss-scale division and weight clipping, and loads per-element debias values directly from the table instead of using a lambda. Also adds a sweep API that checks bit-exactness of the fast math against the reference. This aims to cut ALU cost in the optimizer kernel, at the price of more code and a reliance on the refinement staying bit-exact.

```diff
diff --git a/include/tcnn_amd.h b/include/tcnn_amd.h
--- a/include/tcnn_amd.h
+++ b/include/tcnn_amd.h
@@ -186,6 +186,11 @@
 int         tcnn_optimizer_weights_restored(tcnn_optimizer_t o, tcnn_stream_t stream, const void* params_half);
 int         tcnn_optimizer_serialize(tcnn_optimizer_t o, const void** out_bytes, size_t* out_size);
 int         tcnn_optimizer_deserialize(tcnn_optimizer_t o, const void* bytes, size_t size);
+#define TCNN_ADAM_SWEEP_SQRT 0
+#define TCNN_ADAM_SWEEP_DIV_GRID 1
+#define TCNN_ADAM_SWEEP_DIV_PAIRS 2
+int         tcnn_adam_math_sweep(tcnn_stream_t stream, int what, uint64_t first, uint64_t count, uint32_t n_numerators, float numerator_lo, float numerator_hi, uint64_t seed,
+                                 uint64_t* mismatches, uint64_t* first_bad);
 
 
 int         tcnn_loss_type(const char* loss_json, int* type_out);
diff --git a/tiny-cuda-nn_amd/csrc/adam_device.h b/tiny-cuda-nn_amd/csrc/adam_device.h
--- a/tiny-cuda-nn_amd/csrc/adam_device.h
+++ b/tiny-cuda-nn_amd/csrc/adam_device.h
@@ -3,32 +3,101 @@
 
 namespace tcnn_amd {
 
-template <typename DebiasOf, typename G, typename W>
-__device__ inline void adam_one(const AdamArgs& a, DebiasOf&& debias_of, const float common_debias, const bool is_matrix, const G g_in, float& w_fp, W& w_h,
-                                float& m1, float& m2, uint32_t& step, bool& updated) {
+constexpr uint32_t ADAM_SQRT_LO = (127u - 96u) << 23, ADAM_SQRT_SPAN = 128u << 23;
+constexpr uint32_t ADAM_DIV_N_LO = (127u - 64u) << 23, ADAM_DIV_N_SPAN = 128u << 23;
+constexpr uint32_t ADAM_DIV_D_LO = (127u - 48u) << 23, ADAM_DIV_D_SPAN = 66u << 23;
+__device__ inline uint32_t adam_sqrt_excess(const float x) { return __float_as_uint(x) - ADAM_SQRT_LO; }
+__device__ inline uint32_t adam_div_n_excess(const float n) { return __float_as_uint(n) - ADAM_DIV_N_LO; }
+__device__ inline bool adam_div_d_in_range(const float d) { return __float_as_uint(d) - ADAM_DIV_D_LO < ADAM_DIV_D_SPAN; }
+
+__device__ inline float adam_sqrt_fast(const float x) {
+	const float y = __builtin_amdgcn_rsqf(x);
+	const float s = x * y, h = 0.5f * y;
+	return fmaf(fmaf(-s, s, x), h, s);
+}
+__device__ inline float adam_div_fast(const float n, const float d) {
+	float r = __builtin_amdgcn_rcpf(d);
+	r = fmaf(fmaf(-d, r, 1.0f), r, r);
+	float q = n * r;
+	q = fmaf(fmaf(-d, q, n), r, q);
+	return fmaf(fmaf(-d, q, n), r, q);
+}
+__device__ inline float adam_sqrt(const float x) { return adam_sqrt_excess(x) < ADAM_SQRT_SPAN ? adam_sqrt_fast(x) : sqrtf(x); }
+__device__ inline float adam_div(const float n, const float d) { return adam_div_n_excess(n) < ADAM_DIV_N_SPAN && adam_div_d_in_range(d) ? adam_div_fast(n, d) : n / d; }
+
+__device__ inline bool adam_epsilon_in_range(const AdamArgs& a) { return a.epsilon >= 0.0f && a.epsilon <= 65536.0f; }
+
+struct AdamLane {
+	float weight_fp, first_moment, second_moment, learning_rate;
+	bool updated;
+};
+
+template <bool PLAIN, typename G>
+__device__ inline AdamLane adam_front(const AdamArgs& a, const float debias, const bool is_matrix, const G g_in, const float w_fp, const float m1, const float m2) {
+	AdamLane l;
 	const float g = (float)g_in;
-	float gradient = a.inv_loss_scale_exact ? g * a.inv_loss_scale : g / a.loss_scale;
-	updated = is_matrix ? a.optimize_matrix_params != 0 : (a.optimize_non_matrix_params != 0 && gradient != 0);
-	const float weight_fp = w_fp;
-	if (is_matrix) gradient += a.l2_reg * weight_fp;
+	float gradient = (PLAIN || a.inv_loss_scale_exact) ? g * a.inv_loss_scale : g / a.loss_scale;
+	l.updated = is_matrix ? a.optimize_matrix_params != 0 : (a.optimize_non_matrix_params != 0 && gradient != 0);
+	l.weight_fp = w_fp;
+	if (is_matrix) gradient += a.l2_reg * w_fp;
 	const float gradient_sq = gradient * gradient;
-	const float first_moment = a.beta1 * m1 + (1 - a.beta1) * gradient;
-	const float second_moment = a.beta2 * m2 + (1 - a.beta2) * gradient_sq;
+	l.first_moment = a.beta1 * m1 + (1 - a.beta1) * gradient;
+	l.second_moment = a.beta2 * m2 + (1 - a.beta2) * gradient_sq;
 	float learning_rate = a.learning_rate;
 	if (!is_matrix) learning_rate *= a.non_matrix_learning_rate_factor;
-	const uint32_t current_step = step + 1;
-	float debias = common_debias;
-	if (updated && current_step != a.common_step) debias = debias_of(min(current_step, a.common_step));
-	learning_rate *= debias;
-	const float effective_learning_rate = fminf(fmaxf(learning_rate / (sqrtf(second_moment) + a.epsilon), a.lower_lr_bound), a.upper_lr_bound);
-	const float decayed_weight = (1 - a.relative_weight_decay * learning_rate) * weight_fp - copysignf(a.absolute_weight_decay * learning_rate, weight_fp);
-	float new_weight = decayed_weight - effective_learning_rate * first_moment;
-	if (a.weight_clipping_magnitude != 0.0f) new_weight = fminf(fmaxf(new_weight, -a.weight_clipping_magnitude), a.weight_clipping_magnitude);
-	w_fp = updated ? new_weight : weight_fp;
+	l.learning_rate = learning_rate * debias;
+	return l;
+}
+
+template <bool PLAIN, typename W>
+__device__ inline void adam_back(const AdamArgs& a, const AdamLane& l, const float rate, float& w_fp, W& w_h, float& m1, float& m2, uint32_t& step) {
+	const float effective_learning_rate = fminf(fmaxf(rate, a.lower_lr_bound), a.upper_lr_bound);
+	const float decayed_weight = (1 - a.relative_weight_decay * l.learning_rate) * l.weight_fp - copysignf(a.absolute_weight_decay * l.learning_rate, l.weight_fp);
+	float new_weight = decayed_weight - effective_learning_rate * l.first_moment;
+	if constexpr (!PLAIN) {
+		if (a.weight_clipping_magnitude != 0.0f) new_weight = fminf(fmaxf(new_weight, -a.weight_clipping_magnitude), a.weight_clipping_magnitude);
+	}
+	w_fp = l.updated ? new_weight : l.weight_fp;
 	w_h = (W)new_weight;
-	m1 = updated ? first_moment : m1;
-	m2 = updated ? second_moment : m2;
-	step = updated ? current_step : step;
+	m1 = l.updated ? l.first_moment : m1;
+	m2 = l.updated ? l.second_moment : m2;
+	step = l.updated ? step + 1 : step;
+}
+
+template <bool PLAIN = false, typename G, typename W>
+__device__ inline void adam_one(const AdamArgs& a, const float debias, const bool is_matrix, const G g_in, float& w_fp, W& w_h, float& m1, float& m2, uint32_t& step, bool& updated) {
+	const AdamLane l = adam_front<PLAIN>(a, debias, is_matrix, g_in, w_fp, m1, m2);
+	float rate;
+	if (adam_epsilon_in_range(a) && (adam_sqrt_excess(l.second_moment) | adam_div_n_excess(l.learning_rate)) < ADAM_SQRT_SPAN) rate = adam_div_fast(l.learning_rate, adam_sqrt_fast(l.second_moment) + a.epsilon);
+	else rate = l.learning_rate / (sqrtf(l.second_moment) + a.epsilon);
+	adam_back<PLAIN>(a, l, rate, w_fp, w_h, m1, m2, step);
+	updated = l.updated;
+}
+
+static_assert(ADAM_SQRT_SPAN == ADAM_DIV_N_SPAN && (ADAM_SQRT_SPAN & (ADAM_SQRT_SPAN - 1)) == 0, "the joint range test ORs the excesses");
+template <bool PLAIN, typename G, typename W>
+__device__ inline void adam_four(const AdamArgs& a, const float (&debias)[4], const bool (&is_matrix)[4], const G (&g_in)[4], float (&w_fp)[4], W (&w_h)[4], float (&m1)[4], float (&m2)[4],
+                                 uint32_t (&step)[4], bool (&updated)[4]) {
+	AdamLane l[4];
+	uint32_t excess = 0;
+#pragma unroll
+	for (int e = 0; e < 4; ++e) {
+		l[e] = adam_front<PLAIN>(a, debias[e], is_matrix[e], g_in[e], w_fp[e], m1[e], m2[e]);
+		excess |= adam_sqrt_excess(l[e].second_moment) | adam_div_n_excess(l[e].learning_rate);
+	}
+	float rate[4];
+	if (adam_epsilon_in_range(a) && excess < ADAM_SQRT_SPAN) {
+#pragma unroll
+		for (int e = 0; e < 4; ++e) rate[e] = adam_div_fast(l[e].learning_rate, adam_sqrt_fast(l[e].second_moment) + a.epsilon);
+	} else {
+#pragma unroll
+		for (int e = 0; e < 4; ++e) rate[e] = l[e].learning_rate / (sqrtf(l[e].second_moment) + a.epsilon);
+	}
+#pragma unroll
+	for (int e = 0; e < 4; ++e) {
+		adam_back<PLAIN>(a, l[e], rate[e], w_fp[e], w_h[e], m1[e], m2[e], step[e]);
+		updated[e] = l[e].updated;
+	}
 }
 
 }
diff --git a/tiny-cuda-nn_amd/csrc/capi.cpp b/tiny-cuda-nn_amd/csrc/capi.cpp
--- a/tiny-cuda-nn_amd/csrc/capi.cpp
+++ b/tiny-cuda-nn_amd/csrc/capi.cpp
@@ -160,6 +160,10 @@
 		HIP_CHECK_THROW(hipGetLastError());
 	});
 }
+int tcnn_adam_math_sweep(tcnn_stream_t stream, int what, uint64_t first, uint64_t count, uint32_t n_numerators, float numerator_lo, float numerator_hi, uint64_t seed,
+                         uint64_t* mismatches, uint64_t* first_bad) {
+	return guarded([&] { adam_math_sweep((hipStream_t)stream, what, first, count, n_numerators, numerator_lo, numerator_hi, seed, mismatches, first_bad); });
+}
 int tcnn_has_networks(void) { return 1; }
 float tcnn_default_loss_scale(int precision) { return precision == TCNN_PRECISION_FP32 ? 1.0f : LOSS_SCALE_FP16; }
 int tcnn_preferred_precision(void) { return TCNN_PRECISION_FP16; }
diff --git a/tiny-cuda-nn_amd/csrc/k_misc.hip b/tiny-cuda-nn_amd/csrc/k_misc.hip
--- a/tiny-cuda-nn_amd/csrc/k_misc.hip
+++ b/tiny-cuda-nn_amd/csrc/k_misc.hip
@@ -7,6 +7,8 @@
 #include "reduce_device.h"
 
 #include <hip/hip_fp16.h>
+
+#include <cstring>
 
 #include <cmath>
 #include <limits>
@@ -307,15 +309,30 @@
 template <typename G> struct GradQuad;
 template <> struct GradQuad<half_t> { typedef h4 type; };
 template <> struct GradQuad<float> { typedef f4 type; };
-template <bool QUAD_UNIFORM, typename STEP_T, typename G, typename W>
+__device__ inline void adam_load_debias(const float* __restrict__ debias_table, const uint32_t common_step, const uint4 st, float (&debias)[4]) {
+	debias[0] = debias_table[min(st.x + 1, common_step)];
+	debias[1] = debias_table[min(st.y + 1, common_step)];
+	debias[2] = debias_table[min(st.z + 1, common_step)];
+	debias[3] = debias_table[min(st.w + 1, common_step)];
+}
+template <typename STEP_T, typename G, typename W>
+__device__ inline void adam_single(const AdamArgs& a, const float* __restrict__ debias_table, const bool is_matrix, const size_t i, const G g, float* __restrict__ w_fp, W* __restrict__ w,
+                                   float* __restrict__ m1, float* __restrict__ m2, STEP_T* __restrict__ steps) {
+	bool up;
+	W wh;
+	uint32_t st1 = steps[i];
+	adam_one(a, debias_table[min(st1 + 1, a.common_step)], is_matrix, g, w_fp[i], wh, m1[i], m2[i], st1, up);
+	steps[i] = (STEP_T)st1;
+	if constexpr (sizeof(W) == 2) { if (up) w[i] = wh; }
+}
+
+template <bool PLAIN, bool QUAD_UNIFORM, typename STEP_T, typename G, typename W>
 __global__ void __launch_bounds__(256) k_adam(
 	const AdamArgs a, const size_t n, const size_t n_matrix,
 	float* __restrict__ w_fp, W* __restrict__ w, const G* __restrict__ g, float* __restrict__ m1, float* __restrict__ m2, STEP_T* __restrict__ steps,
 	const float* __restrict__ debias_table
 ) {
 	const size_t base = (size_t)blockIdx.x * (256 * 4 * ADAM_Q) + threadIdx.x * 4;
-	const float debias = debias_table[a.common_step];
-	const auto from_table = [&](const uint32_t t) { return debias_table[t]; };
 	typedef typename GradQuad<G>::type g4;
 	g4 gv[ADAM_Q];
 	bool live[ADAM_Q];
@@ -333,14 +350,16 @@
 	}
 	float4 wf[ADAM_Q], a1[ADAM_Q], a2[ADAM_Q];
 	uint4 st[ADAM_Q];
+	float debias[ADAM_Q][4];
 #pragma unroll
 	for (int q = 0; q < ADAM_Q; ++q) {
 		const size_t i4 = base + (size_t)q * 1024;
 		if (live[q]) {
+			st[q] = adam_load_steps(steps + i4);
 			wf[q] = *(const float4*)(w_fp + i4);
 			a1[q] = *(const float4*)(m1 + i4);
 			a2[q] = *(const float4*)(m2 + i4);
-			st[q] = adam_load_steps(steps + i4);
+			adam_load_debias(debias_table, a.common_step, st[q], debias[q]);
 		}
 	}
 #pragma unroll
@@ -350,14 +369,16 @@
 			W wh[4];
 			bool up[4];
 			const bool quad_matrix = i4 < n_matrix;
-			adam_one(a, from_table, debias, QUAD_UNIFORM ? quad_matrix : i4 + 0 < n_matrix, gv[q][0], wf[q].x, wh[0], a1[q].x, a2[q].x, st[q].x, up[0]);
-			adam_one(a, from_table, debias, QUAD_UNIFORM ? quad_matrix : i4 + 1 < n_matrix, gv[q][1], wf[q].y, wh[1], a1[q].y, a2[q].y, st[q].y, up[1]);
-			adam_one(a, from_table, debias, QUAD_UNIFORM ? quad_matrix : i4 + 2 < n_matrix, gv[q][2], wf[q].z, wh[2], a1[q].z, a2[q].z, st[q].z, up[2]);
-			adam_one(a, from_table, debias, QUAD_UNIFORM ? quad_matrix : i4 + 3 < n_matrix, gv[q][3], wf[q].w, wh[3], a1[q].w, a2[q].w, st[q].w, up[3]);
-			*(float4*)(w_fp + i4) = wf[q];
-			*(float4*)(m1 + i4) = a1[q];
-			*(float4*)(m2 + i4) = a2[q];
-			adam_store_steps(steps + i4, st[q]);
+			const bool is_matrix[4] = {QUAD_UNIFORM ? quad_matrix : i4 + 0 < n_matrix, QUAD_UNIFORM ? quad_matrix : i4 + 1 < n_matrix, QUAD_UNIFORM ? quad_matrix : i4 + 2 < n_matrix,
+			                           QUAD_UNIFORM ? quad_matrix : i4 + 3 < n_matrix};
+			const G gq[4] = {gv[q][0], gv[q][1], gv[q][2], gv[q][3]};
+			float w4[4] = {wf[q].x, wf[q].y, wf[q].z, wf[q].w}, f4_[4] = {a1[q].x, a1[q].y, a1[q].z, a1[q].w}, s4[4] = {a2[q].x, a2[q].y, a2[q].z, a2[q].w};
+			uint32_t c4[4] = {st[q].x, st[q].y, st[q].z, st[q].w};
+			adam_four<PLAIN>(a, debias[q], is_matrix, gq, w4, wh, f4_, s4, c4, up);
+			*(float4*)(w_fp + i4) = float4{w4[0], w4[1], w4[2], w4[3]};
+			*(float4*)(m1 + i4) = float4{f4_[0], f4_[1], f4_[2], f4_[3]};
+			*(float4*)(m2 + i4) = float4{s4[0], s4[1], s4[2], s4[3]};
+			adam_store_steps(steps + i4, uint4{c4[0], c4[1], c4[2], c4[3]});
 			if constexpr (sizeof(W) == 2) {
 				if (up[0] && up[1] && up[2] && up[3]) {
 					*(h4*)(w + i4) = h4{wh[0], wh[1], wh[2], wh[3]};
@@ -367,14 +388,7 @@
 				}
 			}
 		} else if (i4 < n && i4 + 4 > n) {
-			for (size_t i = i4; i < n; ++i) {
-				bool up;
-				W wh;
-				uint32_t st1 = steps[i];
-				adam_one(a, from_table, debias, i < n_matrix, g[i], w_fp[i], wh, m1[i], m2[i], st1, up);
-				steps[i] = (STEP_T)st1;
-				if constexpr (sizeof(W) == 2) { if (up) w[i] = wh; }
-			}
+			for (size_t i = i4; i < n; ++i) adam_single(a, debias_table, i < n_matrix, i, g[i], w_fp, w, m1, m2, steps);
 		}
 	}
 }
@@ -387,14 +401,7 @@
 ) {
 	const size_t i = (size_t)blockIdx.x * blockDim.x + threadIdx.x;
 	if (i >= n) return;
-	const float debias = debias_table[a.common_step];
-	const auto from_table = [&](const uint32_t t) { return debias_table[t]; };
-	bool up;
-	W wh;
-	uint32_t st1 = steps[i];
-	adam_one(a, from_table, debias,  i < n_matrix, g[i], w_fp[i], wh, m1[i], m2[i], st1, up);
-	steps[i] = (STEP_T)st1;
-	if constexpr (sizeof(W) == 2) { if (up) w[i] = wh; }
+	adam_single(a, debias_table, i < n_matrix, i, g[i], w_fp, w, m1, m2, steps);
 }
 
 __global__ void __launch_bounds__(128) k_random_uniform(const size_t n, const uint64_t state, const uint64_t inc, float* __restrict__ out, const float lower, const float upper) {
@@ -600,6 +607,7 @@
 }
 
 namespace {
+inline bool adam_args_plain(const AdamArgs& a) { return a.inv_loss_scale_exact != 0 && a.weight_clipping_magnitude == 0.0f; }
 __global__ void __launch_bounds__(256) k_adam_widen_steps(const size_t n, const uint16_t* __restrict__ in, uint32_t* __restrict__ out) {
 	const size_t i = (size_t)blockIdx.x * blockDim.x + threadIdx.x;
 	if (i < n) out[i] = in[i];
@@ -612,8 +620,12 @@
 		return;
 	}
 	const dim3 grid(blocks_for((n + 3) / 4, 256 * ADAM_Q));
-	if (n_matrix % 4 == 0) hipLaunchKernelGGL((k_adam<true, STEP_T, G, W>), grid, dim3(256), 0, stream, a, n, n_matrix, w_fp, w, g, m1, m2, steps, debias_table);
-	else hipLaunchKernelGGL((k_adam<false, STEP_T, G, W>), grid, dim3(256), 0, stream, a, n, n_matrix, w_fp, w, g, m1, m2, steps, debias_table);
+	const bool uniform = n_matrix % 4 == 0;
+	if (adam_args_plain(a)) {
+		if (uniform) hipLaunchKernelGGL((k_adam<true, true, STEP_T, G, W>), grid, dim3(256), 0, stream, a, n, n_matrix, w_fp, w, g, m1, m2, steps, debias_table);
+		else hipLaunchKernelGGL((k_adam<true, false, STEP_T, G, W>), grid, dim3(256), 0, stream, a, n, n_matrix, w_fp, w, g, m1, m2, steps, debias_table);
+	} else if (uniform) hipLaunchKernelGGL((k_adam<false, true, STEP_T, G, W>), grid, dim3(256), 0, stream, a, n, n_matrix, w_fp, w, g, m1, m2, steps, debias_table);
+	else hipLaunchKernelGGL((k_adam<false, false, STEP_T, G, W>), grid, dim3(256), 0, stream, a, n, n_matrix, w_fp, w, g, m1, m2, steps, debias_table);
 }
 template <typename G, typename W>
 void adam_launch_steps(hipStream_t stream, const AdamArgs& a, size_t n, size_t n_matrix, float* w_fp, W* w, const G* g, float* m1, float* m2, void* steps, bool steps16, const float* debias_table) {
@@ -643,22 +655,25 @@
 constexpr uint32_t PRO_MAX_BLOCKS_PER_RANGE = 64;
 __host__ __device__ inline uint32_t pro_range_blocks(const uint32_t n_elems) { return min(PRO_MAX_BLOCKS_PER_RANGE, max(1u, (n_elems / 4 + PRO_THREADS - 1) / PRO_THREADS)); }
 
-template <typename STEP_T, typename DebiasOf>
-__device__ inline void adam_quad(const AdamArgs& a, DebiasOf&& from_table, const float debias, const bool quad_matrix, const size_t i4, const h4 gv,
+template <bool PLAIN, typename STEP_T>
+__device__ inline void adam_quad(const AdamArgs& a, const float* __restrict__ debias_table, const bool quad_matrix, const size_t i4, const h4 gv,
                                  float* __restrict__ w_fp, half_t* __restrict__ w, float* __restrict__ m1, float* __restrict__ m2, STEP_T* __restrict__ steps) {
 	if (!quad_matrix && gv[0] == (half_t)0.0f && gv[1] == (half_t)0.0f && gv[2] == (half_t)0.0f && gv[3] == (half_t)0.0f) return;
-	float4 wf = *(const float4*)(w_fp + i4), a1 = *(const float4*)(m1 + i4), a2 = *(const float4*)(m2 + i4);
-	uint4 st = adam_load_steps(steps + i4);
+	const uint4 st = adam_load_steps(steps + i4);
+	const float4 wf = *(const float4*)(w_fp + i4), a1 = *(const float4*)(m1 + i4), a2 = *(const float4*)(m2 + i4);
+	float debias[4];
+	adam_load_debias(debias_table, a.common_step, st, debias);
 	half_t wh[4];
 	bool up[4];
-	adam_one(a, from_table, debias, quad_matrix, gv[0], wf.x, wh[0], a1.x, a2.x, st.x, up[0]);
-	adam_one(a, from_table, debias, quad_matrix, gv[1], wf.y, wh[1], a1.y, a2.y, st.y, up[1]);
-	adam_one(a, from_table, debias, quad_matrix, gv[2], wf.z, wh[2], a1.z, a2.z, st.z, up[2]);
-	adam_one(a, from_table, debias, quad_matrix, gv[3], wf.w, wh[3], a1.w, a2.w, st.w, up[3]);
-	*(float4*)(w_fp + i4) = wf;
-	*(float4*)(m1 + i4) = a1;
-	*(float4*)(m2 + i4) = a2;
-	adam_store_steps(steps + i4, st);
+	const bool is_matrix[4] = {quad_matrix, quad_matrix, quad_matrix, quad_matrix};
+	const half_t gq[4] = {gv[0], gv[1], gv[2], gv[3]};
+	float w4[4] = {wf.x, wf.y, wf.z, wf.w}, f4_[4] = {a1.x, a1.y, a1.z, a1.w}, s4[4] = {a2.x, a2.y, a2.z, a2.w};
+	uint32_t c4[4] = {st.x, st.y, st.z, st.w};
+	adam_four<PLAIN>(a, debias, is_matrix, gq, w4, wh, f4_, s4, c4, up);
+	*(float4*)(w_fp + i4) = float4{w4[0], w4[1], w4[2], w4[3]};
+	*(float4*)(m1 + i4) = float4{f4_[0], f4_[1], f4_[2], f4_[3]};
+	*(float4*)(m2 + i4) = float4{s4[0], s4[1], s4[2], s4[3]};
+	adam_store_steps(steps + i4, uint4{c4[0], c4[1], c4[2], c4[3]});
 	if (up[0] && up[1] && up[2] && up[3]) {
 		*(h4*)(w + i4) = h4{wh[0], wh[1], wh[2], wh[3]};
 	} else {
@@ -686,12 +701,10 @@
 #define TCNN_PRO_Q 1
 #endif
 constexpr int PRO_Q = TCNN_PRO_Q;
-template <typename STEP_T>
+template <bool PLAIN, typename STEP_T>
 __global__ void TCNN_PRO_BOUNDS k_adam_prologue(const AdamArgs a, const size_t n, const size_t n_matrix, float* __restrict__ w_fp, half_t* __restrict__ w, half_t* __restrict__ g,
                                                                float* __restrict__ m1, float* __restrict__ m2, STEP_T* __restrict__ steps, const float* __restrict__ debias_table, const PrologueArgs p) {
 	__shared__ float part[SLAB_REDUCE_GROUPS * SLAB_REDUCE_ELEMS];
-	const float debias = debias_table[a.common_step];
-	const auto from_table = [&](const uint32_t t) { return debias_table[t]; };
 	const uint32_t tid = threadIdx.x;
 	if (blockIdx.x < p.n_reduce_blocks) {
 		const uint32_t e = tid & (SLAB_REDUCE_ELEMS - 1), grp = tid / SLAB_REDUCE_ELEMS;
@@ -714,12 +727,7 @@
 			if (p.reduce_accumulate) s += (float)g[i];
 			const half_t gh = (half_t)s;
 			g[i] = gh;
-			bool up;
-			half_t wh;
-			uint32_t st1 = steps[i];
-			adam_one(a, from_table, debias, i < n_matrix, gh, w_fp[i], wh, m1[i], m2[i], st1, up);
-			steps[i] = (STEP_T)st1;
-			if (up) w[i] = wh;
+			adam_single(a, debias_table, i < n_matrix, i, gh, w_fp, w, m1, m2, steps);
 		}
 		return;
 	}
@@ -745,7 +753,7 @@
 			}
 			const h4 gv = h4{fixed_to_half(s[0]), fixed_to_half(s[1]), fixed_to_half(s[2]), fixed_to_half(s[3])};
 			*(h4*)(g + i4) = gv;
-			adam_quad(a, from_table, debias, i4 < n_matrix, i4, gv, w_fp, w, m1, m2, steps);
+			adam_quad<PLAIN>(a, debias_table, i4 < n_matrix, i4, gv, w_fp, w, m1, m2, steps);
 		}
 		return;
 	}
@@ -764,7 +772,7 @@
 #pragma unroll
 	for (int k = 0; k < PRO_Q; ++k) {
 		const size_t i4 = p.bulk_begin + (((size_t)(b - p.n_range_blocks) * PRO_Q + k) * PRO_THREADS + tid) * 4;
-		if (live[k]) adam_quad(a, from_table, debias, i4 < n_matrix, i4, gv[k], w_fp, w, m1, m2, steps);
+		if (live[k]) adam_quad<PLAIN>(a, debias_table, i4 < n_matrix, i4, gv[k], w_fp, w, m1, m2, steps);
 	}
 }
 }
@@ -807,8 +815,11 @@
 	const AdamArgs a = make_adam_args(h, loss_scale, current_step);
 	const uint32_t bulk_blocks = div_round_up((uint32_t)((n - p.bulk_begin) / 4), PRO_THREADS * (uint32_t)PRO_Q);
 	const dim3 grid(p.n_reduce_blocks + p.n_range_blocks + bulk_blocks);
-	if (steps16) hipLaunchKernelGGL(k_adam_prologue<uint16_t>, grid, dim3(PRO_THREADS), 0, stream, a, n, n_matrix, w_fp, (half_t*)w_half, (half_t*)g_half, m1, m2, (uint16_t*)steps, debias_table, p);
-	else hipLaunchKernelGGL(k_adam_prologue<uint32_t>, grid, dim3(PRO_THREADS), 0, stream, a, n, n_matrix, w_fp, (half_t*)w_half, (half_t*)g_half, m1, m2, (uint32_t*)steps, debias_table, p);
+	if (adam_args_plain(a)) {
+		if (steps16) hipLaunchKernelGGL((k_adam_prologue<true, uint16_t>), grid, dim3(PRO_THREADS), 0, stream, a, n, n_matrix, w_fp, (half_t*)w_half, (half_t*)g_half, m1, m2, (uint16_t*)steps, debias_table, p);
+		else hipLaunchKernelGGL((k_adam_prologue<true, uint32_t>), grid, dim3(PRO_THREADS), 0, stream, a, n, n_matrix, w_fp, (half_t*)w_half, (half_t*)g_half, m1, m2, (uint32_t*)steps, debias_table, p);
+	} else if (steps16) hipLaunchKernelGGL((k_adam_prologue<false, uint16_t>), grid, dim3(PRO_THREADS), 0, stream, a, n, n_matrix, w_fp, (half_t*)w_half, (half_t*)g_half, m1, m2, (uint16_t*)steps, debias_table, p);
+	else hipLaunchKernelGGL((k_adam_prologue<false, uint32_t>), grid, dim3(PRO_THREADS), 0, stream, a, n, n_matrix, w_fp, (half_t*)w_half, (half_t*)g_half, m1, m2, (uint32_t*)steps, debias_table, p);
 	HIP_CHECK_THROW(hipGetLastError());
 	return true;
 }
@@ -816,6 +827,95 @@
 void adam_fill_debias_table(hipStream_t stream, float beta1, float beta2, uint32_t from, uint32_t to, float* table) {
 	if (to <= from) return;
 	hipLaunchKernelGGL(k_adam_debias_table, dim3(blocks_for(to - from, 256)), dim3(256), 0, stream, beta1, beta2, from, to, table);
+}
+
+namespace {
+__device__ inline uint32_t sweep_hash(const uint32_t v) {
+	const uint32_t s = v * 747796405u + 2891336453u;
+	const uint32_t w = ((s >> ((s >> 28u) + 4u)) ^ s) * 277803737u;
+	return (w >> 22u) ^ w;
+}
+__device__ inline void sweep_report(const unsigned long long bad, const unsigned long long first_bad, unsigned long long* __restrict__ out) {
+	if (bad) {
+		atomicAdd(out, bad);
+		atomicMin(out + 1, first_bad);
+	}
+}
+__global__ void __launch_bounds__(256) k_adam_sweep_sqrt(const uint64_t first, const uint64_t count, unsigned long long* __restrict__ out) {
+	unsigned long long bad = 0, first_bad = ~0ull;
+	for (uint64_t i = (uint64_t)blockIdx.x * 256 + threadIdx.x; i < count; i += (uint64_t)gridDim.x * 256) {
+		const uint32_t b = (uint32_t)(first + i);
+		const float x = __uint_as_float(b);
+		if (__float_as_uint(adam_sqrt(x)) != __float_as_uint(sqrtf(x))) {
+			++bad;
+			first_bad = min(first_bad, (unsigned long long)b);
+		}
+	}
+	sweep_report(bad, first_bad, out);
+}
+__global__ void __launch_bounds__(256) k_adam_sweep_div_grid(const uint64_t first, const uint64_t count, const uint32_t n_numerators, const uint32_t lo_bits, const uint32_t hi_bits,
+                                                             const uint32_t seed, unsigned long long* __restrict__ out) {
+	unsigned long long bad = 0, first_bad = ~0ull;
+	for (uint64_t i = (uint64_t)blockIdx.x * 256 + threadIdx.x; i < count; i += (uint64_t)gridDim.x * 256) {
+		const uint32_t db = (uint32_t)(first + i);
+		const float d = __uint_as_float(db);
+		const uint32_t pitch = (hi_bits - lo_bits) / n_numerators;
+		const uint32_t n_here = adam_div_d_in_range(d) ? n_numerators : 1u;
+		uint32_t lowest = 0xffffffffu;
+		for (uint32_t k = 0; k < n_here; ++k) {
+			const uint32_t nb = (lo_bits + pitch * k) ^ (sweep_hash(k ^ seed) & 0xffffu);
+			const float n = __uint_as_float(nb);
+			const bool differs = __float_as_uint(adam_div(n, d)) != __float_as_uint(n / d);
+			bad += differs ? 1u : 0u;
+			lowest = min(lowest, differs ? nb : 0xffffffffu);
+		}
+		if (lowest != 0xffffffffu) first_bad = min(first_bad, (unsigned long long)db << 32 | lowest);
+	}
+	sweep_report(bad, first_bad, out);
+}
+__global__ void __launch_bounds__(256) k_adam_sweep_div_pairs(const uint64_t count, const uint32_t seed, unsigned long long* __restrict__ out) {
+	unsigned long long bad = 0, first_bad = ~0ull;
+	for (uint64_t i = (uint64_t)blockIdx.x * 256 + threadIdx.x; i < count; i += (uint64_t)gridDim.x * 256) {
+		const uint32_t h1 = sweep_hash((uint32_t)(2 * i) ^ seed), h2 = sweep_hash((uint32_t)(2 * i + 1) ^ seed), h3 = sweep_hash(h1 ^ h2);
+		const uint32_t nb = ((127u - 70u + (((h1 >> 23) & 0xffu) * 140u >> 8)) << 23) | (h1 & 0x7fffffu) | ((h3 & 3u) == 0 ? 0x80000000u : 0u);
+		const uint32_t db = ((127u - 54u + (((h2 >> 23) & 0xffu) * 78u >> 8)) << 23) | (h2 & 0x7fffffu) | ((h3 & 12u) == 0 ? 0x80000000u : 0u);
+		const float n = __uint_as_float(nb), d = __uint_as_float(db);
+		if (__float_as_uint(adam_div(n, d)) != __float_as_uint(n / d)) {
+			++bad;
+			first_bad = min(first_bad, (unsigned long long)db << 32 | nb);
+		}
+	}
+	sweep_report(bad, first_bad, out);
+}
+}
+
+void adam_math_sweep(hipStream_t stream, int what, uint64_t first, uint64_t count, uint32_t n_numerators, float numerator_lo, float numerator_hi, uint64_t seed, uint64_t* mismatches,
+                     uint64_t* first_bad) {
+	CHECK_THROW(what >= 0 && what <= 2 && mismatches != nullptr && first_bad != nullptr);
+	CHECK_THROW(what == 2 || first + count <= (1ull << 32));
+	uint32_t lo_bits = 0, hi_bits = 0;
+	if (what == 1) {
+		CHECK_THROW(n_numerators > 0 && numerator_lo > 0.0f && numerator_hi >= numerator_lo && std::isfinite(numerator_hi));
+		std::memcpy(&lo_bits, &numerator_lo, 4);
+		std::memcpy(&hi_bits, &numerator_hi, 4);
+	}
+	unsigned long long host[2] = {0ull, ~0ull};
+	unsigned long long* out = nullptr;
+	HIP_CHECK_THROW(hipMalloc((void**)&out, sizeof(host)));
+	hipError_t err = hipMemcpyAsync(out, host, sizeof(host), hipMemcpyHostToDevice, stream);
+	if (err == hipSuccess && count) {
+		const dim3 grid((uint32_t)std::min<uint64_t>((count + 255) / 256, 8192));
+		if (what == 0) hipLaunchKernelGGL(k_adam_sweep_sqrt, grid, dim3(256), 0, stream, first, count, out);
+		else if (what == 1) hipLaunchKernelGGL(k_adam_sweep_div_grid, grid, dim3(256), 0, stream, first, count, n_numerators, lo_bits, hi_bits, (uint32_t)seed, out);
+		else hipLaunchKernelGGL(k_adam_sweep_div_pairs, grid, dim3(256), 0, stream, count, (uint32_t)seed, out);
+		err = hipGetLastError();
+	}
+	if (err == hipSuccess) err = hipMemcpyAsync(host, out, sizeof(host), hipMemcpyDeviceToHost, stream);
+	if (err == hipSuccess) err = hipStreamSynchronize(stream);
+	(void)hipFree(out);
+	HIP_CHECK_THROW(err);
+	*mismatches = host[0];
+	*first_bad = host[1];
 }
 
 namespace {
diff --git a/tiny-cuda-nn_amd/csrc/k_mlp.hip b/tiny-cuda-nn_amd/csrc/k_mlp.hip
--- a/tiny-cuda-nn_amd/csrc/k_mlp.hip
+++ b/tiny-cuda-nn_amd/csrc/k_mlp.hip
@@ -609,7 +609,7 @@
 	half_t w_h;
 	bool updated;
 	const float* __restrict__ table = adam.debias_table;
-	adam_one(adam.args, [&](const uint32_t t) { return table[t]; }, table[adam.args.common_step], true, g, w_fp, w_h, m1, m2, step, updated);
+	adam_one(adam.args, table[min(step + 1, adam.args.common_step)], true, g, w_fp, w_h, m1, m2, step, updated);
 	if (updated) {
 		adam.w_fp[i] = w_fp;
 		((half_t*)adam.w_half)[i] = w_h;
diff --git a/tiny-cuda-nn_amd/csrc/tcnn_common.h b/tiny-cuda-nn_amd/csrc/tcnn_common.h
--- a/tiny-cuda-nn_amd/csrc/tcnn_common.h
+++ b/tiny-cuda-nn_amd/csrc/tcnn_common.h
@@ -571,6 +571,8 @@
                GradientPrecision precision = GradientPrecision::Fp16, Precision weight_precision = Precision::Fp16);
 void adam_widen_steps(hipStream_t stream, size_t n, const void* steps16, void* steps32);
 void adam_fill_debias_table(hipStream_t stream, float beta1, float beta2, uint32_t from, uint32_t to, float* table);
+void adam_math_sweep(hipStream_t stream, int what, uint64_t first, uint64_t count, uint32_t n_numerators, float numerator_lo, float numerator_hi, uint64_t seed, uint64_t* mismatches,
+                     uint64_t* first_bad);
 void copy_columns(hipStream_t stream, size_t elem_bytes, uint32_t n, const void* src, uint32_t src_stride, uint32_t src_col, void* dst, uint32_t dst_stride, uint32_t dst_col, uint32_t width);
 void sgd_step(hipStream_t stream, size_t n, float loss_scale, float learning_rate, float l2_reg, float* weights_full_precision, void* weights, const void* gradients,
               GradientPrecision precision = GradientPrecision::Fp16, Precision weight_precision = Precision::Fp16);
diff --git a/tiny-cuda-nn_amd/tinycudann/_C.py b/tiny-cuda-nn_amd/tinycudann/_C.py
--- a/tiny-cuda-nn_amd/tinycudann/_C.py
+++ b/tiny-cuda-nn_amd/tinycudann/_C.py
@@ -153,6 +153,7 @@
     "tcnn_optimizer_weights_restored": (_int, [_vp, _vp, _vp]),
     "tcnn_optimizer_serialize": (_int, [_vp, _pp, C.POINTER(_sz)]),
     "tcnn_optimizer_deserialize": (_int, [_vp, _vp, _sz]),
+    "tcnn_adam_math_sweep": (_int, [_vp, _int, C.c_uint64, C.c_uint64, _u32, _f32, _f32, C.c_uint64, C.POINTER(C.c_uint64), C.POINTER(C.c_uint64)]),
     "tcnn_loss_type": (_int, [_cp, C.POINTER(C.c_int)]),
     "tcnn_loss_name": (_cp, [_int]),
     "tcnn_loss_evaluate": (_int, [_int, _vp, _f32, _vp, _u32, _u32, _vp, _u32, _int, _vp, _vp, _vp, _u32, _vp, _u32, _vp]),
```

Measured after the change: 1.417 billion, median of 6. +1.5%, better.
